# KumarRobotics/top_down_renderer

Measured on AMD Instinct MI355X. Metric: particle-updates/sec (render+score+resample), higher is better.
Workload: dtype f32

## Files before the change

top_down_renderer_amd/csrc/tdr_common.h:

```cpp
#ifndef TDR_COMMON_H_
#define TDR_COMMON_H_
#include <hip/hip_runtime.h>

#include <cmath>
#include <cstdarg>
#include <cstdint>
#include <cstdio>
#include <cstdlib>
#include <cstring>
#include <limits>
#include <type_traits>
#include <utility>
#include <vector>

#include "tdr.h"
#include "tdr_config.h"
#include "tdr_internal.h"

#ifndef TDR_SCORE_U
#define TDR_SCORE_U 4
#endif
#ifndef TDR_XCD_SWIZZLE
#define TDR_XCD_SWIZZLE 0
#endif
#ifndef TDR_OOB_ALIAS
#define TDR_OOB_ALIAS 1
#endif

int tdr_fail(int code, const char* fmt, ...);
#define fail tdr_fail
#define HIP_TRY(expr)                                                                       \
  do {                                                                                      \
    hipError_t e_ = (expr);                                                                 \
    if (e_ != hipSuccess) return fail(TDR_ERR_HIP, "%s: %s", #expr, hipGetErrorString(e_)); \
  } while (0)
#define LAUNCH_CHECK(name)                                                                   \
  do {                                                                                       \
    hipError_t e_ = hipGetLastError();                                                       \
    if (e_ != hipSuccess) return fail(TDR_ERR_HIP, "launch %s: %s", name, hipGetErrorString(e_)); \
  } while (0)

int tdr_libm_fma();

static inline int64_t cdiv(int64_t a, int64_t b) { return (a + b - 1) / b; }

template <class F>
static inline int with_flags(F&& f) { return f(); }
template <class F, class... Rest>
static inline int with_flags(F&& f, bool b, Rest... rest) {
  auto next = [&](auto B) { return with_flags([&](auto... bs) { return f(B, bs...); }, rest...); };
  return b ? next(std::true_type{}) : next(std::false_type{});
}
template <class F>
static inline int with_nv4(int rf, const char* who, F&& f) {
  switch (rf / 4) {
    case 1: return f(std::integral_constant<int, 1>{});
    case 2: return f(std::integral_constant<int, 2>{});
    case 3: return f(std::integral_constant<int, 3>{});
    case 4: return f(std::integral_constant<int, 4>{});
    default: return fail(TDR_ERR_ARG, "%s: unsupported record size %d", who, rf);
  }
}

#define PFX_HEAD 2048
#define INI_TILE 2048
#define INI_MAX_TILES 2048
int tdr_chain_total(const float* raw, const float* mean_dev, int kind, int64_t n, float* total_out, void* workspace,
                    bool have_sums, hipStream_t st);
struct UwExact {
  float sum, mean, bsum, pad;
};
int tdr_uw_chunk_pass1(const float* raw, int64_t n, void* workspace, int* cnt_valid, hipStream_t st);
int tdr_uw_chunk_pass2(const float* raw, int64_t n, UwExact* ex, const int* cnt_valid, void* workspace, int* cnt_under,
                       hipStream_t st);
int tdr_uw_small(const float* raw, const float* last_dist, int64_t n, float* w, float* info, hipStream_t st);
int tdr_mt_raw_stream(const uint32_t* state, int64_t nblocks, uint32_t* raw, hipStream_t s);
int tdr_mt_advance(const uint32_t* raw, int64_t nblocks, const uint32_t* consumed, uint32_t* state, hipStream_t s);
__host__ __device__ inline bool tdr_has_kslot(int ncls, int rf) { return ncls + 2 <= rf; }
uint32_t* tdr_profile_stats_ptr();
uint32_t* tdr_profile_gate_ptr();
uint32_t* tdr_profile_su_list_ptr();
#endif
```

top_down_renderer_amd/csrc/tdr_filter.hip:

```cpp
#include <random>

#include <rocprim/device/device_radix_sort.hpp>
using TdrSortConfig = rocprim::radix_sort_config<rocprim::default_config, rocprim::merge_sort_config<512, 512, 4>, rocprim::default_config>;

#include "tdr_common.h"
#include "tdr_filter_dev.h"

__device__ __forceinline__ uint32_t mulhi32(uint32_t a, uint32_t b) { return __umulhi(a, b); }
__device__ void philox4x32_10(uint32_t c[4], uint32_t k0, uint32_t k1) {
#pragma unroll
  for (int r = 0; r < 10; r++) {
    uint32_t hi0 = mulhi32(0xD2511F53u, c[0]), lo0 = 0xD2511F53u * c[0];
    uint32_t hi1 = mulhi32(0xCD9E8D57u, c[2]), lo1 = 0xCD9E8D57u * c[2];
    uint32_t n0 = hi1 ^ c[1] ^ k0, n1 = lo1, n2 = hi0 ^ c[3] ^ k1, n3 = lo0;
    c[0] = n0; c[1] = n1; c[2] = n2; c[3] = n3;
    k0 += 0x9E3779B9u; k1 += 0xBB67AE85u;
  }
}

__global__ void propagate_kernel(float* __restrict__ st, int64_t cap, int64_t n, float* __restrict__ last_dist,
                                 float tx, float ty, float omega, int scale_freeze, float pos_cov, float theta_cov,
                                 const float* __restrict__ z4, uint64_t seed, uint64_t step, int64_t index_base,
                                 int libm_fma) {
  const int64_t p = (int64_t)blockIdx.x * blockDim.x + threadIdx.x;
  if (p >= n) return;
  float z[4];
  if (z4) {
    z[0] = z4[4 * p]; z[1] = z4[4 * p + 1]; z[2] = z4[4 * p + 2]; z[3] = z4[4 * p + 3];
  } else {
    uint64_t gi = (uint64_t)(index_base + p);
    uint32_t c[4] = {(uint32_t)gi, (uint32_t)(gi >> 32), (uint32_t)step, (uint32_t)(step >> 32)};
    philox4x32_10(c, (uint32_t)seed, (uint32_t)(seed >> 32));
    float u0 = ((float)(c[0] >> 8) + 1.0f) * (1.0f / 16777216.0f), u1 = (float)(c[1] >> 8) * (1.0f / 16777216.0f);
    float u2 = ((float)(c[2] >> 8) + 1.0f) * (1.0f / 16777216.0f), u3 = (float)(c[3] >> 8) * (1.0f / 16777216.0f);
    float r0 = sqrtf(-2.0f * logf(u0)), r1 = sqrtf(-2.0f * logf(u2));
    z[0] = r0 * cosf(6.283185307f * u1); z[1] = r0 * sinf(6.283185307f * u1);
    z[2] = r1 * cosf(6.283185307f * u3); z[3] = r1 * sinf(6.283185307f * u3);
  }
  propagate_particle(st, cap, p, last_dist, z, tx, ty, omega, scale_freeze, pos_cov, theta_cov, libm_fma);
}

extern "C" int tdr_k_propagate(float* st, int64_t cap, int64_t n, float* last_dist, float tx, float ty, float omega,
                               int scale_freeze, float pos_cov, float theta_cov, const float* z4, uint64_t seed,
                               uint64_t step, int64_t index_base, void* stream) {
  if (!st || !last_dist) return fail(TDR_ERR_ARG, "propagate: null pointer");
  if (n < 0 || cap < n) return fail(TDR_ERR_ARG, "propagate: n exceeds capacity");
  if (n == 0) return TDR_OK;
  hipLaunchKernelGGL(propagate_kernel, dim3((unsigned)cdiv(n, 256)), dim3(256), 0, (hipStream_t)stream, st, cap, n,
                     last_dist, tx, ty, omega, scale_freeze, pos_cov, theta_cov, z4, seed, step, index_base,
                     tdr_libm_fma());
  LAUNCH_CHECK("propagate");
  return TDR_OK;
}

extern "C" void* tdr_rng_create(uint32_t seed) { return new std::mt19937(seed); }
extern "C" void tdr_rng_destroy(void* rng) { delete (std::mt19937*)rng; }
extern "C" float tdr_rng_uniform_host(void* rng) {
  std::uniform_real_distribution<float> d(0., 1.);
  return d(*(std::mt19937*)rng);
}
extern "C" int tdr_propagate_normals_host(void* rng, int64_t n, int scale_freeze, float* z4) {
  if (!rng || !z4 || n < 0) return fail(TDR_ERR_ARG, "propagate_normals: bad arguments");
  std::mt19937& gen = *(std::mt19937*)rng;
  for (int64_t p = 0; p < n; p++) {
    std::normal_distribution<float> disp{0, 1}, th{0, 1};
    z4[4 * p + 0] = th(gen);
    z4[4 * p + 1] = disp(gen);
    z4[4 * p + 2] = disp(gen);
    if (!scale_freeze) {
      std::normal_distribution<float> sc{0, 1};
      z4[4 * p + 3] = sc(gen);
    } else {
      z4[4 * p + 3] = 0.f;
    }
  }
  return TDR_OK;
}

static bool on_road_host(const float* maps, int ncls, int rows, int cols, float resolution, int px, int py) {
  const int c0 = (int)((float)px / resolution), c1 = (int)((float)py / resolution);
  if (ncls < 2) return false;
  if (!(c0 < cols && c1 < rows && c0 >= 0 && c1 >= 0)) return false;
  return maps[(size_t)1 * rows * cols + c1 + (size_t)rows * c0] < 1;
}
static tdr_state draw_particle(std::mt19937& gen, const float* maps, int ncls, int rows, int cols, float resolution,
                               const tdr_filter_params* fp) {
  std::uniform_real_distribution<float> uniform_dist(0., 1.);
  std::normal_distribution<float> normal_dist(0., 1.);
  tdr_state st;
  std::memset(&st, 0, sizeof(st));
  const float map_w = (float)cols * resolution, map_h = (float)rows * resolution;
  if (fp->fixed_scale < 0) st.scale = (float)std::pow(10, ((double)uniform_dist(gen) - 0.5) * 2);
  else st.scale = fp->fixed_scale;
  while (true) {
    if (fp->init_pos_px_x > 0) {
      st.init_x_px = std::min(std::max(normal_dist(gen) * fp->init_pos_px_cov + fp->init_pos_px_x, 0.f), map_w);
      st.init_y_px = std::min(std::max(normal_dist(gen) * fp->init_pos_px_cov + fp->init_pos_px_y, 0.f), map_h);
    } else {
      st.init_x_px = uniform_dist(gen) * map_w;
      st.init_y_px = uniform_dist(gen) * map_h;
    }
    if (on_road_host(maps, ncls, rows, cols, resolution, (int)st.init_x_px, (int)st.init_y_px)) break;
  }
  if (fp->init_pos_deg_theta != std::numeric_limits<float>::infinity()) {
    st.theta = normal_dist(gen) * fp->init_pos_deg_cov + fp->init_pos_deg_theta;
    st.theta = (float)((double)st.theta * (M_PI / 180));
    st.have_init = 1;
  } else {
    st.theta = 0;
    st.have_init = 0;
  }
  return st;
}
extern "C" int tdr_init_particle_host(void* rng, const float* class_maps, int ncls, int rows, int cols, float resolution,
                                      const tdr_filter_params* fp, tdr_state* out) {
  if (!rng || !class_maps || !fp || !out) return fail(TDR_ERR_ARG, "init_particle: bad arguments");
  if (ncls < 2) return fail(TDR_ERR_ARG, "init_particle: class 1 (road) is required for the on-road test");
  bool any_road = false;
  for (size_t k = 0; k < (size_t)rows * cols && !any_road; k++) any_road = class_maps[(size_t)rows * cols + k] < 1;
  if (!any_road) return fail(TDR_ERR_ARG, "init_particle: the map has no road cell, rejection sampling cannot end");
  *out = draw_particle(*(std::mt19937*)rng, class_maps, ncls, rows, cols, resolution, fp);
  return TDR_OK;
}
extern "C" int tdr_init_particles_host(void* rng, const float* class_maps, int ncls, int rows, int cols,
                                       float resolution, const tdr_filter_params* fp, int max_num, tdr_state* out,
                                       int64_t* n_out) {
  if (!rng || !class_maps || !fp || !out || !n_out || max_num < 0) return fail(TDR_ERR_ARG, "init_particles: bad arguments");
  if (ncls < 2) return fail(TDR_ERR_ARG, "init_particles: class 1 (road) is required for the on-road test");
  std::mt19937& gen = *(std::mt19937*)rng;
  bool any_road = false;
  for (size_t k = 0; k < (size_t)rows * cols && !any_road; k++) any_road = class_maps[(size_t)rows * cols + k] < 1;
  if (!any_road) return fail(TDR_ERR_ARG, "init_particles: the map has no road cell, rejection sampling cannot end");
  const size_t num_at_scale = (fp->fixed_scale < 0) ? 10 : 1;
  int64_t count = 0;
  for (int i = 0; i < (int)((size_t)max_num / num_at_scale); i++) {
    const tdr_state proto = draw_particle(gen, class_maps, ncls, rows, cols, resolution, fp);
    for (float scale = 0; scale < 1; scale += 1. / num_at_scale) {
      tdr_state part = draw_particle(gen, class_maps, ncls, rows, cols, resolution, fp);
      if (fp->fixed_scale < 0) {
        part = proto;
        part.scale = (float)std::pow(10., (double)scale);
      }
      if (count < max_num + 16) out[count] = part;
      count++;
      (void)draw_particle(gen, class_maps, ncls, rows, cols, resolution, fp);
    }
  }
  *n_out = count;
  return TDR_OK;
}

__device__ long long block_sum_ll(long long v, long long* sh) {
  const int lane = threadIdx.x & 63, wave = threadIdx.x >> 6;
  for (int o = 32; o > 0; o >>= 1) v += __shfl_down(v, o, 64);
  __syncthreads();
  if (lane == 0) sh[wave] = v;
  __syncthreads();
  long long t = 0;
  const int nw = blockDim.x >> 6;
  for (int w = 0; w < nw; w++) t += sh[w];
  return t;
}

#define UW_G 256
struct UwScratch {
  double a[UW_G];
  double b[UW_G];
};
__device__ __forceinline__ void uw_chunk(int64_t n, int64_t& lo, int64_t& hi) {
  const int64_t per = (n + UW_G - 1) / UW_G;
  lo = (int64_t)blockIdx.x * per;
  hi = lo + per < n ? lo + per : n;
  if (lo > n) lo = n;
}
__device__ double uw_total(const double* part) {
  __shared__ double stage[UW_G];
  __shared__ double result;
  __syncthreads();
  for (int g = threadIdx.x; g < UW_G; g += blockDim.x) stage[g] = part[g];
  __syncthreads();
  if (threadIdx.x == 0) {
    double t = 0;
    for (int g = 0; g < UW_G; g++) t += stage[g];
    result = t;
  }
  __syncthreads();
  return result;
}
__device__ long long uw_count_total(const int* __restrict__ cnt, int nch, long long* shl) {
  long long c = 0;
  for (int j = threadIdx.x; j < nch; j += blockDim.x) c += cnt[j];
  return block_sum_ll(c, shl);
}
__global__ __launch_bounds__(256) void uw_pass3(const float* __restrict__ raw, int64_t n, const UwExact* ex,
                                                const int* __restrict__ cnt_under, int nch, UwScratch* s3,
                                                float* __restrict__ w) {
  __shared__ double shd[4];
  __shared__ long long shl[4];
  const float sum = ex->sum, mean = ex->mean;
  const long long num_under = uw_count_total(cnt_under, nch, shl);
  const float bottom = sqrtf(ex->bsum / (float)num_under);
  const bool fallback = (sum == 0.f || num_under < 1);
  const float fill = mean - bottom;
  int64_t lo, hi;
  uw_chunk(n, lo, hi);
  double acc = 0;
  for (int64_t i = lo + threadIdx.x; i < hi; i += 256) {
    float v = raw[i];
    v = fallback ? 1.f : (isnan(v) ? fill : v);
    w[i] = v;
    acc += (double)v;
  }
  const double t = block_sum_d(acc, shd);
  if (threadIdx.x == 0) s3->a[blockIdx.x] = t;
}
__global__ __launch_bounds__(256) void uw_pass4(const float* __restrict__ last_dist, int64_t n, const UwScratch* s3,
                                                UwScratch* s4, float* __restrict__ w) {
  __shared__ double shd[4];
  const float fs1 = (float)uw_total(s3->a);
  const float fn = (float)n;
  int64_t lo, hi;
  uw_chunk(n, lo, hi);
  double acc = 0;
  for (int64_t i = lo + threadIdx.x; i < hi; i += 256) {
    float v = w[i] / fs1;
    const float d = fminf(last_dist[i] * 5.f, 1.f);
    v = d * v + (1.f - d) / fn;
    w[i] = v;
    acc += (double)v;
  }
  const double t = block_sum_d(acc, shd);
  if (threadIdx.x == 0) s4->a[blockIdx.x] = t;
}
__device__ __forceinline__ void uw_write_info(const UwScratch* s5, const int* __restrict__ cnt_valid,
                                              const int* __restrict__ cnt_under, int nch, const UwExact* ex, float* info) {
  static_assert(UW_G == 256, "one candidate per thread");
  __shared__ float sb[4];
  __shared__ long long si[4];
  __shared__ long long shl[4];
  float best = (float)s5->a[threadIdx.x];
  long long besti = (long long)s5->b[threadIdx.x];
  if (best != best) { best = -INFINITY; besti = 0x7fffffffffffffffll; }
  for (int o = 32; o > 0; o >>= 1) {
    const float ob = __shfl_down(best, o, 64);
    const long long oi = __shfl_down(besti, o, 64);
    if (ob > best || (ob == best && oi < besti)) { best = ob; besti = oi; }
  }
  if ((threadIdx.x & 63) == 0) { sb[threadIdx.x >> 6] = best; si[threadIdx.x >> 6] = besti; }
  const float sum = ex->sum, mean = ex->mean;
  const long long nv = uw_count_total(cnt_valid, nch, shl), nu = uw_count_total(cnt_under, nch, shl);
  const float bottom = sqrtf(ex->bsum / (float)nu);
  if (threadIdx.x != 0) return;
  for (int k = 1; k < 4; k++)
    if (sb[k] > best || (sb[k] == best && si[k] < besti)) { best = sb[k]; besti = si[k]; }
  if (besti == 0x7fffffffffffffffll) besti = 0;
  info[0] = __int_as_float((int)besti);
  info[1] = sum; info[2] = mean; info[3] = bottom; info[4] = (sum == 0.f || nu < 1) ? 1.f : 0.f;
  info[5] = (float)nv; info[6] = (float)nu; info[7] = 0.f;
}
__global__ __launch_bounds__(256) void uw_pass5(int64_t n, const UwScratch* s4, UwScratch* s5, float* __restrict__ w) {
  __shared__ float sb[4];
  __shared__ long long si[4];
  const float fs2 = (float)uw_total(s4->a);
  int64_t lo, hi;
  uw_chunk(n, lo, hi);
  float best = -INFINITY;
  long long besti = 0x7fffffffffffffffll;
  for (int64_t i = lo + threadIdx.x; i < hi; i += 256) {
    const float v = w[i] / fs2;
    w[i] = v;
    if (v > best || (v == best && i < besti)) { best = v; besti = i; }
  }
  for (int o = 32; o > 0; o >>= 1) {
    const float ob = __shfl_down(best, o, 64);
    const long long oi = __shfl_down(besti, o, 64);
    if (ob > best || (ob == best && oi < besti)) { best = ob; besti = oi; }
  }
  if ((threadIdx.x & 63) == 0) { sb[threadIdx.x >> 6] = best; si[threadIdx.x >> 6] = besti; }
  __syncthreads();
  if (threadIdx.x == 0) {
    for (int k = 1; k < 4; k++)
      if (sb[k] > best || (sb[k] == best && si[k] < besti)) { best = sb[k]; besti = si[k]; }
    s5->a[blockIdx.x] = (double)best;
    s5->b[blockIdx.x] = (double)besti;
  }
}
__global__ __launch_bounds__(256) void uw_pass6(const UwScratch* s5, const int* __restrict__ cnt_valid,
                                                const int* __restrict__ cnt_under, int nch, const UwExact* ex, float* info) {
  uw_write_info(s5, cnt_valid, cnt_under, nch, ex, info);
}

#define TDR_UW_SINGLE_MAX_N 32768
extern "C" int tdr_k_update_weights(const float* raw_w, const float* last_dist, int64_t n, float* w_out,
                                    float* info_out, void* stream) {
  if (!raw_w || !last_dist || !w_out || !info_out) return fail(TDR_ERR_ARG, "update_weights: null pointer");
  if (n < 1) return fail(TDR_ERR_ARG, "update_weights: n must be >= 1");
  hipStream_t s = (hipStream_t)stream;
  if (n <= TDR_UW_SINGLE_MAX_N) {
    const int rc = tdr_uw_small(raw_w, last_dist, n, w_out, info_out, s);
    if (rc) return rc;
    LAUNCH_CHECK("update_weights");
    return TDR_OK;
  }
  constexpr size_t kFixed = 8 * sizeof(float) + 64 + 3 * sizeof(UwScratch) + sizeof(UwExact) + 64;
  static_assert(kFixed + 40 * 1024 <= TDR_UW_INFO_FLOATS * sizeof(float), "info scratch");
  UwScratch* sc = reinterpret_cast<UwScratch*>(
      (reinterpret_cast<uintptr_t>(info_out + 8) + 63) & ~(uintptr_t)63);
  UwExact* ex = reinterpret_cast<UwExact*>(sc + 3);
  void* chain_ws = reinterpret_cast<void*>((reinterpret_cast<uintptr_t>(ex + 1) + 63) & ~(uintptr_t)63);
  const size_t chain_room = TDR_UW_INFO_FLOATS * sizeof(float) - kFixed;
  const int64_t nch = tdr_prefix_workspace_bytes(n) / 32;
  if ((size_t)tdr_prefix_workspace_bytes(n) + (size_t)nch * 2 * sizeof(int) > chain_room)
    return fail(TDR_ERR_ARG, "update_weights: n = %lld needs more than TDR_UW_INFO_FLOATS of scratch", (long long)n);
  int* cnt_valid = reinterpret_cast<int*>(reinterpret_cast<char*>(chain_ws) + tdr_prefix_workspace_bytes(n));
  int* cnt_under = cnt_valid + nch;
  int rc = tdr_uw_chunk_pass1(raw_w, n, chain_ws, cnt_valid, s);
  if (rc) return rc;
  rc = tdr_chain_total(raw_w, nullptr, 0, n, &ex->sum, chain_ws, true, s);
  if (rc) return rc;
  rc = tdr_uw_chunk_pass2(raw_w, n, ex, cnt_valid, chain_ws, cnt_under, s);
  if (rc) return rc;
  rc = tdr_chain_total(raw_w, &ex->mean, 1, n, &ex->bsum, chain_ws, true, s);
  if (rc) return rc;
  hipLaunchKernelGGL(uw_pass3, dim3(UW_G), dim3(256), 0, s, raw_w, n, (const UwExact*)ex, (const int*)cnt_under, (int)nch,
                     sc + 0, w_out);
  hipLaunchKernelGGL(uw_pass4, dim3(UW_G), dim3(256), 0, s, last_dist, n, (const UwScratch*)(sc + 0), sc + 1, w_out);
  hipLaunchKernelGGL(uw_pass5, dim3(UW_G), dim3(256), 0, s, n, (const UwScratch*)(sc + 1), sc + 2, w_out);
  hipLaunchKernelGGL(uw_pass6, dim3(1), dim3(256), 0, s, (const UwScratch*)(sc + 2), (const int*)cnt_valid,
                     (const int*)cnt_under, (int)nch, (const UwExact*)ex, info_out);
  LAUNCH_CHECK("update_weights(multi)");
  return TDR_OK;
}

__global__ void resample_kernel(const float* __restrict__ runmax, int64_t n, int64_t n_new, float shift,
                                int64_t i_begin, int64_t i_end, int32_t* __restrict__ idx) {
  const int64_t i = i_begin + (int64_t)blockIdx.x * blockDim.x + threadIdx.x;
  if (i >= i_end) return;
  idx[i - i_begin] = (int32_t)resample_pick(runmax, n, n_new, i, shift);
}

extern "C" int tdr_k_resample(const float* runmax, int64_t n, int64_t n_new, float shift, int64_t i_begin,
                              int64_t i_end, int32_t* idx_out, void* stream) {
  if (!runmax || !idx_out) return fail(TDR_ERR_ARG, "resample: null pointer");
  if (n < 1 || n_new < 1 || i_begin < 0 || i_end > n_new || i_begin > i_end)
    return fail(TDR_ERR_ARG, "resample: bad range");
  if (i_begin == i_end) return TDR_OK;
  hipLaunchKernelGGL(resample_kernel, dim3((unsigned)cdiv(i_end - i_begin, 256)), dim3(256), 0, (hipStream_t)stream,
                     runmax, n, n_new, shift, i_begin, i_end, idx_out);
  LAUNCH_CHECK("resample");
  return TDR_OK;
}

__global__ void resample_dev_kernel(const float* __restrict__ runmax, int64_t n, int64_t n_new, const float* __restrict__ shift_dev,
                                    int64_t i_begin, int64_t i_end, int32_t* __restrict__ idx) {
  const int64_t i = i_begin + (int64_t)blockIdx.x * blockDim.x + threadIdx.x;
  if (i >= i_end) return;
  idx[i - i_begin] = (int32_t)resample_pick(runmax, n, n_new, i, *shift_dev);
}
extern "C" int tdr_k_resample_dev(const float* runmax, int64_t n, int64_t n_new, const float* shift_dev, int64_t i_begin,
                                  int64_t i_end, int32_t* idx_out, void* stream) {
  if (!runmax || !idx_out || !shift_dev) return fail(TDR_ERR_ARG, "resample: null pointer");
  if (n < 1 || n_new < 1 || i_begin < 0 || i_end > n_new || i_begin > i_end)
    return fail(TDR_ERR_ARG, "resample: bad range");
  if (i_begin == i_end) return TDR_OK;
  hipLaunchKernelGGL(resample_dev_kernel, dim3((unsigned)cdiv(i_end - i_begin, 256)), dim3(256), 0, (hipStream_t)stream,
                     runmax, n, n_new, shift_dev, i_begin, i_end, idx_out);
  LAUNCH_CHECK("resample");
  return TDR_OK;
}

__device__ __forceinline__ void gather_state(const float* __restrict__ src, int64_t src_cap, int64_t src_shard, int64_t j,
                                             float* __restrict__ dst, int64_t dst_cap, int64_t i) {
  if (src_shard > 0) {
    const int64_t r = j / src_shard, l = j - r * src_shard;
#pragma unroll
    for (int f = 0; f < TDR_ST_FIELDS; f++) dst[f * dst_cap + i] = src[(r * TDR_ST_FIELDS + f) * src_shard + l];
  } else {
    gather_particle(src, src_cap, j, dst, dst_cap, i);
  }
}
__global__ void gather_states_kernel(const float* __restrict__ src, int64_t src_cap, int64_t src_shard,
                                     const int32_t* __restrict__ idx, int64_t n_new, float* __restrict__ dst,
                                     int64_t dst_cap) {
  const int64_t i = (int64_t)blockIdx.x * blockDim.x + threadIdx.x;
  if (i >= n_new) return;
  gather_state(src, src_cap, src_shard, idx[i], dst, dst_cap, i);
}

extern "C" int tdr_k_gather_states(const float* src, int64_t src_cap, int64_t src_shard, const int32_t* idx,
                                   int64_t n_new, float* dst, int64_t dst_cap, void* stream) {
  if (!src || !idx || !dst) return fail(TDR_ERR_ARG, "gather_states: null pointer");
  if (n_new < 0 || dst_cap < n_new || src_shard < 0) return fail(TDR_ERR_ARG, "gather_states: n_new exceeds capacity");
  if (n_new == 0) return TDR_OK;
  hipLaunchKernelGGL(gather_states_kernel, dim3((unsigned)cdiv(n_new, 256)), dim3(256), 0, (hipStream_t)stream, src,
                     src_cap, src_shard, idx, n_new, dst, dst_cap);
  LAUNCH_CHECK("gather_states");
  return TDR_OK;
}

__device__ __forceinline__ McScratch* mc_scratch(float* out) { return reinterpret_cast<McScratch*>(out + 24); }
__global__ __launch_bounds__(1024) void mean_cov_kernel(const float* __restrict__ st, int64_t cap, int64_t n,
                                                       const float* __restrict__ about, float* __restrict__ out,
                                                       int libm_fma) {
  mean_cov_body(st, cap, n, about, out, libm_fma);
}
__global__ __launch_bounds__(MC_THREADS) void mc_sums_kernel(const float* __restrict__ st, int64_t cap, int64_t n,
                                                             float* __restrict__ out, int libm_fma) {
  mc_sums_body(st, cap, n, mc_scratch(out), libm_fma);
}
__global__ __launch_bounds__(MC_THREADS) void mc_cov_kernel(const float* __restrict__ st, int64_t cap, int64_t n,
                                                            const float* __restrict__ about, float* __restrict__ out) {
  mc_cov_body(st, cap, n, about, mc_scratch(out));
}
__global__ __launch_bounds__(MC_THREADS) void mc_final_kernel(int64_t n, const float* __restrict__ about,
                                                              float* __restrict__ out) {
  mc_final_body(n, about, mc_scratch(out), out);
}

extern "C" int tdr_k_mean_cov(const float* st, int64_t cap, int64_t n, const float* about, float* out, void* stream) {
  if (!st || !out || n < 1 || cap < n) return fail(TDR_ERR_ARG, "mean_cov: bad arguments");
  hipStream_t s = (hipStream_t)stream;
  if (n <= MC_SINGLE_MAX_N) {
    hipLaunchKernelGGL(mean_cov_kernel, dim3(1), dim3(1024), 0, s, st, cap, n, about, out, tdr_libm_fma());
  } else {
    hipLaunchKernelGGL(mc_sums_kernel, dim3(MC_WGS), dim3(MC_THREADS), 0, s, st, cap, n, out, tdr_libm_fma());
    hipLaunchKernelGGL(mc_cov_kernel, dim3(MC_WGS), dim3(MC_THREADS), 0, s, st, cap, n, about, out);
    hipLaunchKernelGGL(mc_final_kernel, dim3(1), dim3(MC_THREADS), 0, s, n, about, out);
  }
  LAUNCH_CHECK("mean_cov");
  return TDR_OK;
}

__global__ void set_scale_kernel(float* __restrict__ st, int64_t cap, int64_t n, const float* __restrict__ scale) {
  const int64_t p = (int64_t)blockIdx.x * blockDim.x + threadIdx.x;
  if (p < n) st[TDR_ST_SCALE * cap + p] = *scale;
}
extern "C" int tdr_k_set_scale(float* st, int64_t cap, int64_t n, const float* scale_dev, void* stream) {
  if (!st || !scale_dev || n < 0 || cap < n) return fail(TDR_ERR_ARG, "set_scale: bad arguments");
  if (n == 0) return TDR_OK;
  hipLaunchKernelGGL(set_scale_kernel, dim3((unsigned)cdiv(n, 256)), dim3(256), 0, (hipStream_t)stream, st, cap, n,
                     scale_dev);
  LAUNCH_CHECK("set_scale");
  return TDR_OK;
}

__global__ void shift_init_kernel(float* __restrict__ st, int64_t cap, int64_t n, float dx, float dy) {
  const int64_t p = (int64_t)blockIdx.x * blockDim.x + threadIdx.x;
  if (p < n) {
    st[TDR_ST_INIT_X * cap + p] += dx;
    st[TDR_ST_INIT_Y * cap + p] += dy;
  }
}
extern "C" int tdr_k_shift_init(float* st, int64_t cap, int64_t n, float dx, float dy, void* stream) {
  if (!st || n < 0 || cap < n) return fail(TDR_ERR_ARG, "shift_init: bad arguments");
  if (n == 0) return TDR_OK;
  hipLaunchKernelGGL(shift_init_kernel, dim3((unsigned)cdiv(n, 256)), dim3(256), 0, (hipStream_t)stream, st, cap, n,
                     dx, dy);
  LAUNCH_CHECK("shift_init");
  return TDR_OK;
}

__device__ __forceinline__ void save_ml_state(const float* __restrict__ info, const float* __restrict__ st, int64_t cap,
                                              int64_t src_shard, int64_t n, float* __restrict__ out) {
  const int64_t best = ml_index(info, n);
  float f[TDR_ST_FIELDS];
  if (src_shard > 0) {
    const int64_t r = best / src_shard, l = best - r * src_shard;
#pragma unroll
    for (int k = 0; k < TDR_ST_FIELDS; k++) f[k] = st[(r * TDR_ST_FIELDS + k) * src_shard + l];
  } else {
#pragma unroll
    for (int k = 0; k < TDR_ST_FIELDS; k++) f[k] = st[(int64_t)k * cap + best];
  }
  ml_record(f, out);
}
__global__ void save_ml_state_kernel(const float* __restrict__ info, const float* __restrict__ st, int64_t cap,
                                     int64_t src_shard, int64_t n, float* __restrict__ out) {
  if (threadIdx.x != 0 || blockIdx.x != 0) return;
  save_ml_state(info, st, cap, src_shard, n, out);
}
extern "C" int tdr_k_save_ml_state(const float* info, const float* st, int64_t cap, int64_t src_shard, int64_t n,
                                   float* out12, void* stream) {
  if (!info || !st || !out12 || n < 1 || src_shard < 0 || (src_shard == 0 && cap < n))
    return fail(TDR_ERR_ARG, "save_ml_state: bad arguments");
  hipLaunchKernelGGL(save_ml_state_kernel, dim3(1), dim3(64), 0, (hipStream_t)stream, info, st, cap, src_shard, n,
                     out12);
  LAUNCH_CHECK("save_ml_state");
  return TDR_OK;
}

__global__ __launch_bounds__(256) void resample_gather_kernel(const float* __restrict__ runmax, int64_t n, int64_t n_new,
                                                              const float* __restrict__ shift_dev, float shift,
                                                              int64_t i_begin, int64_t i_end, int32_t* __restrict__ idx,
                                                              const float* __restrict__ src, int64_t src_cap,
                                                              int64_t src_shard, float* __restrict__ dst, int64_t dst_cap,
                                                              const float* __restrict__ info, float* __restrict__ out12) {
  const int64_t i = i_begin + (int64_t)blockIdx.x * blockDim.x + threadIdx.x;
  if (i < i_end) {
    const int64_t j = resample_pick(runmax, n, n_new, i, shift_dev ? *shift_dev : shift);
    idx[i - i_begin] = (int32_t)j;
    gather_state(src, src_cap, src_shard, j, dst, dst_cap, i - i_begin);
  }
  if (blockIdx.x == 0 && threadIdx.x == 0) save_ml_state(info, src, src_cap, src_shard, n, out12);
}
extern "C" int tdr_k_resample_gather(const float* runmax, int64_t n, int64_t n_new, const float* shift_dev, float shift,
                                     int64_t i_begin, int64_t i_end, int32_t* idx_out, const float* src, int64_t src_cap,
                                     int64_t src_shard, float* dst, int64_t dst_cap, const float* info, float* out12,
                                     void* stream) {
  if (!runmax || !idx_out || !src || !dst || !info || !out12) return fail(TDR_ERR_ARG, "resample_gather: null pointer");
  if (n < 1 || n_new < 1 || i_begin < 0 || i_end > n_new || i_begin > i_end)
    return fail(TDR_ERR_ARG, "resample_gather: bad range");
  if (src_shard < 0 || (src_shard == 0 && src_cap < n) || dst_cap < i_end - i_begin || dst == src)
    return fail(TDR_ERR_ARG, "resample_gather: bad state buffers");
  const unsigned blocks = (unsigned)std::max<int64_t>(1, cdiv(i_end - i_begin, 256));
  hipLaunchKernelGGL(resample_gather_kernel, dim3(blocks), dim3(256), 0, (hipStream_t)stream, runmax, n, n_new, shift_dev,
                     shift, i_begin, i_end, idx_out, src, src_cap, src_shard, dst, dst_cap, info, out12);
  LAUNCH_CHECK("resample_gather");
  return TDR_OK;
}

__global__ void sample_ml_states_kernel(const float* __restrict__ st, int64_t cap, int64_t n, int num,
                                        float* __restrict__ out) {
  const int i = blockIdx.x * blockDim.x + threadIdx.x;
  if (i >= num) return;
  sample_ml_state(st, cap, n, num, i, out + 3 * i);
}
extern "C" int tdr_k_sample_ml_states(const float* st, int64_t cap, int64_t n, int num, float* out, void* stream) {
  if (!st || !out || n < 1 || cap < n || num < 1) return fail(TDR_ERR_ARG, "sample_ml_states: bad arguments");
  hipLaunchKernelGGL(sample_ml_states_kernel, dim3((unsigned)cdiv(num, 256)), dim3(256), 0, (hipStream_t)stream, st,
                     cap, n, num, out);
  LAUNCH_CHECK("sample_ml_states");
  return TDR_OK;
}

__global__ void shard_pack2_kernel(const float* __restrict__ a, const float* __restrict__ b, int64_t nl,
                                   float* __restrict__ out) {
  const int64_t i = (int64_t)blockIdx.x * blockDim.x + threadIdx.x;
  if (i < nl) { out[i] = a[i]; out[nl + i] = b[i]; }
}
__global__ void shard_unpack2_kernel(const float* __restrict__ in, int world, int64_t nl, float* __restrict__ a,
                                     float* __restrict__ b) {
  const int64_t g = (int64_t)blockIdx.x * blockDim.x + threadIdx.x;
  if (g >= (int64_t)world * nl) return;
  const int64_t r = g / nl, l = g - r * nl;
  a[g] = in[(2 * r) * nl + l];
  b[g] = in[(2 * r + 1) * nl + l];
}
__global__ void unshard_states_kernel(const float* __restrict__ in, int world, int64_t nl, float* __restrict__ st,
                                      int64_t cap) {
  const int64_t g = (int64_t)blockIdx.x * blockDim.x + threadIdx.x;
  if (g >= (int64_t)world * nl) return;
  const int64_t r = g / nl, l = g - r * nl;
#pragma unroll
  for (int f = 0; f < TDR_ST_FIELDS; f++) st[f * cap + g] = in[(r * TDR_ST_FIELDS + f) * nl + l];
}
extern "C" int tdr_k_shard_pack2(const float* a, const float* b, int64_t nl, float* out, void* stream) {
  if (!a || !b || !out || nl < 0) return fail(TDR_ERR_ARG, "shard_pack2: bad arguments");
  if (nl == 0) return TDR_OK;
  hipLaunchKernelGGL(shard_pack2_kernel, dim3((unsigned)cdiv(nl, 256)), dim3(256), 0, (hipStream_t)stream, a, b, nl, out);
  LAUNCH_CHECK("shard_pack2");
  return TDR_OK;
}
extern "C" int tdr_k_shard_unpack2(const float* in, int world, int64_t nl, float* a_glob, float* b_glob, void* stream) {
  if (!in || !a_glob || !b_glob || world < 1 || nl < 0) return fail(TDR_ERR_ARG, "shard_unpack2: bad arguments");
  if (nl == 0) return TDR_OK;
  hipLaunchKernelGGL(shard_unpack2_kernel, dim3((unsigned)cdiv((int64_t)world * nl, 256)), dim3(256), 0,
                     (hipStream_t)stream, in, world, nl, a_glob, b_glob);
  LAUNCH_CHECK("shard_unpack2");
  return TDR_OK;
}
extern "C" int tdr_k_unshard_states(const float* in, int world, int64_t nl, float* st, int64_t cap, void* stream) {
  if (!in || !st || world < 1 || nl < 0 || cap < (int64_t)world * nl) return fail(TDR_ERR_ARG, "unshard_states: bad arguments");
  if (nl == 0) return TDR_OK;
  hipLaunchKernelGGL(unshard_states_kernel, dim3((unsigned)cdiv((int64_t)world * nl, 256)), dim3(256), 0,
                     (hipStream_t)stream, in, world, nl, st, cap);
  LAUNCH_CHECK("unshard_states");
  return TDR_OK;
}

__global__ void aos_to_soa_kernel(const tdr_state* __restrict__ aos, int64_t n, float* __restrict__ st, int64_t cap) {
  const int64_t p = (int64_t)blockIdx.x * blockDim.x + threadIdx.x;
  if (p >= n) return;
  const tdr_state s = aos[p];
  st[TDR_ST_INIT_X * cap + p] = s.init_x_px;
  st[TDR_ST_INIT_Y * cap + p] = s.init_y_px;
  st[TDR_ST_DX * cap + p] = s.dx_m;
  st[TDR_ST_DY * cap + p] = s.dy_m;
  st[TDR_ST_THETA * cap + p] = s.theta;
  st[TDR_ST_SCALE * cap + p] = s.scale;
  st[TDR_ST_HAVE_INIT * cap + p] = s.have_init ? 1.f : 0.f;
}
__global__ void soa_to_aos_kernel(const float* __restrict__ st, int64_t cap, int64_t n, tdr_state* __restrict__ aos) {
  const int64_t p = (int64_t)blockIdx.x * blockDim.x + threadIdx.x;
  if (p >= n) return;
  tdr_state s;
  s.init_x_px = st[TDR_ST_INIT_X * cap + p];
  s.init_y_px = st[TDR_ST_INIT_Y * cap + p];
  s.dx_m = st[TDR_ST_DX * cap + p];
  s.dy_m = st[TDR_ST_DY * cap + p];
  s.theta = st[TDR_ST_THETA * cap + p];
  s.scale = st[TDR_ST_SCALE * cap + p];
  s.have_init = st[TDR_ST_HAVE_INIT * cap + p] != 0.f;
  s.pad_[0] = s.pad_[1] = s.pad_[2] = 0;
  aos[p] = s;
}
extern "C" int tdr_k_states_aos_to_soa(const tdr_state* aos, int64_t n, float* st, int64_t cap, void* stream) {
  if (!aos || !st || n < 0 || cap < n) return fail(TDR_ERR_ARG, "aos_to_soa: bad arguments");
  if (n == 0) return TDR_OK;
  hipLaunchKernelGGL(aos_to_soa_kernel, dim3((unsigned)cdiv(n, 256)), dim3(256), 0, (hipStream_t)stream, aos, n, st,
                     cap);
  LAUNCH_CHECK("aos_to_soa");
  return TDR_OK;
}
extern "C" int tdr_k_states_soa_to_aos(const float* st, int64_t cap, int64_t n, tdr_state* aos, void* stream) {
  if (!aos || !st || n < 0 || cap < n) return fail(TDR_ERR_ARG, "soa_to_aos: bad arguments");
  if (n == 0) return TDR_OK;
  hipLaunchKernelGGL(soa_to_aos_kernel, dim3((unsigned)cdiv(n, 256)), dim3(256), 0, (hipStream_t)stream, st, cap, n,
                     aos);
  LAUNCH_CHECK("soa_to_aos");
  return TDR_OK;
}

__device__ __forceinline__ uint32_t spread_bits16(uint32_t v) {
  v &= 0xFFFFu;
  v = (v | (v << 8)) & 0x00FF00FFu;
  v = (v | (v << 4)) & 0x0F0F0F0Fu;
  v = (v | (v << 2)) & 0x33333333u;
  v = (v | (v << 1)) & 0x55555555u;
  return v;
}
__global__ void loc_key_kernel(const float* __restrict__ st, int64_t cap, int64_t n, float xmax, float ymax,
                               uint32_t* __restrict__ keys, int32_t* __restrict__ vals) {
  const int64_t p = (int64_t)blockIdx.x * blockDim.x + threadIdx.x;
  if (p >= n) return;
  const float sc = st[TDR_ST_SCALE * cap + p];
  float cx = st[TDR_ST_DX * cap + p] * sc + st[TDR_ST_INIT_X * cap + p];
  float cy = st[TDR_ST_DY * cap + p] * sc + st[TDR_ST_INIT_Y * cap + p];
  if (!(cx == cx)) cx = 0.f;
  if (!(cy == cy)) cy = 0.f;
  const uint32_t hx = (uint32_t)fminf(fmaxf(cx * 2.f, 0.f), xmax);
  const uint32_t hy = (uint32_t)fminf(fmaxf(cy * 2.f, 0.f), ymax);
  keys[p] = spread_bits16(hx) | (spread_bits16(hy) << 1);
  vals[p] = (int32_t)p;
}

__device__ __forceinline__ uint64_t spread_bits21_3(uint64_t v) {
  v &= 0x1FFFFFull;
  v = (v | (v << 32)) & 0x1F00000000FFFFull;
  v = (v | (v << 16)) & 0x1F0000FF0000FFull;
  v = (v | (v << 8)) & 0x100F00F00F00F00Full;
  v = (v | (v << 4)) & 0x10C30C30C30C30C3ull;
  v = (v | (v << 2)) & 0x1249249249249249ull;
  return v;
}
__global__ void loc_key_pose_kernel(const float* __restrict__ st, int64_t cap, int64_t n, float xmax, float ymax,
                                    float theta_step, uint64_t* __restrict__ keys, int32_t* __restrict__ vals) {
  const int64_t p = (int64_t)blockIdx.x * blockDim.x + threadIdx.x;
  if (p >= n) return;
  const float sc = st[TDR_ST_SCALE * cap + p];
  float cx = st[TDR_ST_DX * cap + p] * sc + st[TDR_ST_INIT_X * cap + p];
  float cy = st[TDR_ST_DY * cap + p] * sc + st[TDR_ST_INIT_Y * cap + p];
  float th = st[TDR_ST_THETA * cap + p];
  if (!(cx == cx)) cx = 0.f;
  if (!(cy == cy)) cy = 0.f;
  if (!(fabsf(th) < 1e6f)) th = 0.f;
  th = th - 6.2831855f * floorf(th / 6.2831855f);
  const uint64_t hx = (uint64_t)fminf(fmaxf(cx * 2.f, 0.f), xmax);
  const uint64_t hy = (uint64_t)fminf(fmaxf(cy * 2.f, 0.f), ymax);
  const uint64_t ht = (uint64_t)fminf(fmaxf(th / theta_step, 0.f), 2097151.f);
  keys[p] = spread_bits21_3(hx) | (spread_bits21_3(hy) << 1) | (spread_bits21_3(ht) << 2);
  vals[p] = (int32_t)p;
}
static size_t radix_tmp_bytes64(int64_t n) {
  size_t bytes = 0;
  uint64_t* k = nullptr;
  int32_t* v = nullptr;
  hipError_t e = rocprim::radix_sort_pairs(nullptr, bytes, k, k, v, v, (size_t)n, 0u, 63u, (hipStream_t)0, false);
  if (e != hipSuccess || bytes == 0) bytes = (size_t)(n + 4096) * 32;
  return bytes;
}
extern "C" size_t tdr_locality_pose_tmp_ints(int64_t n) {
  if (n < 1) n = 1;
  return (size_t)(5 * n + 64) + (radix_tmp_bytes64(n) + 3) / 4 + 64;
}
extern "C" int tdr_k_locality_order_pose(const float* st, int64_t cap, int64_t n, int map_rows, int map_cols,
                                         float theta_radius, int32_t* perm_out, int32_t* keys_tmp, void* stream) {
  if (!st || !perm_out || !keys_tmp || n < 0 || cap < n || map_rows < 1 || map_cols < 1 || !(theta_radius > 0.f))
    return fail(TDR_ERR_ARG, "locality_order_pose: bad arguments");
  if (map_rows > 1000000 || map_cols > 1000000) return fail(TDR_ERR_ARG, "locality_order_pose: map too large");
  if (n == 0) return TDR_OK;
  hipStream_t s = (hipStream_t)stream;
  uint64_t* keys_in = reinterpret_cast<uint64_t*>(keys_tmp);
  uint64_t* keys_out = keys_in + n;
  int32_t* vals_in = keys_tmp + 4 * n;
  void* tmp = keys_tmp + 5 * n + 64 - ((5 * n) % 64);
  size_t tmp_bytes = radix_tmp_bytes64(n);
  hipLaunchKernelGGL(loc_key_pose_kernel, dim3((unsigned)cdiv(n, 256)), dim3(256), 0, s, st, cap, n,
                     (float)(2 * map_cols - 1), (float)(2 * map_rows - 1), 0.5f / theta_radius, keys_in, vals_in);
  LAUNCH_CHECK("loc_key_pose");
  HIP_TRY(rocprim::radix_sort_pairs(tmp, tmp_bytes, keys_in, keys_out, vals_in, perm_out, (size_t)n, 0u, 63u, s, false));
  return TDR_OK;
}

static size_t radix_tmp_bytes(int64_t n) {
  size_t bytes = 0;
  uint32_t* k = nullptr;
  int32_t* v = nullptr;
  hipError_t e = rocprim::radix_sort_pairs<TdrSortConfig>(nullptr, bytes, k, k, v, v, (size_t)n, 0u, 32u, (hipStream_t)0, false);
  if (e != hipSuccess || bytes == 0) bytes = (size_t)(n + 4096) * 16;
  return bytes;
}

extern "C" size_t tdr_locality_tmp_ints(int64_t n, int map_rows, int map_cols) {
  (void)map_rows; (void)map_cols;
  if (n < 1) n = 1;
  return (size_t)(3 * n + 64) + (radix_tmp_bytes(n) + 3) / 4 + 64;
}

extern "C" int tdr_k_locality_order(const float* st, int64_t cap, int64_t n, int map_rows, int map_cols,
                                    int32_t* perm_out, int32_t* keys_tmp, void* stream) {
  if (!st || !perm_out || !keys_tmp || n < 0 || cap < n || map_rows < 1 || map_cols < 1)
    return fail(TDR_ERR_ARG, "locality_order: bad arguments");
  if (map_rows > 32767 || map_cols > 32767) return fail(TDR_ERR_ARG, "locality_order: map larger than 32767 px");
  if (n == 0) return TDR_OK;
  hipStream_t s = (hipStream_t)stream;
  uint32_t* keys_in = reinterpret_cast<uint32_t*>(keys_tmp);
  uint32_t* keys_out = keys_in + n;
  int32_t* vals_in = keys_tmp + 2 * n;
  void* tmp = keys_tmp + 3 * n + 64 - ((3 * n) % 64);
  size_t tmp_bytes = radix_tmp_bytes(n);
  hipLaunchKernelGGL(loc_key_kernel, dim3((unsigned)cdiv(n, 256)), dim3(256), 0, s, st, cap, n,
                     (float)(2 * map_cols - 1), (float)(2 * map_rows - 1), keys_in, vals_in);
  LAUNCH_CHECK("loc_key");
  unsigned bits = 2;
  while ((1u << (bits / 2)) < (unsigned)(2 * std::max(map_rows, map_cols)) && bits < 32) bits += 2;
  HIP_TRY(rocprim::radix_sort_pairs<TdrSortConfig>(tmp, tmp_bytes, keys_in, keys_out, vals_in, perm_out, (size_t)n, 0u, bits, s,
                                    false));
  return TDR_OK;
}
```

top_down_renderer_amd/csrc/tdr_prefix.hip:

```cpp
#include "tdr_common.h"
#include "tdr_batch.h"

#define TDR_PFX_BLOCK 4096
__global__ __launch_bounds__(64) void prefix_serial_kernel(const float* __restrict__ w, int64_t n,
                                                           float* __restrict__ runmax) {
  __shared__ float4 buf4[TDR_PFX_BLOCK / 4];
  float* buf = reinterpret_cast<float*>(buf4);
  const int lane = threadIdx.x;
  float run = 0.f;
  float carry_max = -INFINITY;
  for (int64_t base = 0; base < n; base += TDR_PFX_BLOCK) {
    const int cnt = (int)min((int64_t)TDR_PFX_BLOCK, n - base);
    for (int t = lane; t < TDR_PFX_BLOCK; t += 64) buf[t] = (t < cnt) ? w[base + t] : 0.f;
    __builtin_amdgcn_s_waitcnt(0);
    __builtin_amdgcn_wave_barrier();
    if (lane == 0) {
      const int q4 = (cnt + 3) / 4;
#pragma unroll 4
      for (int q = 0; q < q4; q++) {
        float4 v = buf4[q];
        run = run + v.x; v.x = run;
        run = run + v.y; v.y = run;
        run = run + v.z; v.z = run;
        run = run + v.w; v.w = run;
        buf4[q] = v;
      }
    }
    __builtin_amdgcn_s_waitcnt(0);
    __builtin_amdgcn_wave_barrier();
    float m = -INFINITY;
    float loc[64];
#pragma unroll
    for (int t = 0; t < 64; t++) {
      float x = buf[lane * 64 + t];
      if (x != x) x = -INFINITY;
      m = fmaxf(m, x);
      loc[t] = m;
    }
    float incl = m;
#pragma unroll
    for (int o = 1; o < 64; o <<= 1) {
      float t = __shfl_up(incl, o, 64);
      if (lane >= o) incl = fmaxf(incl, t);
    }
    float excl = __shfl_up(incl, 1, 64);
    if (lane == 0) excl = -INFINITY;
    excl = fmaxf(excl, carry_max);
    __builtin_amdgcn_wave_barrier();
#pragma unroll
    for (int t = 0; t < 64; t++) buf[lane * 64 + t] = fmaxf(loc[t], excl);
    __builtin_amdgcn_s_waitcnt(0);
    __builtin_amdgcn_wave_barrier();
    for (int t = lane; t < cnt; t += 64) runmax[base + t] = buf[t];
    carry_max = fmaxf(__shfl(incl, 63, 64), carry_max);
    __builtin_amdgcn_s_waitcnt(0);
    __builtin_amdgcn_wave_barrier();
  }
}

#define PFX_THREADS 1024
#define PFX_K 8
#define PFX_TILE (PFX_THREADS * PFX_K)
#define PFX_TIE_CAP 2048

__device__ __forceinline__ void pfx_sync() {
  __builtin_amdgcn_fence(__ATOMIC_RELEASE, "workgroup", "local");
  __builtin_amdgcn_s_barrier();
  __builtin_amdgcn_fence(__ATOMIC_ACQUIRE, "workgroup", "local");
}

template <int NT, class T>
__device__ __forceinline__ T pfx_block_scan(T v, T* sh, T& total) {
  const int lane = threadIdx.x & 63, wave = threadIdx.x >> 6;
#pragma unroll
  for (int o = 1; o < 64; o <<= 1) {
    T t = __shfl_up(v, o, 64);
    if (lane >= o) v += t;
  }
  pfx_sync();
  if (lane == 63) sh[wave] = v;
  pfx_sync();
  T off = 0, tot = 0;
#pragma unroll
  for (int k = 0; k < NT / 64; k++) {
    const T x = sh[k];
    if (k < wave) off += x;
    tot += x;
  }
  total = tot;
  return v + off;
}
template <int NT>
__device__ __forceinline__ float pfx_block_scan_max(float v, float* sh) {
  const int lane = threadIdx.x & 63, wave = threadIdx.x >> 6;
#pragma unroll
  for (int o = 1; o < 64; o <<= 1) {
    float t = __shfl_up(v, o, 64);
    if (lane >= o) v = fmaxf(v, t);
  }
  pfx_sync();
  if (lane == 63) sh[wave] = v;
  pfx_sync();
  float off = -INFINITY;
  for (int k = 0; k < wave; k++) off = fmaxf(off, sh[k]);
  return fmaxf(v, off);
}

template <int NT>
__device__ __forceinline__ void pfx_exact_range(const float* __restrict__ w, long long lo, long long hi,
                                             float* __restrict__ runmax, float* __restrict__ prefix_opt,
                                             float& r_io, float& carry_io, int head_len = PFX_HEAD) {
  const long long n = hi;
  __shared__ long long sh_ll[NT / 64];
  __shared__ int sh_i[NT / 64];
  __shared__ float sh_f[NT / 64];
  __shared__ int tie_pos[PFX_TIE_CAP];
  __shared__ long long tie_sval[PFX_TIE_CAP];
  __shared__ signed char tie_corr[PFX_TIE_CAP];
  __shared__ float head[PFX_HEAD];
  __shared__ float last_val[NT], last_max[NT];
  __shared__ int s_first_bad, s_first_cross, s_first_nz;
  __shared__ float s_r, s_carry;
  __shared__ long long s_base;
  const int tid = threadIdx.x;
  pfx_sync();
  if (tid == 0) { s_r = r_io; s_carry = carry_io; s_base = lo; }
  pfx_sync();
  if (lo == 0) {
    const int hn = (int)min((long long)head_len, (long long)n);
    for (int t = tid; t < hn; t += NT) head[t] = w[t];
    pfx_sync();
    if (tid == 0) {
      float run = 0.f, mx = -INFINITY;
      for (int t = 0; t < hn; t++) {
        run = run + head[t];
        if (prefix_opt) prefix_opt[t] = run;
        if (run == run) mx = fmaxf(mx, run);
        head[t] = mx;
      }
      s_r = run; s_carry = mx; s_base = hn;
    }
    pfx_sync();
    for (int t = tid; t < hn; t += NT) runmax[t] = head[t];
    pfx_sync();
  }

  while (true) {
    const long long base = s_base;
    if (base >= n) break;
    const float r = s_r;
    const float carry = s_carry;
    const int cnt = (int)min((long long)(NT * PFX_K), (long long)n - base);
    const unsigned rb = __float_as_uint(r);
    const int re = (rb >> 23) & 0xFF;
    float wv[PFX_K];
#pragma unroll
    for (int k = 0; k < PFX_K; k++) {
      const int li = tid * PFX_K + k;
      wv[k] = (li < cnt) ? w[base + li] : 0.f;
    }
    if (tid == 0) { s_first_bad = (NT * PFX_K); s_first_cross = (NT * PFX_K); s_first_nz = (NT * PFX_K); }
    pfx_sync();

    if (r != r) {
#pragma unroll
      for (int k = 0; k < PFX_K; k++) {
        const int li = tid * PFX_K + k;
        if (li < cnt) {
          runmax[base + li] = carry;
          if (prefix_opt) prefix_opt[base + li] = r;
        }
      }
      pfx_sync();
      if (tid == 0) s_base = base + cnt;
      pfx_sync();
      continue;
    }
    const bool r_zero = (rb & 0x7FFFFFFFu) == 0;
    const bool r_slow = (rb >> 31) != 0 || re == 0 || re == 255;
    if (r_slow) {
      int stop = 0;
      if (r_zero) {
#pragma unroll
        for (int k = 0; k < PFX_K; k++) {
          const int li = tid * PFX_K + k;
          if (li < cnt && (__float_as_uint(wv[k]) & 0x7FFFFFFFu) != 0) atomicMin(&s_first_nz, li);
        }
        pfx_sync();
        stop = min(s_first_nz, cnt);
      }
      const float m0 = fmaxf(carry, r);
#pragma unroll
      for (int k = 0; k < PFX_K; k++) {
        const int li = tid * PFX_K + k;
        if (li < stop) {
          runmax[base + li] = m0;
          if (prefix_opt) prefix_opt[base + li] = r;
        }
      }
      pfx_sync();
      if (tid == 0) {
        float nr = r, nc = stop > 0 ? m0 : carry;
        long long nb = base + stop;
        if (stop < cnt) {
          nr = r + w[base + stop];
          if (nr == nr) nc = fmaxf(nc, nr);
          runmax[base + stop] = nc;
          if (prefix_opt) prefix_opt[base + stop] = nr;
          nb = base + stop + 1;
        }
        s_r = nr; s_carry = nc; s_base = nb;
      }
      pfx_sync();
      continue;
    }

    const int e = re - 127;
    const long long R = (long long)((rb & 0x7FFFFFu) | 0x800000u);
    long long inc[PFX_K];
    bool tie[PFX_K], neg[PFX_K];
    long long tsum = 0;
    int ntie = 0;
#pragma unroll
    for (int k = 0; k < PFX_K; k++) {
      const int li = tid * PFX_K + k;
      const unsigned b = __float_as_uint(wv[k]);
      const int ew = (b >> 23) & 0xFF;
      unsigned mw = b & 0x7FFFFFu;
      const bool zero = (b & 0x7FFFFFFFu) == 0;
      const int E = ew == 0 ? -126 : ew - 127;
      if (ew != 0) mw |= 0x800000u;
      const int sft = e - E;
      const bool in = li < cnt;
      const bool bad = in && ((ew == 255) || (sft < 0));
      neg[k] = (b >> 31) != 0 && !zero;
      const int sc = sft < 0 ? 0 : (sft > 26 ? 26 : sft);
      const unsigned f = mw >> sc;
      const unsigned rem = mw & ((1u << sc) - 1u);
      const unsigned half = sc >= 1 ? (1u << (sc - 1)) : 0u;
      const bool up = sc >= 1 && rem > half;
      tie[k] = in && !bad && sc >= 1 && rem == half;
      long long q = (long long)f + (up ? 1 : 0);
      if (neg[k]) q = -q;
      if (!in || bad) q = 0;
      if (bad) atomicMin(&s_first_bad, li);
      inc[k] = q;
      tsum += q;
      ntie += tie[k] ? 1 : 0;
    }
    long long tot_ll;
    const long long sincl = pfx_block_scan<NT, long long>(tsum, sh_ll, tot_ll);
    long long S[PFX_K];
    {
      long long acc = sincl - tsum;
#pragma unroll
      for (int k = 0; k < PFX_K; k++) { acc += inc[k]; S[k] = acc; }
    }
    int tot_tie;
    const int tincl = pfx_block_scan<NT, int>(ntie, sh_i, tot_tie);
    const int tfirst = tincl - ntie;
    {
      int pos = tfirst;
#pragma unroll
      for (int k = 0; k < PFX_K; k++)
        if (tie[k]) {
          if (pos < PFX_TIE_CAP) {
            tie_pos[pos] = (tid * PFX_K + k) | (neg[k] ? (int)0x80000000 : 0);
            tie_sval[pos] = S[k];
          } else if (pos == PFX_TIE_CAP) {
            atomicMin(&s_first_bad, tid * PFX_K + k);
          }
          pos++;
        }
    }
    pfx_sync();
    if (tid == 0 && tot_tie > 0) {
      long long c = 0;
      const int fb = s_first_bad;
      const int nt = min(tot_tie, PFX_TIE_CAP);
      for (int t = 0; t < nt; t++) {
        const int pk = tie_pos[t];
        const int li = pk & 0x7FFFFFFF;
        signed char corr = 0;
        if (li < fb) {
          const long long V = R + tie_sval[t] + c;
          if (V & 1) corr = (pk < 0) ? -1 : 1;
        }
        tie_corr[t] = corr;
        c += corr;
      }
    }
    pfx_sync();
    int csum = 0;
    int corr[PFX_K];
    {
      int pos = tfirst;
#pragma unroll
      for (int k = 0; k < PFX_K; k++) {
        corr[k] = 0;
        if (tie[k]) { corr[k] = pos < PFX_TIE_CAP ? tie_corr[pos] : 0; pos++; }
        csum += corr[k];
      }
    }
    int tot_c;
    const int cincl = pfx_block_scan<NT, int>(csum, sh_i, tot_c);
    long long state[PFX_K];
    {
      int cacc = cincl - csum;
#pragma unroll
      for (int k = 0; k < PFX_K; k++) {
        cacc += corr[k];
        state[k] = R + S[k] + cacc;
        const int li = tid * PFX_K + k;
        if (li < cnt && (state[k] >= (1ll << 24) || state[k] < (1ll << 23))) atomicMin(&s_first_cross, li);
      }
    }
    pfx_sync();
    const int stop = min(min(s_first_bad, s_first_cross), cnt);
    float val[PFX_K], lm[PFX_K];
    float m = -INFINITY;
#pragma unroll
    for (int k = 0; k < PFX_K; k++) {
      const int li = tid * PFX_K + k;
      val[k] = __uint_as_float(((unsigned)re << 23) | ((unsigned)state[k] & 0x7FFFFFu));
      if (li < stop) m = fmaxf(m, val[k]);
      lm[k] = m;
    }
    const float mincl = pfx_block_scan_max<NT>(m, sh_f);
    float mexcl = __shfl_up(mincl, 1, 64);
    {
      pfx_sync();
      last_max[tid] = mincl;
      pfx_sync();
      mexcl = tid > 0 ? last_max[tid - 1] : -INFINITY;
    }
    const float mbase = fmaxf(carry, mexcl);
    float lastv = r, lastm = carry;
#pragma unroll
    for (int k = 0; k < PFX_K; k++) {
      const int li = tid * PFX_K + k;
      if (li < stop) {
        const float rm = fmaxf(mbase, lm[k]);
        runmax[base + li] = rm;
        if (prefix_opt) prefix_opt[base + li] = val[k];
        lastv = val[k];
        lastm = rm;
      }
    }
    pfx_sync();
    last_val[tid] = lastv;
    last_max[tid] = lastm;
    pfx_sync();
    if (tid == 0) {
      float pv = r, pm = carry;
      if (stop > 0) {
        const int ot = (stop - 1) / PFX_K;
        pv = last_val[ot];
        pm = last_max[ot];
      }
      long long nb = base + stop;
      if (stop < cnt) {
        const float nr = pv + w[base + stop];
        if (nr == nr) pm = fmaxf(pm, nr);
        runmax[base + stop] = pm;
        if (prefix_opt) prefix_opt[base + stop] = nr;
        pv = nr;
        nb = base + stop + 1;
      }
      s_r = pv; s_carry = pm; s_base = nb;
    }
    pfx_sync();
  }
  r_io = s_r;
  carry_io = s_carry;
  pfx_sync();
}

__global__ __launch_bounds__(PFX_THREADS) void prefix_exact_kernel(const float* __restrict__ w, int64_t n,
                                                                   float* __restrict__ runmax,
                                                                   float* __restrict__ prefix_opt) {
  float r = 0.f, carry = -INFINITY;
  pfx_exact_range<PFX_THREADS>(w, 0, n, runmax, prefix_opt, r, carry);
}

#define PFXM_THREADS 256
#define PFXM_K 16
#define PFXM_CHUNK (PFXM_THREADS * PFXM_K)
#define PFXM_SAT (1u << 30)
struct PfxChunk {
  double sum;
  int re;
  unsigned d0, d1;
  float r0, carry0;
  int accepted;
};
static_assert(sizeof(PfxChunk) == 32, "PfxChunk");
#ifndef PFXW_THREADS
#define PFXW_THREADS 512
#endif
#define PFXW_K (PFXM_CHUNK / PFXW_THREADS)
#define CHAIN_K PFXW_K
#define UWS_WC (64 * CHAIN_K)
#define PFXM_RE_MIN 24
#define PFXM_RE_MAX 254

#ifdef TDR_UW_TIMELINE
__device__ unsigned long long g_uw_tl[16];
extern "C" int tdr_debug_read_uw_timeline(unsigned long long* out) {
  return hipMemcpyFromSymbol(out, HIP_SYMBOL(g_uw_tl), sizeof(unsigned long long) * 16) == hipSuccess ? 0 : -1;
}
#define UW_STAMP(k) do { __syncthreads(); if (threadIdx.x == 0) g_uw_tl[k] = wall_clock64(); } while (0)
#define UW_COUNT(k) do { if (threadIdx.x == 0) g_uw_tl[k]++; } while (0)
#else
#define UW_STAMP(k) do { } while (0)
#define UW_COUNT(k) do { } while (0)
#endif

struct PfxPair { unsigned a0, a1; };
__device__ __forceinline__ unsigned pfx_sat(unsigned x) { return x > PFXM_SAT ? PFXM_SAT : x; }
__device__ __forceinline__ PfxPair pfx_compose(PfxPair A, PfxPair B) {
  PfxPair c;
  c.a0 = pfx_sat(A.a0 + ((A.a0 & 1u) ? B.a1 : B.a0));
  c.a1 = pfx_sat(A.a1 + ((A.a1 & 1u) ? B.a0 : B.a1));
  return c;
}
__device__ __forceinline__ PfxPair pfx_element_pair(unsigned f, bool tie) {
  PfxPair p;
  p.a0 = f + (tie ? (f & 1u) : 0u);
  p.a1 = f + (tie ? ((f & 1u) ^ 1u) : 0u);
  return p;
}
template <int K>
__device__ __forceinline__ PfxPair chain_lane_pair(const unsigned (&f)[K], unsigned tiebits) {
  PfxPair mine = {0u, 0u};
#pragma unroll
  for (int k = 0; k < K; k++) mine = pfx_compose(mine, pfx_element_pair(f[k], ((tiebits >> k) & 1u) != 0u));
  return mine;
}
template <int CTRL, int ROW_MASK>
__device__ __forceinline__ PfxPair pfx_pair_dpp(PfxPair v) {
  PfxPair t;
  t.a0 = (unsigned)__builtin_amdgcn_update_dpp(0, (int)v.a0, CTRL, ROW_MASK, 0xF, false);
  t.a1 = (unsigned)__builtin_amdgcn_update_dpp(0, (int)v.a1, CTRL, ROW_MASK, 0xF, false);
  return t;
}
__device__ __forceinline__ PfxPair pfx_pair_wave_scan(PfxPair v) {
  v = pfx_compose(pfx_pair_dpp<0x111, 0xF>(v), v);
  v = pfx_compose(pfx_pair_dpp<0x112, 0xF>(v), v);
  v = pfx_compose(pfx_pair_dpp<0x114, 0xF>(v), v);
  v = pfx_compose(pfx_pair_dpp<0x118, 0xF>(v), v);
  v = pfx_compose(pfx_pair_dpp<0x142, 0xA>(v), v);
  v = pfx_compose(pfx_pair_dpp<0x143, 0xC>(v), v);
  return v;
}
template <int NT>
__device__ __forceinline__ PfxPair pfx_pair_scan(PfxPair v, PfxPair* sh, PfxPair& total) {
  const int lane = threadIdx.x & 63, wave = threadIdx.x >> 6;
  v = pfx_pair_wave_scan(v);
  pfx_sync();
  if (lane == 63) sh[wave] = v;
  pfx_sync();
  PfxPair pre = {0u, 0u}, tot = {0u, 0u};
#pragma unroll
  for (int k = 0; k < NT / 64; k++) {
    const PfxPair x = sh[k];
    if (k < wave) pre = pfx_compose(pre, x);
    tot = pfx_compose(tot, x);
  }
  total = tot;
  PfxPair ex = pfx_pair_dpp<0x138, 0xF>(v);
  return pfx_compose(pre, ex);
}
template <int CTRL, int ROW_MASK>
__device__ __forceinline__ int uws_min_dpp(int v) {
  return min(v, __builtin_amdgcn_update_dpp(0x7FFFFFFF, v, CTRL, ROW_MASK, 0xF, false));
}
__device__ __forceinline__ int uws_wave_min(int v) {
  v = uws_min_dpp<0x111, 0xF>(v);
  v = uws_min_dpp<0x112, 0xF>(v);
  v = uws_min_dpp<0x114, 0xF>(v);
  v = uws_min_dpp<0x118, 0xF>(v);
  v = uws_min_dpp<0x142, 0xA>(v);
  v = uws_min_dpp<0x143, 0xC>(v);
  return __builtin_amdgcn_readlane(v, 63);
}
template <int CTRL, int ROW_MASK>
__device__ __forceinline__ double uws_add_dpp(double v) {
  const int lo = __builtin_amdgcn_update_dpp(0, __double2loint(v), CTRL, ROW_MASK, 0xF, false);
  const int hi = __builtin_amdgcn_update_dpp(0, __double2hiint(v), CTRL, ROW_MASK, 0xF, false);
  return v + __hiloint2double(hi, lo);
}
__device__ __forceinline__ double uws_wave_scan_d(double v) {
  v = uws_add_dpp<0x111, 0xF>(v);
  v = uws_add_dpp<0x112, 0xF>(v);
  v = uws_add_dpp<0x114, 0xF>(v);
  v = uws_add_dpp<0x118, 0xF>(v);
  v = uws_add_dpp<0x142, 0xA>(v);
  v = uws_add_dpp<0x143, 0xC>(v);
  return v;
}
template <int CTRL, int ROW_MASK>
__device__ __forceinline__ unsigned uws_addu_dpp(unsigned v) {
  return v + (unsigned)__builtin_amdgcn_update_dpp(0, (int)v, CTRL, ROW_MASK, 0xF, false);
}
__device__ __forceinline__ unsigned uws_wave_scan_u(unsigned v) {
  v = uws_addu_dpp<0x111, 0xF>(v);
  v = uws_addu_dpp<0x112, 0xF>(v);
  v = uws_addu_dpp<0x114, 0xF>(v);
  v = uws_addu_dpp<0x118, 0xF>(v);
  v = uws_addu_dpp<0x142, 0xA>(v);
  v = uws_addu_dpp<0x143, 0xC>(v);
  return v;
}
template <int CTRL, int ROW_MASK>
__device__ __forceinline__ float pfs_max_dpp(float v) {
  return fmaxf(v, __uint_as_float((unsigned)__builtin_amdgcn_update_dpp((int)0xFF800000u, (int)__float_as_uint(v), CTRL,
                                                                        ROW_MASK, 0xF, false)));
}
__device__ __forceinline__ float pfs_wave_scan_max(float v) {
  v = pfs_max_dpp<0x111, 0xF>(v);
  v = pfs_max_dpp<0x112, 0xF>(v);
  v = pfs_max_dpp<0x114, 0xF>(v);
  v = pfs_max_dpp<0x118, 0xF>(v);
  v = pfs_max_dpp<0x142, 0xA>(v);
  v = pfs_max_dpp<0x143, 0xC>(v);
  return v;
}
__device__ __forceinline__ double uws_readlane_d(double v, int lane) {
  return __hiloint2double(__builtin_amdgcn_readlane(__double2hiint(v), lane),
                          __builtin_amdgcn_readlane(__double2loint(v), lane));
}
__device__ __forceinline__ double chain_readlane(double v, int lane) { return uws_readlane_d(v, lane); }
__device__ __forceinline__ float chain_readlane(float v, int lane) {
  return __uint_as_float((unsigned)__builtin_amdgcn_readlane((int)__float_as_uint(v), lane));
}
template <int NT>
__device__ __forceinline__ double chain_wg_sum(double acc, double* shd) {
#pragma unroll
  for (int o = 32; o >= 1; o >>= 1) acc += __shfl_xor(acc, o, 64);
  if ((threadIdx.x & 63) == 0) shd[threadIdx.x >> 6] = acc;
  pfx_sync();
  double t = 0.0;
  for (int k = 0; k < NT / 64; k++) t += shd[k];
  return t;
}

enum { CHAIN_SUM = 0, CHAIN_BOTTOM = 1, CHAIN_RUNSUM = 2 };
struct ChainGlobal {
  const float* p;
  static constexpr bool lds = false;
  __device__ __forceinline__ float read(long long i, bool take) const { return take ? p[i] : 0.f; }
};
__device__ __forceinline__ int uws_idx(int e) { return e + (e >> 5); }
#define UWS_PAD 16
template <bool GUARD>
struct ChainLds {
  static constexpr bool lds = true;
  __device__ __forceinline__ float read(long long i, bool take) const {
    extern __shared__ float uws_lraw[];
    if (GUARD) return take ? uws_lraw[uws_idx((int)i)] : 0.f;
    return uws_lraw[uws_idx((int)i)];
  }
};
__device__ __forceinline__ float chain_add(float r, float x) { return r + x; }
__device__ __forceinline__ float chain_add(float r, double x) { return (float)((double)r + x); }
__device__ __forceinline__ bool chain_finite(float x) { return fabsf(x) < INFINITY; }
__device__ __forceinline__ bool chain_finite(double x) { return fabs(x) < INFINITY; }
#define CHAIN_BOUND_24 24
#define CHAIN_BOUND_22 22
template <int LOG2_BOUND>
__device__ __forceinline__ void chain_classify(float x, unsigned re, unsigned& f, bool& tie, bool& bad) {
  const float t = x * __uint_as_float((277u - re) << 23);
  bad = !(x >= 0.f) || !(t < (float)(1 << LOG2_BOUND));
  const float fl = floorf(t);
  const float fr = t - fl;
  tie = fr == 0.5f;
  f = (unsigned)fl + (fr > 0.5f ? 1u : 0u);
  if (bad) { f = 0; tie = false; }
}
template <int LOG2_BOUND>
__device__ __forceinline__ void chain_classify(double x, unsigned re, unsigned& f, bool& tie, bool& bad) {
  const double scale = __longlong_as_double((long long)(1023 + 150 - (int)re) << 52);
  const double t = x * scale;
  bad = !(x >= 0.0) || !(t < (double)(1 << LOG2_BOUND));
  const double tg = (t + 8388608.0) - 8388608.0;
  const double fl = floor(tg);
  const double fr = tg - fl;
  tie = fr == 0.5;
  f = (unsigned)fl + (fr > 0.5 ? 1u : 0u);
  if (bad) { f = 0; tie = false; }
}
template <class X, class SRC, int LOG2B>
struct ChainAddend {
  using value_t = X;
  using src_t = SRC;
  SRC src;
  int kind;
  float mean;
  __device__ __forceinline__ X value(float v) const {
    if (kind == CHAIN_RUNSUM) return (X)v;
    if (kind == CHAIN_SUM) return (v != v) ? X(0) : (X)v;
    if (v != v || !(v < mean)) return X(0);
    const double d = (double)(v - mean);
    return (X)(d * d);
  }
  __device__ __forceinline__ X load(long long i, bool take) const {
    const X x = value(src.read(i, take));
    return take ? x : X(0);
  }
  template <int K>
  __device__ __forceinline__ void load_items(long long lo, int cnt, int t0, X (&xv)[K]) const {
    if constexpr (!SRC::lds && sizeof(X) == sizeof(float)) {
      if (t0 + K <= cnt && ((lo & 3) == 0)) {
        const float4* p = reinterpret_cast<const float4*>(src.p + lo + t0);
#pragma unroll
        for (int k = 0; k < K / 4; k++) {
          const float4 v = p[k];
          xv[4 * k] = value(v.x); xv[4 * k + 1] = value(v.y); xv[4 * k + 2] = value(v.z); xv[4 * k + 3] = value(v.w);
        }
        return;
      }
    }
#pragma unroll
    for (int k = 0; k < K; k++) xv[k] = load(lo + t0 + k, t0 + k < cnt);
  }
  static __device__ __forceinline__ void classify(X x, unsigned re, unsigned& f, bool& tie, bool& bad) {
    chain_classify<LOG2B>(x, re, f, tie, bad);
  }
  __device__ __forceinline__ ChainAddend<double, SRC, CHAIN_BOUND_22> as_double() const { return {src, kind, mean}; }
};
using PfxRunSum = ChainAddend<float, ChainGlobal, CHAIN_BOUND_24>;
using ChainStat = ChainAddend<double, ChainGlobal, CHAIN_BOUND_22>;
using UwsAddF = ChainAddend<float, ChainLds<false>, CHAIN_BOUND_22>;
using UwsAddD = ChainAddend<double, ChainLds<false>, CHAIN_BOUND_22>;
using UwsWgAdd = ChainAddend<double, ChainLds<true>, CHAIN_BOUND_22>;
__device__ __forceinline__ float chain_mant(unsigned re, unsigned state) { return __uint_as_float((re << 23) | (state & 0x7FFFFFu)); }

template <class X> struct ChainWgStop { int stop; unsigned state; X xstop; };
template <int NT, class X>
struct ChainWg {
  static constexpr bool nan_inf_apart = false;
  PfxPair* shp;
  ChainWgStop<X>* s;
  __device__ __forceinline__ bool leader() const { return threadIdx.x == 0; }
  __device__ __forceinline__ void reset(int cnt) const {
    pfx_sync();
    if (threadIdx.x == 0) s->stop = cnt;
    pfx_sync();
  }
  template <int K>
  __device__ __forceinline__ unsigned enter(unsigned R, const unsigned (&f)[K], unsigned tiebits) const {
    PfxPair total;
    const PfxPair ex = pfx_pair_scan<NT>(chain_lane_pair(f, tiebits), shp, total);
    return R + ((R & 1u) ? ex.a1 : ex.a0);
  }
  __device__ __forceinline__ int first_of(int first, int cnt) const {
    if (first < cnt) atomicMin(&s->stop, first);
    pfx_sync();
    return s->stop;
  }
  template <int K>
  __device__ __forceinline__ void pick(const unsigned (&st)[K], const X (&xv)[K], int t0, int pos, int stop, int cnt,
                                       unsigned& sv, X& xstop) const {
#pragma unroll
    for (int k = 0; k < K; k++) {
      const int li = t0 + k;
      if (li >= pos && li == stop - 1) s->state = st[k];
      if (li == stop) s->xstop = xv[k];
    }
    pfx_sync();
    sv = s->state;
    xstop = s->xstop;
  }
};
template <bool NOTIE>
struct ChainWave {
  static constexpr bool nan_inf_apart = true;
  __device__ __forceinline__ bool leader() const { return (threadIdx.x & 63) == 0; }
  __device__ __forceinline__ void reset(int) const {}
  template <int K>
  __device__ __forceinline__ unsigned enter(unsigned R, const unsigned (&f)[K], unsigned tiebits) const {
    if (NOTIE && __ballot(tiebits != 0u) == 0ull) {
      unsigned lane_sum = 0u;
#pragma unroll
      for (int k = 0; k < K; k++) lane_sum += f[k];
      return R + (uws_wave_scan_u(lane_sum) - lane_sum);
    }
    const PfxPair ex = pfx_pair_dpp<0x138, 0xF>(pfx_pair_wave_scan(chain_lane_pair(f, tiebits)));
    return R + ((R & 1u) ? ex.a1 : ex.a0);
  }
  __device__ __forceinline__ int first_of(int first, int) const { return uws_wave_min(first); }
  template <int K, class X>
  __device__ __forceinline__ void pick(const unsigned (&st)[K], const X (&xv)[K], int t0, int pos, int stop, int cnt,
                                       unsigned& sv, X& xstop) const {
    unsigned v = 0u;
    X xs = X(0);
#pragma unroll
    for (int k = 0; k < K; k++) {
      if (t0 + k == stop - 1) v = st[k];
      if (t0 + k == stop) xs = xv[k];
    }
    if (stop > pos) sv = (unsigned)__builtin_amdgcn_readlane((int)v, (stop - 1) / K);
    if (stop < cnt) xstop = chain_readlane(xs, stop / K);
  }
};

struct ChainNoSink {
  static constexpr bool own_irregular = false;
  __device__ __forceinline__ void put(int, int, float) {}
  __device__ __forceinline__ void committed(float) {}
  __device__ __forceinline__ void put_stop(int, int, float) {}
};
template <int K>
struct ChainRegSink {
  static constexpr bool own_irregular = false;
  float pv[K];
  __device__ __forceinline__ void put(int k, int, float v) { pv[k] = v; }
  __device__ __forceinline__ void committed(float) {}
  __device__ __forceinline__ void put_stop(int t0, int li, float r) {
#pragma unroll
    for (int k = 0; k < K; k++)
      if (t0 + k == li) pv[k] = r;
  }
};
struct PfxGlobalSink {
  static constexpr bool own_irregular = true;
  const float* __restrict__ w;
  long long lo;
  float* __restrict__ runmax;
  float* __restrict__ prefix_opt;
  float& carry;
  int head_len;
  __device__ __forceinline__ void put(int, int li, float v) {
    runmax[lo + li] = fmaxf(carry, v);
    if (prefix_opt) prefix_opt[lo + li] = v;
  }
  __device__ __forceinline__ void committed(float r) { carry = fmaxf(carry, r); }
  __device__ __forceinline__ void put_stop(int, int li, float nr) {
    if (nr == nr) carry = fmaxf(carry, nr);
    if (threadIdx.x == 0) {
      runmax[lo + li] = carry;
      if (prefix_opt) prefix_opt[lo + li] = nr;
    }
  }
  __device__ __forceinline__ void irregular(float& r, int& pos, int cnt) {
    const long long a = lo + pos;
    const long long b = a == 0 ? min((long long)head_len, (long long)cnt) : lo + cnt;
    pfx_exact_range<PFXW_THREADS>(w, a, b, runmax, prefix_opt, r, carry, head_len);
    pos = (int)(b - lo);
  }
};

template <bool STOP, class A, int K, class SCOPE>
__device__ __forceinline__ int chain_step(const typename A::value_t (&xv)[K], int t0, int pos, int cnt, float r,
                                          const SCOPE& sc, unsigned (&st)[K]) {
  const unsigned rb = __float_as_uint(r), re = rb >> 23, R = (rb & 0x7FFFFFu) | 0x800000u;
  unsigned f[K];
  unsigned tiebits = 0u;
  int first = cnt;
#pragma unroll
  for (int k = 0; k < K; k++) {
    const int li = t0 + k;
    bool bad, tie;
    A::classify(xv[k], re, f[k], tie, bad);
    if (STOP) {
      if (li < pos || li >= cnt) { f[k] = 0u; tie = false; bad = false; }
      if (bad) first = min(first, li);
    }
    tiebits |= tie ? (1u << k) : 0u;
  }
  unsigned state = sc.enter(R, f, tiebits);
#pragma unroll
  for (int k = 0; k < K; k++) {
    state += f[k] + (((tiebits >> k) & 1u) ? ((state + f[k]) & 1u) : 0u);
    st[k] = state;
    const int li = t0 + k;
    if (STOP && li >= pos && li < cnt && state >= (1u << 24)) first = min(first, li);
  }
  return first;
}
template <class A, int K, class SCOPE, class SINK>
__device__ __forceinline__ float chain_walk(const A& a, const typename A::value_t (&xv)[K], int t0, int pos, int cnt,
                                            float r, const SCOPE& sc, SINK& sink) {
  using X = typename A::value_t;
  while (pos < cnt) {
#ifdef TDR_UW_TIMELINE
    if (A::src_t::lds && a.kind < 2 && sc.leader()) g_uw_tl[10 + a.kind]++;
#endif
    const unsigned rb = __float_as_uint(r);
    const unsigned re = rb >> 23;
    const bool regular = re >= PFXM_RE_MIN && re <= PFXM_RE_MAX;
    if (SCOPE::nan_inf_apart && r != r) {
#pragma unroll
      for (int k = 0; k < K; k++)
        if (t0 + k >= pos && t0 + k < cnt) sink.put(k, t0 + k, r);
      break;
    }
    if constexpr (SINK::own_irregular) {
      if (!regular) {
        sink.irregular(r, pos, cnt);
        continue;
      }
    }
    sc.reset(cnt);
    int first = cnt;
    unsigned st[K] = {};
    if (!regular) {
      const bool isinf = SCOPE::nan_inf_apart && (rb & 0x7FFFFFFFu) == 0x7F800000u;
#pragma unroll
      for (int k = 0; k < K; k++) {
        const int li = t0 + k;
        const bool acts = isinf ? !chain_finite(xv[k]) : (xv[k] != X(0));
        if (li >= pos && li < cnt && acts) first = min(first, li);
      }
    } else {
      first = chain_step<true, A>(xv, t0, pos, cnt, r, sc, st);
    }
    const int stop = sc.first_of(first, cnt);
#pragma unroll
    for (int k = 0; k < K; k++)
      if (t0 + k >= pos && t0 + k < stop) sink.put(k, t0 + k, regular ? chain_mant(re, st[k]) : r);
    unsigned sv = 0u;
    X xstop = X(0);
    sc.pick(st, xv, t0, pos, stop, cnt, sv, xstop);
    if (regular) {
      if (stop > pos) r = chain_mant(re, sv);
      sink.committed(r);
    }
    if (stop < cnt) {
      r = chain_add(r, xstop);
      sink.put_stop(t0, stop, r);
      pos = stop + 1;
    } else {
      pos = cnt;
    }
  }
  return r;
}

template <bool KEEP, class A>
__device__ __forceinline__ float chain_head_lanes(const A& a, int hn) {
  using X = typename A::value_t;
  extern __shared__ float uws_lraw[];
  const int lane = threadIdx.x & 63;
  float run = 0.f;
  X nxt = a.load(min(lane, hn - 1), lane < hn);
  for (int b = 0; b < hn; b += 64) {
    const X cur = nxt;
    nxt = a.load(min(b + 64 + lane, hn - 1), b + 64 + lane < hn);
    float mine = 0.f;
#pragma unroll
    for (int j = 0; j < 64; j++) {
      run = chain_add(run, chain_readlane(cur, j));
      if (KEEP) mine = (lane == j) ? run : mine;
    }
    if (KEEP && b + lane < hn) uws_lraw[uws_idx(b + lane)] = mine;
  }
  return run;
}
#ifndef CHAIN_HEAD
#define CHAIN_HEAD 1024
#endif
template <int NT, class A>
__device__ __forceinline__ float chain_head_serial(const A& a, int hn, float r0) {
  __shared__ double head[CHAIN_HEAD];
  __shared__ float s_head_r;
  pfx_sync();
  for (int t = threadIdx.x; t < hn; t += NT) head[t] = a.load(t, true);
  pfx_sync();
  if (threadIdx.x == 0) {
    float run = r0;
    if (a.kind == CHAIN_SUM) {
      for (int t = 0; t < hn; t++) run = chain_add(run, (float)head[t]);
    } else {
      for (int t = 0; t < hn; t++) run = chain_add(run, head[t]);
    }
    s_head_r = run;
  }
  pfx_sync();
  return s_head_r;
}

template <int NT, int K, class A>
__device__ __forceinline__ void chain_sum_body(const A& a, int64_t n, PfxChunk* __restrict__ ch) {
  __shared__ double shd[NT / 64];
  const long long lo = (long long)blockIdx.x * PFXM_CHUNK;
  const int cnt = (int)min((long long)PFXM_CHUNK, (long long)n - lo);
  typename A::value_t xv[K];
  a.load_items(lo, cnt, threadIdx.x * K, xv);
  double acc = 0.0;
#pragma unroll
  for (int k = 0; k < K; k++) acc += (double)xv[k];
  const double t = chain_wg_sum<NT>(acc, shd);
  if (threadIdx.x == 0) ch[blockIdx.x].sum = t;
}
template <int NT, int K, class A>
__device__ __forceinline__ void chain_summary_body(const A& a, int64_t n, PfxChunk* __restrict__ ch, int c_first) {
  __shared__ double shd[NT / 64];
  __shared__ PfxPair shp[NT / 64];
  __shared__ int s_bad;
  const int c = blockIdx.x + c_first;
  const long long lo = (long long)c * PFXM_CHUNK;
  const int cnt = (int)min((long long)PFXM_CHUNK, (long long)n - lo);
  double acc = 0.0;
  for (int j = threadIdx.x; j < c; j += NT) acc += ch[j].sum;
  if (threadIdx.x == 0) s_bad = 0;
  const double before = chain_wg_sum<NT>(acc, shd);
  const float r_pred = (float)before, r_end = (float)(before + ch[c].sum);
  const unsigned pb = __float_as_uint(r_pred), eb = __float_as_uint(r_end);
  const int re = (pb >> 23) & 0xFF;
  const bool plausible = (pb >> 31) == 0 && re >= PFXM_RE_MIN && re <= PFXM_RE_MAX && (int)((eb >> 23) & 0xFF) == re && (eb >> 31) == 0;
  if (!plausible) {
    if (threadIdx.x == 0) { ch[c].re = -1; ch[c].d0 = 0u; ch[c].d1 = 0u; }
    return;
  }
  typename A::value_t xv[K];
  a.load_items(lo, cnt, threadIdx.x * K, xv);
  PfxPair mine = {0u, 0u};
  bool anybad = false;
#pragma unroll
  for (int k = 0; k < K; k++) {
    unsigned f; bool tie, bad;
    A::classify(xv[k], (unsigned)re, f, tie, bad);
    anybad |= bad;
    mine = pfx_compose(mine, pfx_element_pair(f, tie));
  }
  if (anybad) s_bad = 1;
  PfxPair total;
  (void)pfx_pair_scan<NT>(mine, shp, total);
  if (threadIdx.x == 0) {
    const bool ok = s_bad == 0 && total.a0 < (1u << 24) && total.a1 < (1u << 24);
    ch[c].re = ok ? re : -1;
    ch[c].d0 = total.a0;
    ch[c].d1 = total.a1;
  }
}
#define PFXW_BLOCK 512
template <bool FILL, class CH, class SLOW>
__device__ __forceinline__ void chain_walk_chunks(CH* __restrict__ ch, int nch, int c_first, float& r, float& carry, SLOW slow) {
  __shared__ int sm_re[PFXW_BLOCK];
  __shared__ unsigned sm_d0[PFXW_BLOCK], sm_d1[PFXW_BLOCK];
  __shared__ int sm_acc[FILL ? PFXW_BLOCK : 1];
  __shared__ float sm_r0[FILL ? PFXW_BLOCK : 1], sm_c0[FILL ? PFXW_BLOCK : 1];
  for (int cb = 0; cb < nch; cb += PFXW_BLOCK) {
    pfx_sync();
    for (int t = threadIdx.x; t < PFXW_BLOCK && cb + t < nch; t += PFXW_THREADS) {
      const PfxChunk x = ch[cb + t];
      sm_re[t] = x.re; sm_d0[t] = x.d0; sm_d1[t] = x.d1;
      if constexpr (FILL) sm_acc[t] = 0;
    }
    pfx_sync();
    const int ce = min(nch, cb + PFXW_BLOCK);
    for (int c = max(cb, c_first); c < ce; c++) {
      const unsigned rb = __float_as_uint(r);
      const int re = (int)(rb >> 23);
      const unsigned R = (rb & 0x7FFFFFu) | 0x800000u;
      const unsigned D = (R & 1u) ? sm_d1[c - cb] : sm_d0[c - cb];
      if (c > 0 && sm_re[c - cb] == re && R + D < (1u << 24)) {
        if constexpr (FILL) { sm_r0[c - cb] = r; sm_c0[c - cb] = carry; sm_acc[c - cb] = 1; }
        r = chain_mant((unsigned)re, R + D);
        carry = fmaxf(carry, r);
      } else {
        slow(c);
      }
#ifdef TDR_PFX_TIMING
      if constexpr (FILL)
        if (threadIdx.x == 0) *reinterpret_cast<long long*>(&ch[c].sum) = (long long)wall_clock64();
#endif
    }
    if constexpr (FILL) {
      pfx_sync();
      for (int t = threadIdx.x; t < PFXW_BLOCK && cb + t < nch; t += PFXW_THREADS) {
        PfxChunk* o = ch + cb + t;
        o->r0 = sm_r0[t];
        o->carry0 = sm_c0[t];
        o->accepted = sm_acc[t];
      }
    }
  }
}

__global__ __launch_bounds__(PFXM_THREADS) void pfx_chunk_sum_kernel(const float* __restrict__ w, int64_t n,
                                                                     PfxChunk* __restrict__ ch) {
  chain_sum_body<PFXM_THREADS, PFXM_K>(PfxRunSum{{w}, CHAIN_RUNSUM, 0.f}, n, ch);
}
__global__ __launch_bounds__(PFXM_THREADS) void pfx_chunk_summary_kernel(const float* __restrict__ w, int64_t n,
                                                                         PfxChunk* __restrict__ ch, int c_first) {
  chain_summary_body<PFXM_THREADS, PFXM_K>(PfxRunSum{{w}, CHAIN_RUNSUM, 0.f}, n, ch, c_first);
}
__device__ __forceinline__ void pfx_walk_chunk(const float* __restrict__ w, long long lo, int cnt,
                                               float* __restrict__ runmax, float* __restrict__ prefix_opt,
                                               float& r, float& carry, int head_len) {
  __shared__ PfxPair shp[PFXW_THREADS / 64];
  __shared__ ChainWgStop<float> stp;
  const PfxRunSum a{{w}, CHAIN_RUNSUM, 0.f};
  const int t0 = threadIdx.x * PFXW_K;
  float wv[PFXW_K];
  a.load_items(lo, cnt, t0, wv);
  const ChainWg<PFXW_THREADS, float> sc{shp, &stp};
  PfxGlobalSink sink{w, lo, runmax, prefix_opt, carry, head_len};
  r = chain_walk(a, wv, t0, 0, cnt, r, sc, sink);
}
__global__ __launch_bounds__(PFXW_THREADS) void pfx_walk_kernel(const float* __restrict__ w, int64_t n,
                                                               PfxChunk* __restrict__ ch, int nch,
                                                               float* __restrict__ runmax,
                                                               float* __restrict__ prefix_opt, int head_len,
                                                               int c_first, const float* __restrict__ tail) {
  float r = c_first > 0 ? tail[0] : 0.f, carry = c_first > 0 ? tail[1] : -INFINITY;
  chain_walk_chunks<true>(ch, nch, c_first, r, carry, [&](int c) {
    const long long lo = (long long)c * PFXM_CHUNK;
    const int cnt = (int)min((long long)PFXM_CHUNK, (long long)n - lo);
    pfx_walk_chunk(w, lo, cnt, runmax, prefix_opt, r, carry, head_len);
  });
}
__global__ __launch_bounds__(PFXM_THREADS) void pfx_chunk_fill_kernel(const float* __restrict__ w, int64_t n,
                                                                      const PfxChunk* __restrict__ ch,
                                                                      float* __restrict__ runmax,
                                                                      float* __restrict__ prefix_opt) {
  __shared__ PfxPair shp[PFXM_THREADS / 64];
  const int c = blockIdx.x;
  const PfxChunk hdr = ch[c];
  if (!hdr.accepted) return;
  const long long lo = (long long)c * PFXM_CHUNK;
  const int cnt = (int)min((long long)PFXM_CHUNK, (long long)n - lo);
  const PfxRunSum a{{w}, CHAIN_RUNSUM, 0.f};
  const int t0 = threadIdx.x * PFXM_K;
  float wv[PFXM_K];
  a.load_items(lo, cnt, t0, wv);
  const ChainWg<PFXM_THREADS, float> sc{shp, nullptr};
  unsigned st[PFXM_K];
  (void)chain_step<false, PfxRunSum>(wv, t0, 0, cnt, hdr.r0, sc, st);
  float val[PFXM_K];
#pragma unroll
  for (int k = 0; k < PFXM_K; k++) val[k] = chain_mant(__float_as_uint(hdr.r0) >> 23, st[k]);
  const float carry = hdr.carry0;
  if (t0 + PFXM_K <= cnt && ((lo & 3) == 0)) {
    float4* o = reinterpret_cast<float4*>(runmax + lo + t0);
#pragma unroll
    for (int k = 0; k < PFXM_K / 4; k++)
      o[k] = make_float4(fmaxf(carry, val[4 * k]), fmaxf(carry, val[4 * k + 1]), fmaxf(carry, val[4 * k + 2]),
                         fmaxf(carry, val[4 * k + 3]));
    if (prefix_opt) {
      float4* q = reinterpret_cast<float4*>(prefix_opt + lo + t0);
#pragma unroll
      for (int k = 0; k < PFXM_K / 4; k++) q[k] = make_float4(val[4 * k], val[4 * k + 1], val[4 * k + 2], val[4 * k + 3]);
    }
  } else {
#pragma unroll
    for (int k = 0; k < PFXM_K; k++)
      if (t0 + k < cnt) {
        runmax[lo + t0 + k] = fmaxf(carry, val[k]);
        if (prefix_opt) prefix_opt[lo + t0 + k] = val[k];
      }
  }
}

struct ChainSrc {
  const float* raw;
  const float* mean;
  int kind;
};
__device__ __forceinline__ ChainStat chain_stat(const ChainSrc& s) { return {{s.raw}, s.kind, s.kind ? *s.mean : 0.f}; }
__global__ __launch_bounds__(PFXW_THREADS) void chain_sum_kernel(ChainSrc s, int64_t n, PfxChunk* __restrict__ ch) {
  chain_sum_body<PFXW_THREADS, CHAIN_K>(chain_stat(s), n, ch);
}
__global__ __launch_bounds__(PFXW_THREADS) void chain_summary_kernel(ChainSrc s, int64_t n, PfxChunk* __restrict__ ch,
                                                                    int c_first) {
  chain_summary_body<PFXW_THREADS, CHAIN_K>(chain_stat(s), n, ch, c_first);
}
template <class A>
__device__ __forceinline__ void chain_walk_chunk(const A& a, long long lo, int cnt, float& r, int pos) {
  __shared__ PfxPair shp[PFXW_THREADS / 64];
  __shared__ ChainWgStop<double> stp;
  const int t0 = threadIdx.x * CHAIN_K;
  double xv[CHAIN_K];
  a.load_items(lo, cnt, t0, xv);
  const ChainWg<PFXW_THREADS, double> sc{shp, &stp};
  ChainNoSink sink;
  r = chain_walk(a, xv, t0, pos, cnt, r, sc, sink);
}
__global__ __launch_bounds__(PFXW_THREADS) void chain_walk_kernel(ChainSrc s, int64_t n, const PfxChunk* __restrict__ ch,
                                                                 int nch, float* __restrict__ total_out, int c_first,
                                                                 const float* __restrict__ r_first) {
  const ChainStat a = chain_stat(s);
  const int hn = c_first > 0 ? 0 : (int)min((long long)CHAIN_HEAD, (long long)n);
  float r = chain_head_serial<PFXW_THREADS>(a, hn, c_first > 0 ? *r_first : 0.f), carry = 0.f;
  chain_walk_chunks<false>(ch, nch, c_first, r, carry, [&](int c) {
    const long long lo = (long long)c * PFXM_CHUNK;
    chain_walk_chunk(a, lo, (int)min((long long)PFXM_CHUNK, (long long)n - lo), r, c == 0 ? hn : 0);
  });
  if (threadIdx.x == 0) *total_out = r;
}
#define CHAIN_HEAD_N 32768
static int chain_head_chunks(int64_t n) { return (tdr_cfg().pfx_small && n >= CHAIN_HEAD_N) ? CHAIN_HEAD_N / PFXM_CHUNK : 0; }
static int chain_head_launch(const float* raw, const float* mean_dev, int kind, int n_head, float* r_out, int64_t n,
                             PfxChunk* ch, int nch, hipStream_t st);
int tdr_chain_total(const float* raw, const float* mean_dev, int kind, int64_t n, float* total_out, void* workspace,
                    bool have_sums, hipStream_t st) {
  const int64_t nch64 = cdiv(n, (int64_t)PFXM_CHUNK);
  if (nch64 > (1 << 24)) return fail(TDR_ERR_ARG, "chain_total: n too large");
  const int nch = (int)nch64;
  PfxChunk* ch = reinterpret_cast<PfxChunk*>(workspace);
  ChainSrc s{raw, mean_dev, kind};
  const int c_first = chain_head_chunks(n);
  if (!have_sums) hipLaunchKernelGGL(chain_sum_kernel, dim3(nch), dim3(PFXW_THREADS), 0, st, s, n, ch);
  float* r_first = reinterpret_cast<float*>(&ch[0].r0);
  if (c_first > 0) {
    const int rc = chain_head_launch(raw, mean_dev, kind, c_first * PFXM_CHUNK, r_first, n, ch, nch, st);
    if (rc) return rc;
  } else if (nch > c_first) {
    hipLaunchKernelGGL(chain_summary_kernel, dim3(nch - c_first), dim3(PFXW_THREADS), 0, st, s, n, ch, c_first);
  }
  hipLaunchKernelGGL(chain_walk_kernel, dim3(1), dim3(PFXW_THREADS), 0, st, s, n, (const PfxChunk*)ch, nch, total_out,
                     c_first, (const float*)r_first);
  return TDR_OK;
}

template <int NT>
__device__ __forceinline__ int uw_wg_sum_int(int v, int* sh) {
#pragma unroll
  for (int o = 32; o >= 1; o >>= 1) v += __shfl_xor(v, o, 64);
  pfx_sync();
  if ((threadIdx.x & 63) == 0) sh[threadIdx.x >> 6] = v;
  pfx_sync();
  int t = 0;
  for (int k = 0; k < NT / 64; k++) t += sh[k];
  return t;
}
template <bool BELOW>
__device__ __forceinline__ int uw_chunk_count(const float* __restrict__ raw, int64_t n, float mean, int* sh) {
  const long long lo = (long long)blockIdx.x * PFXM_CHUNK;
  const int cnt = (int)min((long long)PFXM_CHUNK, (long long)n - lo);
  const ChainAddend<float, ChainGlobal, CHAIN_BOUND_22> plain{{raw}, CHAIN_RUNSUM, 0.f};
  float v[CHAIN_K];
  const int t0 = threadIdx.x * CHAIN_K;
  plain.load_items(lo, cnt, t0, v);
  int c = 0;
#pragma unroll
  for (int k = 0; k < CHAIN_K; k++) c += (t0 + k < cnt && v[k] == v[k] && (!BELOW || v[k] < mean)) ? 1 : 0;
  return uw_wg_sum_int<PFXW_THREADS>(c, sh);
}
__global__ __launch_bounds__(PFXW_THREADS) void uw_chunk_pass1_kernel(const float* __restrict__ raw, int64_t n,
                                                                     PfxChunk* __restrict__ ch, int* __restrict__ cnt_valid) {
  __shared__ int shc[PFXW_THREADS / 64];
  const int c = uw_chunk_count<false>(raw, n, 0.f, shc);
  if (threadIdx.x == 0) cnt_valid[blockIdx.x] = c;
  chain_sum_body<PFXW_THREADS, CHAIN_K>(ChainStat{{raw}, CHAIN_SUM, 0.f}, n, ch);
}
__global__ __launch_bounds__(PFXW_THREADS) void uw_chunk_pass2_kernel(const float* __restrict__ raw, int64_t n,
                                                                     UwExact* __restrict__ ex,
                                                                     const int* __restrict__ cnt_valid,
                                                                     PfxChunk* __restrict__ ch, int* __restrict__ cnt_under) {
  __shared__ int shc[PFXW_THREADS / 64];
  __shared__ long long shv[PFXW_THREADS / 64];
  long long nv = 0;
  for (int j = threadIdx.x; j < (int)gridDim.x; j += PFXW_THREADS) nv += cnt_valid[j];
#pragma unroll
  for (int o = 32; o >= 1; o >>= 1) nv += __shfl_xor(nv, o, 64);
  if ((threadIdx.x & 63) == 0) shv[threadIdx.x >> 6] = nv;
  pfx_sync();
  nv = 0;
  for (int k = 0; k < PFXW_THREADS / 64; k++) nv += shv[k];
  const float mean = ex->sum / (float)nv;
  const int c = uw_chunk_count<true>(raw, n, mean, shc);
  if (threadIdx.x == 0) {
    cnt_under[blockIdx.x] = c;
    if (blockIdx.x == 0) ex->mean = mean;
  }
  chain_sum_body<PFXW_THREADS, CHAIN_K>(ChainStat{{raw}, CHAIN_BOTTOM, mean}, n, ch);
}
int tdr_uw_chunk_pass1(const float* raw, int64_t n, void* workspace, int* cnt_valid, hipStream_t st) {
  hipLaunchKernelGGL(uw_chunk_pass1_kernel, dim3((unsigned)cdiv(n, (int64_t)PFXM_CHUNK)), dim3(PFXW_THREADS), 0, st, raw, n,
                     reinterpret_cast<PfxChunk*>(workspace), cnt_valid);
  return TDR_OK;
}
int tdr_uw_chunk_pass2(const float* raw, int64_t n, UwExact* ex, const int* cnt_valid, void* workspace, int* cnt_under,
                       hipStream_t st) {
  hipLaunchKernelGGL(uw_chunk_pass2_kernel, dim3((unsigned)cdiv(n, (int64_t)PFXM_CHUNK)), dim3(PFXW_THREADS), 0, st, raw, n,
                     ex, cnt_valid, reinterpret_cast<PfxChunk*>(workspace), cnt_under);
  return TDR_OK;
}

__device__ __forceinline__ float uws_chain_total(int kind, int n, float mean) {
  const UwsWgAdd a{{}, kind, mean};
  const int hn = min(CHAIN_HEAD, n);
  float r = chain_head_serial<PFXW_THREADS>(a, hn, 0.f);
  UW_STAMP(kind ? 5 : 2);
  const int nch = (n + PFXM_CHUNK - 1) / PFXM_CHUNK;
  for (int c = 0; c < nch; c++) {
    const int lo = c * PFXM_CHUNK;
    const int cnt = min((int)PFXM_CHUNK, n - lo);
    if (c == 0 && hn >= cnt) continue;
    chain_walk_chunk(a, lo, cnt, r, c == 0 ? hn : 0);
  }
  return r;
}
#define UWS_THREADS 1024
#define UWS_DUAL_SLOTS 8
#define UWS_DUAL_FLAG 0x100
struct UwsShared {
  double csum[64];
  int code[64];
  unsigned d0[64], d1[64];
  uint4 dual[UWS_DUAL_SLOTS][64];
  double shd[UWS_THREADS / 64];
  float total;
};
template <class A>
__device__ __forceinline__ float uws_wave_walk(const A& a, int lo, int cnt, float r, int pos) {
  const auto ad = a.as_double();
  const int t0 = (threadIdx.x & 63) * CHAIN_K;
  double xv[CHAIN_K];
  ad.load_items(lo, cnt, t0, xv);
  ChainNoSink sink;
  return chain_walk(ad, xv, t0, pos, cnt, r, ChainWave<false>{}, sink);
}
template <class A>
__device__ __forceinline__ float uws_wave_dual(const A& a, int lo, int cnt, float r, const uint4* pq, int& pos) {
  const int lane = threadIdx.x & 63, t0 = lane * CHAIN_K;
  const unsigned rb = __float_as_uint(r), re = rb >> 23, R = (rb & 0x7FFFFFu) | 0x800000u;
  const uint4 v = pq[lane];
  const unsigned after = R + ((R & 1u) ? v.y : v.x);
  const unsigned long long cross = __ballot(after >= (1u << 24));
  pos = cnt;
  if (cross == 0ull) return chain_mant(re, (unsigned)__builtin_amdgcn_readlane((int)after, 63));
  const int L = __ffsll((long long)cross) - 1;
  float rl = chain_mant(re, L > 0 ? (unsigned)__builtin_amdgcn_readlane((int)after, L - 1) : R);
  typename A::value_t x[CHAIN_K];
  a.load_items(lo, cnt, t0, x);
#pragma unroll
  for (int k = 0; k < CHAIN_K; k++) rl = chain_add(rl, x[k]);
  const float r2 = __uint_as_float((unsigned)__builtin_amdgcn_readlane((int)__float_as_uint(rl), L));
  const unsigned rb2 = __float_as_uint(r2), R2 = (rb2 & 0x7FFFFFu) | 0x800000u;
  const int next = (L + 1) * CHAIN_K;
  if (next >= cnt) return r2;
  pos = next;
  if ((rb2 >> 23) != re + 1u) return r2;
  const unsigned qL = (unsigned)__builtin_amdgcn_readlane((int)v.z, L);
  if (qL != (unsigned)__builtin_amdgcn_readlane((int)v.w, L)) return r2;
  const unsigned q63 = (unsigned)__builtin_amdgcn_readlane((int)(((R2 + qL) & 1u) ? v.w : v.z), 63);
  if (q63 >= PFXM_SAT || R2 + (q63 - qL) >= (1u << 24)) return r2;
  pos = cnt;
  return chain_mant(re + 1u, R2 + (q63 - qL));
}
template <class A>
__device__ __forceinline__ float uws_chain_total_waves(const A& a, int n, UwsShared& sh, float* rin = nullptr) {
  const int kind = a.kind;
  constexpr int NW = UWS_THREADS / 64;
  const int lane = threadIdx.x & 63, wave = __builtin_amdgcn_readfirstlane(threadIdx.x >> 6), t0 = lane * CHAIN_K;
  const int nwc = (n + UWS_WC - 1) / UWS_WC;
  float r = 0.f;
  if (wave == 0) {
    r = kind == CHAIN_RUNSUM ? chain_head_lanes<true>(a, min(UWS_WC, n)) : chain_head_lanes<false>(a, min(UWS_WC, n));
  } else {
    int my_code;
    {
      const double own = lane < nwc ? sh.csum[lane] : 0.0;
      const double after = uws_wave_scan_d(own), before = after - own;
      const int re_b = (int)(__float_as_uint((float)before) >> 23), re_a = (int)(__float_as_uint((float)after) >> 23);
      const bool inr = lane >= 1 && lane < nwc && re_b >= PFXM_RE_MIN && re_a <= PFXM_RE_MAX;
      const bool dualc = inr && re_a == re_b + 1;
      const unsigned long long dm = __ballot(dualc);
      const int slot = __popcll(dm & ((1ull << lane) - 1ull));
      my_code = (inr && re_a == re_b) ? re_b : (dualc && slot < UWS_DUAL_SLOTS) ? (re_b | UWS_DUAL_FLAG | (slot << 16)) : -1;
    }
    for (int c = wave; c < nwc; c += NW - 1) {
      const int code = __builtin_amdgcn_readlane(my_code, c);
      const int lo = c * UWS_WC, cnt = min(UWS_WC, n - lo);
      PfxPair P = {0u, 0u}, Q = {0u, 0u};
      bool anybad = false;
      if (code >= 0) {
        const unsigned re = (unsigned)(code & 0xFF);
        const bool dual = (code & UWS_DUAL_FLAG) != 0;
        typename A::value_t x[CHAIN_K];
        a.load_items(lo, cnt, t0, x);
        bool anytie = false;
        unsigned f; bool tie, bad;
#pragma unroll
        for (int k = 0; k < CHAIN_K; k++) {
          A::classify(x[k], re, f, tie, bad);
          anybad |= bad; anytie |= tie;
          P.a0 += f;
        }
        if (dual) {
#pragma unroll
          for (int k = 0; k < CHAIN_K; k++) {
            A::classify(x[k], re + 1u, f, tie, bad);
            anybad |= bad; anytie |= tie;
            Q.a0 += f;
          }
        }
        if (__ballot(anytie) == 0ull) {
          P.a0 = P.a1 = uws_wave_scan_u(P.a0);
          if (dual) Q.a0 = Q.a1 = uws_wave_scan_u(Q.a0);
        } else {
          unsigned re_t = re;
          asm volatile("" : "+s"(re_t));
          P = PfxPair{0u, 0u}; Q = PfxPair{0u, 0u};
#pragma unroll
          for (int k = 0; k < CHAIN_K; k++) {
            A::classify(x[k], re_t, f, tie, bad);
            P = pfx_compose(P, pfx_element_pair(f, tie));
          }
          P = pfx_pair_wave_scan(P);
          if (dual) {
#pragma unroll
            for (int k = 0; k < CHAIN_K; k++) {
              A::classify(x[k], re_t + 1u, f, tie, bad);
              Q = pfx_compose(Q, pfx_element_pair(f, tie));
            }
            Q = pfx_pair_wave_scan(Q);
          }
        }
        if (dual) sh.dual[code >> 16][lane] = make_uint4(P.a0, P.a1, Q.a0, Q.a1);
      }
      const bool ok = code >= 0 && __ballot(anybad) == 0ull;
      if (lane == 63) {
        sh.code[c] = (ok && ((code & UWS_DUAL_FLAG) || (P.a0 < (1u << 24) && P.a1 < (1u << 24)))) ? code : -1;
        sh.d0[c] = P.a0; sh.d1[c] = P.a1;
      }
    }
  }
  pfx_sync();
  UW_STAMP(kind ? 5 : 2);
  if (wave == 0) {
    const int v_code = (lane >= 1 && lane < nwc) ? sh.code[lane] : -1;
    const unsigned v_d0 = (lane >= 1 && lane < nwc) ? sh.d0[lane] : 0u, v_d1 = (lane >= 1 && lane < nwc) ? sh.d1[lane] : 0u;
    float v_rin = 0.f;
    int c = 1;
    while (c < nwc) {
      const unsigned rb = __float_as_uint(r);
      const int re = (int)(rb >> 23);
      const unsigned R = (rb & 0x7FFFFFu) | 0x800000u;
      bool overflow = false;
      const unsigned long long other = ~__ballot(lane < nwc && v_code == re) & (~0ull << c);
      const int cend = other ? __ffsll((long long)other) - 1 : 64;
      if (cend > c) {
        const bool in_run = lane >= c && lane < cend;
        unsigned after;
        if (__ballot(in_run && v_d0 != v_d1) == 0ull) {
          after = R + uws_wave_scan_u(in_run ? v_d0 : 0u);
        } else {
          const PfxPair in = pfx_pair_wave_scan(in_run ? PfxPair{v_d0, v_d1} : PfxPair{0u, 0u});
          after = R + ((R & 1u) ? in.a1 : in.a0);
        }
        const unsigned long long cross = __ballot(in_run && after >= (1u << 24));
        const int c1 = cross ? __ffsll((long long)cross) - 1 : cend;
        if (kind == CHAIN_RUNSUM) {
          const unsigned prev = (unsigned)__builtin_amdgcn_update_dpp(0, (int)after, 0x138, 0xF, 0xF, false);
          if (lane >= c && lane < c1) v_rin = lane == c ? r : chain_mant((unsigned)re, prev);
        }
        if (c1 > c) r = chain_mant((unsigned)re, (unsigned)__builtin_amdgcn_readlane((int)after, c1 - 1));
#ifdef TDR_UW_TIMELINE
        if (threadIdx.x == 0) g_uw_tl[12] += c1 - c;
#endif
        c = c1;
        if (c1 == cend) continue;
        overflow = true;
      }
      const int lo = c * UWS_WC, cnt = min(UWS_WC, n - lo);
      const int code = __builtin_amdgcn_readlane(v_code, c);
      if (kind == CHAIN_RUNSUM) v_rin = (lane == c) ? r : v_rin;
      int pos = 0;
      const int re_now = (int)(__float_as_uint(r) >> 23);
      if (!overflow && code >= 0 && re_now <= PFXM_RE_MAX && (code & 0x1FF) == (re_now | UWS_DUAL_FLAG)) {
        r = uws_wave_dual(a, lo, cnt, r, sh.dual[code >> 16], pos);
        UW_COUNT(13);
      }
      if (pos < cnt) {
        UW_COUNT(14);
        r = uws_wave_walk(a, lo, cnt, r, pos);
      }
      c++;
    }
    if (kind == CHAIN_RUNSUM) rin[lane] = v_rin;
    if (lane == 0) sh.total = r;
  }
  pfx_sync();
  return sh.total;
}
template <int NT>
__device__ __forceinline__ double uws_sum_d(double v, double* sh) {
  v = uws_wave_scan_d(v);
  pfx_sync();
  if ((threadIdx.x & 63) == 63) sh[threadIdx.x >> 6] = v;
  pfx_sync();
  double t = 0;
  for (int w = 0; w < NT / 64; w++) t += sh[w];
  return t;
}
template <bool WAVES>
__device__ __forceinline__ void uw_small_body(const float* __restrict__ raw, const float* __restrict__ last_dist, int n,
                                              float* __restrict__ w, float* __restrict__ info) {
  extern __shared__ float uws_lraw[];
  float* const lraw = uws_lraw;
  constexpr int nt = WAVES ? UWS_THREADS : PFXW_THREADS;
  __shared__ UwsShared ush;
  double* const shd = ush.shd;
  __shared__ float sh_best[nt / 64];
  __shared__ int sh_besti[nt / 64];
  const int tid = threadIdx.x;
#ifdef TDR_UW_TIMELINE
  if (tid == 0) { for (int k = 10; k < 16; k++) g_uw_tl[k] = 0; }
#endif
  UW_STAMP(0);
  float sum = 0.f, mean = 0.f, bsum = 0.f;
  long long num_valid = 0, num_under = 0;
  double valid_sum = 0.0;
  if constexpr (WAVES) {
    const int lane = tid & 63, nwc = (n + UWS_WC - 1) / UWS_WC;
#pragma unroll
    for (int kind = 0; kind < 2; kind++) {
      int cnt = 0;
      for (int c = tid >> 6; c < nwc; c += nt / 64) {
        const int base = c * UWS_WC + lane;
        float v[CHAIN_K];
        if (kind == 0) {
#pragma unroll
          for (int m = 0; m < CHAIN_K; m++) v[m] = base + 64 * m < n ? raw[base + 64 * m] : __uint_as_float(0x7FC00000u);
#pragma unroll
          for (int m = 0; m < CHAIN_K; m++)
            if (base + 64 * m < n) lraw[uws_idx(base + 64 * m)] = v[m];
        } else {
#pragma unroll
          for (int m = 0; m < CHAIN_K; m++) {
            const float x = lraw[uws_idx(min(base + 64 * m, n - 1))];
            v[m] = base + 64 * m < n ? x : __uint_as_float(0x7FC00000u);
          }
        }
        double acc = 0;
#pragma unroll
        for (int m = 0; m < CHAIN_K; m++) {
          const bool take = kind == 0 ? v[m] == v[m] : (v[m] == v[m] && v[m] < mean);
          double x = (double)(kind == 0 ? v[m] : v[m] - mean);
          if (kind) x = x * x;
          cnt += take ? 1 : 0;
          acc += take ? x : 0.0;
        }
        acc = uws_wave_scan_d(acc);
        if (lane == 63) ush.csum[c] = acc;
      }
      const long long count = (long long)uws_sum_d<nt>((double)cnt, shd);
      if (kind == 0) valid_sum = uws_readlane_d(uws_wave_scan_d(lane < nwc ? ush.csum[lane] : 0.0), 63);
      UW_STAMP(kind ? 4 : 1);
      const float total = kind == 0 ? uws_chain_total_waves(UwsAddF{{}, CHAIN_SUM, 0.f}, n, ush)
                                    : uws_chain_total_waves(UwsAddD{{}, CHAIN_BOTTOM, mean}, n, ush);
      UW_STAMP(kind ? 6 : 3);
      if (kind == 0) {
        sum = total; num_valid = count;
        mean = sum / (float)num_valid;
      } else {
        bsum = total; num_under = count;
      }
    }
  } else {
    double cnt = 0;
    int i = tid;
    for (; i + 3 * nt < n; i += 4 * nt) {
      const float v0 = raw[i], v1 = raw[i + nt], v2 = raw[i + 2 * nt], v3 = raw[i + 3 * nt];
      lraw[uws_idx(i)] = v0; lraw[uws_idx(i + nt)] = v1; lraw[uws_idx(i + 2 * nt)] = v2; lraw[uws_idx(i + 3 * nt)] = v3;
      cnt += (v0 == v0 ? 1.0 : 0.0) + (v1 == v1 ? 1.0 : 0.0) + (v2 == v2 ? 1.0 : 0.0) + (v3 == v3 ? 1.0 : 0.0);
    }
    for (; i < n; i += nt) {
      const float v = raw[i];
      lraw[uws_idx(i)] = v;
      cnt += (v == v) ? 1.0 : 0.0;
    }
    num_valid = (long long)uws_sum_d<nt>(cnt, shd);
    UW_STAMP(1);
    sum = uws_chain_total(CHAIN_SUM, n, 0.f);
    UW_STAMP(3);
    mean = sum / (float)num_valid;
    double cu = 0;
    for (int i = tid; i < n; i += nt) {
      const float v = lraw[uws_idx(i)];
      cu += (v == v && v < mean) ? 1.0 : 0.0;
    }
    num_under = (long long)uws_sum_d<nt>(cu, shd);
    UW_STAMP(4);
    bsum = uws_chain_total(CHAIN_BOTTOM, n, mean);
    UW_STAMP(6);
  }
  const float bottom = sqrtf(bsum / (float)num_under);
  const bool fallback = (sum == 0.f || num_under < 1);
  const float fill = mean - bottom;
  const float fn = (float)n;
  float fs1;
  double s2 = 0;
  if constexpr (WAVES) {
    const double fill_sum = num_valid == n ? 0.0 : (double)(n - num_valid) * (double)fill;
    fs1 = (float)(fallback ? (double)n : valid_sum + fill_sum);
    UW_STAMP(7);
    for (int i0 = tid; i0 < n; i0 += 16 * nt) {
      float ld[16];
#pragma unroll
      for (int j = 0; j < 16; j++) ld[j] = i0 + j * nt < n ? last_dist[i0 + j * nt] : 0.f;
#pragma unroll
      for (int j = 0; j < 16; j++) {
        const int i = i0 + j * nt;
        if (i < n) {
          float v = lraw[uws_idx(i)];
          v = (fallback ? 1.f : (v != v ? fill : v)) / fs1;
          const float d = fminf(ld[j] * 5.f, 1.f);
          v = d * v + (1.f - d) / fn;
          lraw[uws_idx(i)] = v;
          s2 += (double)v;
        }
      }
    }
  } else {
    pfx_sync();
    double s1a = 0;
    for (int i = tid; i < n; i += nt) {
      float v = lraw[uws_idx(i)];
      v = fallback ? 1.f : (v != v ? fill : v);
      lraw[uws_idx(i)] = v;
      s1a += (double)v;
    }
    fs1 = (float)uws_sum_d<nt>(s1a, shd);
    UW_STAMP(7);
    auto one = [&](int i, float ld) {
      float v = lraw[uws_idx(i)] / fs1;
      const float d = fminf(ld * 5.f, 1.f);
      v = d * v + (1.f - d) / fn;
      lraw[uws_idx(i)] = v;
      s2 += (double)v;
    };
    int i = tid;
    for (; i + 3 * nt < n; i += 4 * nt) {
      const float l0 = last_dist[i], l1 = last_dist[i + nt], l2 = last_dist[i + 2 * nt], l3 = last_dist[i + 3 * nt];
      one(i, l0); one(i + nt, l1); one(i + 2 * nt, l2); one(i + 3 * nt, l3);
    }
    for (; i < n; i += nt) one(i, last_dist[i]);
  }
  const float fs2 = (float)uws_sum_d<nt>(s2, shd);
  UW_STAMP(8);
  float best = -INFINITY;
  int besti = 0x7fffffff;
  for (int i = tid; i < n; i += nt) {
    const float v = lraw[uws_idx(i)] / fs2;
    w[i] = v;
    if (v > best || (v == best && i < besti)) { best = v; besti = i; }
  }
  for (int o = 32; o > 0; o >>= 1) {
    const float ob = __shfl_down(best, o, 64);
    const int oi = __shfl_down(besti, o, 64);
    if (ob > best || (ob == best && oi < besti)) { best = ob; besti = oi; }
  }
  pfx_sync();
  if ((tid & 63) == 0) { sh_best[tid >> 6] = best; sh_besti[tid >> 6] = besti; }
  pfx_sync();
  if (tid == 0) {
    for (int k = 1; k < nt / 64; k++)
      if (sh_best[k] > best || (sh_best[k] == best && sh_besti[k] < besti)) { best = sh_best[k]; besti = sh_besti[k]; }
    if (besti == 0x7fffffff) besti = 0;
    info[0] = __int_as_float(besti);
    info[1] = sum; info[2] = mean; info[3] = bottom; info[4] = fallback ? 1.f : 0.f;
    info[5] = (float)num_valid; info[6] = (float)num_under; info[7] = 0.f;
  }
  UW_STAMP(9);
}
template <bool WAVES>
__global__ __launch_bounds__(WAVES ? UWS_THREADS : PFXW_THREADS) void uw_small_kernel(const float* __restrict__ raw,
                                                                const float* __restrict__ last_dist, int n,
                                                                float* __restrict__ w, float* __restrict__ info) {
  uw_small_body<WAVES>(raw, last_dist, n, w, info);
}
template <bool WAVES>
__global__ __launch_bounds__(WAVES ? UWS_THREADS : PFXW_THREADS) void uw_small_batch_kernel(const TdrBatchEntry* __restrict__ tab) {
  const TdrBatchEntry& e = tab[blockIdx.x];
  uw_small_body<WAVES>(e.raw_w, e.last_dist, (int)e.n, e.w_out, e.info_out);
}
int tdr_uw_small(const float* raw, const float* last_dist, int64_t n, float* w, float* info, hipStream_t st) {
  if (n < 1 || n > 32768) return fail(TDR_ERR_ARG, "uw_small: n out of range");
  const size_t lds = ((size_t)n + (size_t)(n >> 5) + 1 + UWS_PAD) * sizeof(float);
  static bool attr_set[64] = {false};
  int dev = 0;
  if (hipGetDevice(&dev) != hipSuccess || dev < 0) dev = 0;
  if (dev >= 64 || !attr_set[dev]) {
    if (hipFuncSetAttribute(reinterpret_cast<const void*>(uw_small_kernel<false>),
                            hipFuncAttributeMaxDynamicSharedMemorySize, 133 * 1024) != hipSuccess ||
        hipFuncSetAttribute(reinterpret_cast<const void*>(uw_small_kernel<true>),
                            hipFuncAttributeMaxDynamicSharedMemorySize, 133 * 1024) != hipSuccess)
      return fail(TDR_ERR_HIP, "uw_small: cannot raise the dynamic LDS limit");
    if (dev < 64) attr_set[dev] = true;
  }
  if (tdr_cfg().uw_waves)
    hipLaunchKernelGGL(uw_small_kernel<true>, dim3(1), dim3(UWS_THREADS), lds, st, raw, last_dist, (int)n, w, info);
  else
    hipLaunchKernelGGL(uw_small_kernel<false>, dim3(1), dim3(PFXW_THREADS), lds, st, raw, last_dist, (int)n, w, info);
  return TDR_OK;
}

struct PfsShared {
  UwsShared u;
  float rin[64];
  float cmax[64];
  int irregular;
};
__device__ __forceinline__ void pfs_wave_fill(int lo, int cnt, float r) {
  extern __shared__ float uws_lraw[];
  const UwsAddF a{{}, CHAIN_RUNSUM, 0.f};
  const int t0 = (threadIdx.x & 63) * CHAIN_K;
  float x[CHAIN_K];
  a.load_items(lo, cnt, t0, x);
  ChainRegSink<CHAIN_K> sink;
#pragma unroll
  for (int k = 0; k < CHAIN_K; k++) sink.pv[k] = 0.f;
  (void)chain_walk(a, x, t0, 0, cnt, r, ChainWave<true>{}, sink);
#pragma unroll
  for (int k = 0; k < CHAIN_K; k++)
    if (t0 + k < cnt) uws_lraw[uws_idx(lo + t0 + k)] = sink.pv[k];
}
__device__ __forceinline__ void pfx_small_body(const float* __restrict__ w, int n, float* __restrict__ runmax,
                                               float* __restrict__ prefix_opt,
                                               float* __restrict__ tail) {
  extern __shared__ float uws_lraw[];
  float* const lraw = uws_lraw;
  __shared__ PfsShared sh;
  constexpr int nt = UWS_THREADS, NW = UWS_THREADS / 64;
  const int tid = threadIdx.x, lane = tid & 63, wave = __builtin_amdgcn_readfirstlane(tid >> 6);
  const int nwc = (n + UWS_WC - 1) / UWS_WC;
  if (tid == 0) sh.irregular = 0;
  pfx_sync();
  bool irr = false;
  for (int c = wave; c < nwc; c += NW) {
    const int base = c * UWS_WC + lane;
    float v[CHAIN_K];
#pragma unroll
    for (int m = 0; m < CHAIN_K; m++) v[m] = base + 64 * m < n ? w[base + 64 * m] : 0.f;
    double acc = 0;
#pragma unroll
    for (int m = 0; m < CHAIN_K; m++) {
      if (base + 64 * m < n) lraw[uws_idx(base + 64 * m)] = v[m];
      irr |= !(v[m] >= 0.f);
      acc += (double)v[m];
    }
    acc = uws_wave_scan_d(acc);
    if (lane == 63) sh.u.csum[c] = acc;
  }
  if (__ballot(irr) != 0ull && lane == 0) atomicOr(&sh.irregular, 1);
  pfx_sync();
  const float total = uws_chain_total_waves(UwsAddF{{}, CHAIN_RUNSUM, 0.f}, n, sh.u, sh.rin);
  for (int c = 1 + wave; c < nwc; c += NW) pfs_wave_fill(c * UWS_WC, min(UWS_WC, n - c * UWS_WC), sh.rin[c]);
  pfx_sync();
  if (sh.irregular == 0) {
    if (tail && tid == 0) { tail[0] = total; tail[1] = total; }
    for (int i = tid; i < n; i += nt) {
      const float v = lraw[uws_idx(i)];
      runmax[i] = v;
      if (prefix_opt) prefix_opt[i] = v;
    }
    return;
  }
  const int t0 = lane * CHAIN_K;
  for (int c = wave; c < nwc; c += NW) {
    const int lo = c * UWS_WC, cnt = min(UWS_WC, n - lo);
    float m = -INFINITY;
#pragma unroll
    for (int k = 0; k < CHAIN_K; k++) {
      const float v = lraw[uws_idx(lo + t0 + k)];
      if (t0 + k < cnt && v == v) m = fmaxf(m, v);
    }
    m = pfs_wave_scan_max(m);
    if (lane == 63) sh.cmax[c] = m;
  }
  pfx_sync();
  const float before = pfs_wave_scan_max(lane < nwc ? sh.cmax[lane] : -INFINITY);
  if (tail && tid == 63) { tail[0] = total; tail[1] = before; }
  for (int c = wave; c < nwc; c += NW) {
    const int lo = c * UWS_WC, cnt = min(UWS_WC, n - lo);
    const float carry = c > 0 ? __uint_as_float((unsigned)__builtin_amdgcn_readlane((int)__float_as_uint(before), c - 1)) : -INFINITY;
    float pv[CHAIN_K], lm[CHAIN_K];
    float m = -INFINITY;
#pragma unroll
    for (int k = 0; k < CHAIN_K; k++) {
      pv[k] = lraw[uws_idx(lo + t0 + k)];
      if (t0 + k < cnt && pv[k] == pv[k]) m = fmaxf(m, pv[k]);
      lm[k] = m;
    }
    const float incl = pfs_wave_scan_max(m);
    float ex = __uint_as_float((unsigned)__builtin_amdgcn_update_dpp((int)0xFF800000u, (int)__float_as_uint(incl), 0x138, 0xF, 0xF, false));
    ex = fmaxf(ex, carry);
#pragma unroll
    for (int k = 0; k < CHAIN_K; k++)
      if (t0 + k < cnt) {
        runmax[lo + t0 + k] = fmaxf(lm[k], ex);
        if (prefix_opt) prefix_opt[lo + t0 + k] = pv[k];
      }
  }
}
static_assert(PFXM_THREADS % 64 == 0 && PFXW_THREADS % 64 == 0 && PFXM_THREADS <= UWS_THREADS && PFXW_THREADS <= UWS_THREADS,
              "summary blocks: whole waves of the head's workgroup");
__global__ __launch_bounds__(UWS_THREADS) void pfx_small_kernel(const float* __restrict__ w, int n,
                                                                float* __restrict__ runmax, float* __restrict__ prefix_opt,
                                                                float* __restrict__ tail, int64_t n_all,
                                                                PfxChunk* __restrict__ ch, int c_first) {
  if (blockIdx.x > 0) {
    if (threadIdx.x < PFXM_THREADS)
      chain_summary_body<PFXM_THREADS, PFXM_K>(PfxRunSum{{w}, CHAIN_RUNSUM, 0.f}, n_all, ch, c_first - 1);
    return;
  }
  pfx_small_body(w, n, runmax, prefix_opt, tail);
}
__global__ __launch_bounds__(UWS_THREADS) void pfx_small_batch_kernel(const TdrBatchEntry* __restrict__ tab) {
  const TdrBatchEntry& e = tab[blockIdx.x];
  pfx_small_body(e.w_out, (int)e.n, e.runmax_out, nullptr, nullptr);
}
#define TDR_PFX_SMALL_MAX_N 32768
static int pfx_small(const float* w, int64_t n, float* runmax, float* prefix_opt, hipStream_t st, float* tail = nullptr,
                     int64_t n_all = 0, PfxChunk* ch = nullptr, int nch = 0) {
  if (n < 1 || n > TDR_PFX_SMALL_MAX_N) return fail(TDR_ERR_ARG, "pfx_small: n out of range");
  const size_t lds = ((size_t)n + (size_t)(n >> 5) + 1 + UWS_PAD) * sizeof(float);
  static bool attr_set[64] = {false};
  int dev = 0;
  if (hipGetDevice(&dev) != hipSuccess || dev < 0) dev = 0;
  if (dev >= 64 || !attr_set[dev]) {
    if (hipFuncSetAttribute(reinterpret_cast<const void*>(pfx_small_kernel), hipFuncAttributeMaxDynamicSharedMemorySize,
                            133 * 1024) != hipSuccess)
      return fail(TDR_ERR_HIP, "pfx_small: cannot raise the dynamic LDS limit");
    if (dev < 64) attr_set[dev] = true;
  }
  const int c_first = ch ? (int)(n / PFXM_CHUNK) : 0;
  hipLaunchKernelGGL(pfx_small_kernel, dim3(1 + (ch ? (unsigned)std::max(0, nch - c_first) : 0u)), dim3(UWS_THREADS), lds,
                     st, w, (int)n, runmax, prefix_opt, tail, n_all, ch, c_first);
  return TDR_OK;
}

template <int KIND>
__global__ __launch_bounds__(UWS_THREADS) void chain_head_kernel(const float* __restrict__ raw, const float* __restrict__ mean_dev,
                                                                 int n, float* __restrict__ r_out, int64_t n_all,
                                                                 PfxChunk* __restrict__ ch, int c_first) {
  const float mean = KIND ? *mean_dev : 0.f;
  if (blockIdx.x > 0) {
    if (threadIdx.x < PFXW_THREADS)
      chain_summary_body<PFXW_THREADS, CHAIN_K>(ChainStat{{raw}, KIND, mean}, n_all, ch, c_first - 1);
    return;
  }
  extern __shared__ float uws_lraw[];
  __shared__ UwsShared ush;
  const int tid = threadIdx.x, lane = tid & 63, nwc = (n + UWS_WC - 1) / UWS_WC;
  for (int c = tid >> 6; c < nwc; c += UWS_THREADS / 64) {
    const int base = c * UWS_WC + lane;
    float v[CHAIN_K];
#pragma unroll
    for (int m = 0; m < CHAIN_K; m++) v[m] = base + 64 * m < n ? raw[base + 64 * m] : __uint_as_float(0x7FC00000u);
    double acc = 0;
#pragma unroll
    for (int m = 0; m < CHAIN_K; m++) {
      if (base + 64 * m < n) uws_lraw[uws_idx(base + 64 * m)] = v[m];
      const bool take = KIND == 0 ? v[m] == v[m] : (v[m] == v[m] && v[m] < mean);
      double x = (double)(KIND == 0 ? v[m] : v[m] - mean);
      if (KIND) x = x * x;
      acc += take ? x : 0.0;
    }
    acc = uws_wave_scan_d(acc);
    if (lane == 63) ush.csum[c] = acc;
  }
  pfx_sync();
  float r;
  if constexpr (KIND == CHAIN_SUM) r = uws_chain_total_waves(UwsAddF{{}, CHAIN_SUM, 0.f}, n, ush);
  else r = uws_chain_total_waves(UwsAddD{{}, CHAIN_BOTTOM, mean}, n, ush);
  if (tid == 0) *r_out = r;
}
static int chain_head_launch(const float* raw, const float* mean_dev, int kind, int n_head, float* r_out, int64_t n,
                             PfxChunk* ch, int nch, hipStream_t st) {
  const size_t lds = ((size_t)n_head + (size_t)(n_head >> 5) + 1 + UWS_PAD) * sizeof(float);
  static bool attr_set[64] = {false};
  int dev = 0;
  if (hipGetDevice(&dev) != hipSuccess || dev < 0) dev = 0;
  if (dev >= 64 || !attr_set[dev]) {
    if (hipFuncSetAttribute(reinterpret_cast<const void*>(chain_head_kernel<0>), hipFuncAttributeMaxDynamicSharedMemorySize,
                            133 * 1024) != hipSuccess ||
        hipFuncSetAttribute(reinterpret_cast<const void*>(chain_head_kernel<1>), hipFuncAttributeMaxDynamicSharedMemorySize,
                            133 * 1024) != hipSuccess)
      return fail(TDR_ERR_HIP, "chain_head: cannot raise the dynamic LDS limit");
    if (dev < 64) attr_set[dev] = true;
  }
  const int c_first = n_head / PFXM_CHUNK;
  const dim3 grid(1 + (unsigned)std::max(0, nch - c_first));
  if (kind == 0)
    hipLaunchKernelGGL(chain_head_kernel<0>, grid, dim3(UWS_THREADS), lds, st, raw, mean_dev, n_head, r_out, n, ch, c_first);
  else
    hipLaunchKernelGGL(chain_head_kernel<1>, grid, dim3(UWS_THREADS), lds, st, raw, mean_dev, n_head, r_out, n, ch, c_first);
  return TDR_OK;
}

#define TDR_PFX_MULTI_MIN_N 6144
#define TDR_PFX_EXACT_MIN_N 24576
#define TDR_PFX_SMALL_MIN_N 256
extern "C" int64_t tdr_prefix_workspace_bytes(int64_t n) {
  return n < 1 ? 0 : (int64_t)sizeof(PfxChunk) * cdiv(n, (int64_t)PFXM_CHUNK);
}
static int prefix_multi(const float* w, int64_t n, float* runmax_out, float* prefix_out, void* workspace,
                        hipStream_t st) {
  const int64_t nch64 = cdiv(n, (int64_t)PFXM_CHUNK);
  if (nch64 > (1 << 24)) return fail(TDR_ERR_ARG, "prefix: n too large");
  const int nch = (int)nch64;
  PfxChunk* ch = reinterpret_cast<PfxChunk*>(workspace);
  const int c_first = chain_head_chunks(n);
  float* tail = reinterpret_cast<float*>(&ch[0].r0);
  static_assert(offsetof(PfxChunk, carry0) == offsetof(PfxChunk, r0) + sizeof(float), "tail: sum, maximum");
  hipLaunchKernelGGL(pfx_chunk_sum_kernel, dim3(nch), dim3(PFXM_THREADS), 0, st, w, n, ch);
  if (c_first > 0) {
    const int rc = pfx_small(w, (int64_t)c_first * PFXM_CHUNK, runmax_out, prefix_out, st, tail, n, ch, nch);
    if (rc) return rc;
  } else if (nch > c_first) {
    hipLaunchKernelGGL(pfx_chunk_summary_kernel, dim3(nch - c_first), dim3(PFXM_THREADS), 0, st, w, n, ch, c_first);
  }
  const int head_len = tdr_cfg().pfx_head;
  hipLaunchKernelGGL(pfx_walk_kernel, dim3(1), dim3(PFXW_THREADS), 0, st, w, n, ch, nch, runmax_out, prefix_out,
                     head_len, c_first, (const float*)tail);
  hipLaunchKernelGGL(pfx_chunk_fill_kernel, dim3(nch), dim3(PFXM_THREADS), 0, st, w, n, (const PfxChunk*)ch,
                     runmax_out, prefix_out);
  return TDR_OK;
}
extern "C" int tdr_k_prefix(const float* w, int64_t n, float* runmax_out, void* workspace, void* stream) {
  if (!w || !runmax_out || n < 1) return fail(TDR_ERR_ARG, "prefix: bad arguments");
  if (tdr_cfg().pfx_small && n >= TDR_PFX_SMALL_MIN_N && n <= TDR_PFX_SMALL_MAX_N) {
    const int rc = pfx_small(w, n, runmax_out, nullptr, (hipStream_t)stream);
    if (rc) return rc;
  } else if (workspace && n >= TDR_PFX_MULTI_MIN_N) {
    const int rc = prefix_multi(w, n, runmax_out, nullptr, workspace, (hipStream_t)stream);
    if (rc) return rc;
  } else if (n < TDR_PFX_EXACT_MIN_N)
    hipLaunchKernelGGL(prefix_serial_kernel, dim3(1), dim3(64), 0, (hipStream_t)stream, w, n, runmax_out);
  else
    hipLaunchKernelGGL(prefix_exact_kernel, dim3(1), dim3(PFX_THREADS), 0, (hipStream_t)stream, w, n, runmax_out,
                       (float*)nullptr);
  LAUNCH_CHECK("prefix");
  return TDR_OK;
}
extern "C" int tdr_k_prefix_mode(const float* w, int64_t n, int mode, float* runmax_out, float* prefix_out,
                                 void* workspace, void* stream) {
  if (!w || !runmax_out || n < 1) return fail(TDR_ERR_ARG, "prefix_mode: bad arguments");
  if (mode == 2 && !workspace) return fail(TDR_ERR_ARG, "prefix_mode: mode 2 needs a workspace");
  if (mode == 3) {
    const int rc = pfx_small(w, n, runmax_out, prefix_out, (hipStream_t)stream);
    if (rc) return rc;
  } else if (mode == 0)
    hipLaunchKernelGGL(prefix_serial_kernel, dim3(1), dim3(64), 0, (hipStream_t)stream, w, n, runmax_out);
  else if (mode == 2) {
    const int rc = prefix_multi(w, n, runmax_out, prefix_out, workspace, (hipStream_t)stream);
    if (rc) return rc;
  } else
    hipLaunchKernelGGL(prefix_exact_kernel, dim3(1), dim3(PFX_THREADS), 0, (hipStream_t)stream, w, n, runmax_out,
                       prefix_out);
  LAUNCH_CHECK("prefix_mode");
  return TDR_OK;
}

static int batch_lds_attr(const void* fn) {
  return hipFuncSetAttribute(fn, hipFuncAttributeMaxDynamicSharedMemorySize, 133 * 1024) == hipSuccess ? TDR_OK
         : fail(TDR_ERR_HIP, "batch: cannot raise the dynamic LDS limit");
}
int tdr_batch_update_weights(const TdrBatchEntry* tab, int k, int64_t n_max, hipStream_t st) {
  if (!tab || k < 1 || n_max < 1 || n_max > 32768) return fail(TDR_ERR_ARG, "batch_update_weights: bad arguments");
  const size_t lds = ((size_t)n_max + (size_t)(n_max >> 5) + 1 + UWS_PAD) * sizeof(float);
  if (tdr_cfg().uw_waves) {
    if (int rc = batch_lds_attr(reinterpret_cast<const void*>(uw_small_batch_kernel<true>))) return rc;
    hipLaunchKernelGGL(uw_small_batch_kernel<true>, dim3((unsigned)k), dim3(UWS_THREADS), lds, st, tab);
  } else {
    if (int rc = batch_lds_attr(reinterpret_cast<const void*>(uw_small_batch_kernel<false>))) return rc;
    hipLaunchKernelGGL(uw_small_batch_kernel<false>, dim3((unsigned)k), dim3(PFXW_THREADS), lds, st, tab);
  }
  LAUNCH_CHECK("batch_update_weights");
  return TDR_OK;
}
int tdr_batch_prefix(const TdrBatchEntry* tab, int k, int64_t n_max, hipStream_t st) {
  if (!tab || k < 1 || n_max < 1 || n_max > TDR_PFX_SMALL_MAX_N) return fail(TDR_ERR_ARG, "batch_prefix: bad arguments");
  const size_t lds = ((size_t)n_max + (size_t)(n_max >> 5) + 1 + UWS_PAD) * sizeof(float);
  if (int rc = batch_lds_attr(reinterpret_cast<const void*>(pfx_small_batch_kernel))) return rc;
  hipLaunchKernelGGL(pfx_small_batch_kernel, dim3((unsigned)k), dim3(UWS_THREADS), lds, st, tab);
  LAUNCH_CHECK("batch_prefix");
  return TDR_OK;
}
```

Before: 25.09 million.

## Replace single-block chain head with grid-wide wave-chunk summary and walk for large n

```diff
diff --git a/top_down_renderer_amd/csrc/tdr_common.h b/top_down_renderer_amd/csrc/tdr_common.h
--- a/top_down_renderer_amd/csrc/tdr_common.h
+++ b/top_down_renderer_amd/csrc/tdr_common.h
@@ -66,13 +66,15 @@
 #define INI_TILE 2048
 #define INI_MAX_TILES 2048
 int tdr_chain_total(const float* raw, const float* mean_dev, int kind, int64_t n, float* total_out, void* workspace,
-                    bool have_sums, hipStream_t st);
+                    bool have_sums, bool grid, hipStream_t st);
+int64_t tdr_chain_workspace_bytes(int64_t n, bool grid);
+bool tdr_chain_grid(int64_t n);
 struct UwExact {
   float sum, mean, bsum, pad;
 };
-int tdr_uw_chunk_pass1(const float* raw, int64_t n, void* workspace, int* cnt_valid, hipStream_t st);
-int tdr_uw_chunk_pass2(const float* raw, int64_t n, UwExact* ex, const int* cnt_valid, void* workspace, int* cnt_under,
-                       hipStream_t st);
+int tdr_uw_chunk_pass1(const float* raw, int64_t n, void* workspace, bool grid, int* cnt_valid, hipStream_t st);
+int tdr_uw_chunk_pass2(const float* raw, int64_t n, UwExact* ex, const int* cnt_valid, void* workspace, bool grid,
+                       int* cnt_under, hipStream_t st);
 int tdr_uw_small(const float* raw, const float* last_dist, int64_t n, float* w, float* info, hipStream_t st);
 int tdr_mt_raw_stream(const uint32_t* state, int64_t nblocks, uint32_t* raw, hipStream_t s);
 int tdr_mt_advance(const uint32_t* raw, int64_t nblocks, const uint32_t* consumed, uint32_t* state, hipStream_t s);
diff --git a/top_down_renderer_amd/csrc/tdr_filter.hip b/top_down_renderer_amd/csrc/tdr_filter.hip
--- a/top_down_renderer_amd/csrc/tdr_filter.hip
+++ b/top_down_renderer_amd/csrc/tdr_filter.hip
@@ -309,18 +309,21 @@
   UwExact* ex = reinterpret_cast<UwExact*>(sc + 3);
   void* chain_ws = reinterpret_cast<void*>((reinterpret_cast<uintptr_t>(ex + 1) + 63) & ~(uintptr_t)63);
   const size_t chain_room = TDR_UW_INFO_FLOATS * sizeof(float) - kFixed;
-  const int64_t nch = tdr_prefix_workspace_bytes(n) / 32;
-  if ((size_t)tdr_prefix_workspace_bytes(n) + (size_t)nch * 2 * sizeof(int) > chain_room)
+  const int64_t nch = tdr_chain_workspace_bytes(n, false) / 32;
+  const size_t counts = (size_t)nch * 2 * sizeof(int);
+  const bool grid = tdr_chain_grid(n) && (size_t)tdr_chain_workspace_bytes(n, true) + counts <= chain_room;
+  const size_t ws_bytes = (size_t)tdr_chain_workspace_bytes(n, grid);
+  if (ws_bytes + counts > chain_room)
     return fail(TDR_ERR_ARG, "update_weights: n = %lld needs more than TDR_UW_INFO_FLOATS of scratch", (long long)n);
-  int* cnt_valid = reinterpret_cast<int*>(reinterpret_cast<char*>(chain_ws) + tdr_prefix_workspace_bytes(n));
+  int* cnt_valid = reinterpret_cast<int*>(reinterpret_cast<char*>(chain_ws) + ws_bytes);
   int* cnt_under = cnt_valid + nch;
-  int rc = tdr_uw_chunk_pass1(raw_w, n, chain_ws, cnt_valid, s);
+  int rc = tdr_uw_chunk_pass1(raw_w, n, chain_ws, grid, cnt_valid, s);
   if (rc) return rc;
-  rc = tdr_chain_total(raw_w, nullptr, 0, n, &ex->sum, chain_ws, true, s);
+  rc = tdr_chain_total(raw_w, nullptr, 0, n, &ex->sum, chain_ws, true, grid, s);
   if (rc) return rc;
-  rc = tdr_uw_chunk_pass2(raw_w, n, ex, cnt_valid, chain_ws, cnt_under, s);
+  rc = tdr_uw_chunk_pass2(raw_w, n, ex, cnt_valid, chain_ws, grid, cnt_under, s);
   if (rc) return rc;
-  rc = tdr_chain_total(raw_w, &ex->mean, 1, n, &ex->bsum, chain_ws, true, s);
+  rc = tdr_chain_total(raw_w, &ex->mean, 1, n, &ex->bsum, chain_ws, true, grid, s);
   if (rc) return rc;
   hipLaunchKernelGGL(uw_pass3, dim3(UW_G), dim3(256), 0, s, raw_w, n, (const UwExact*)ex, (const int*)cnt_under, (int)nch,
                      sc + 0, w_out);
diff --git a/top_down_renderer_amd/csrc/tdr_prefix.hip b/top_down_renderer_amd/csrc/tdr_prefix.hip
--- a/top_down_renderer_amd/csrc/tdr_prefix.hip
+++ b/top_down_renderer_amd/csrc/tdr_prefix.hip
@@ -395,6 +395,25 @@
   int accepted;
 };
 static_assert(sizeof(PfxChunk) == 32, "PfxChunk");
+struct WcRec {
+  double sum;
+  int code;
+  unsigned d0, d1;
+  float rin;
+};
+struct WcCtl {
+  int slots;
+  int irregular;
+  int pad[2];
+};
+#define UWG_DUAL_SLOTS 32
+struct ChainGridWs {
+  PfxChunk* ch;
+  WcRec* wc;
+  int* irr;
+  WcCtl* ctl;
+  uint4* dual;
+};
 #ifndef PFXW_THREADS
 #define PFXW_THREADS 512
 #endif
@@ -838,10 +857,9 @@
   return r;
 }
 
-template <bool KEEP, class A>
-__device__ __forceinline__ float chain_head_lanes(const A& a, int hn) {
+template <bool KEEP, class A, class PUT>
+__device__ __forceinline__ float chain_head_lanes(const A& a, int hn, PUT keep) {
   using X = typename A::value_t;
-  extern __shared__ float uws_lraw[];
   const int lane = threadIdx.x & 63;
   float run = 0.f;
   X nxt = a.load(min(lane, hn - 1), lane < hn);
@@ -854,9 +872,14 @@
       run = chain_add(run, chain_readlane(cur, j));
       if (KEEP) mine = (lane == j) ? run : mine;
     }
-    if (KEEP && b + lane < hn) uws_lraw[uws_idx(b + lane)] = mine;
+    if (KEEP && b + lane < hn) keep(b + lane, mine);
   }
   return run;
+}
+template <bool KEEP, class A>
+__device__ __forceinline__ float chain_head_lanes(const A& a, int hn) {
+  extern __shared__ float uws_lraw[];
+  return chain_head_lanes<KEEP>(a, hn, [](int i, float v) { uws_lraw[uws_idx(i)] = v; });
 }
 #ifndef CHAIN_HEAD
 #define CHAIN_HEAD 1024
@@ -881,9 +904,11 @@
   return s_head_r;
 }
 
-template <int NT, int K, class A>
-__device__ __forceinline__ void chain_sum_body(const A& a, int64_t n, PfxChunk* __restrict__ ch) {
+template <int NT, int K, bool FLAGS = false, class A>
+__device__ __forceinline__ void chain_sum_body(const A& a, int64_t n, const ChainGridWs& ws) {
+  static_assert(K == CHAIN_K && NT * K == PFXM_CHUNK, "one wave, one wave-chunk");
   __shared__ double shd[NT / 64];
+  __shared__ int shi[FLAGS ? NT / 64 : 1];
   const long long lo = (long long)blockIdx.x * PFXM_CHUNK;
   const int cnt = (int)min((long long)PFXM_CHUNK, (long long)n - lo);
   typename A::value_t xv[K];
@@ -891,15 +916,33 @@
   double acc = 0.0;
 #pragma unroll
   for (int k = 0; k < K; k++) acc += (double)xv[k];
+  if constexpr (FLAGS) {
+    bool irr = false;
+#pragma unroll
+    for (int k = 0; k < K; k++) irr |= !(xv[k] >= 0);
+    const bool any = __ballot(irr) != 0ull;
+    if ((threadIdx.x & 63) == 0) shi[threadIdx.x >> 6] = any ? 1 : 0;
+  }
   const double t = chain_wg_sum<NT>(acc, shd);
-  if (threadIdx.x == 0) ch[blockIdx.x].sum = t;
+  if (threadIdx.x == 0) ws.ch[blockIdx.x].sum = t;
+  if (ws.wc) {
+    if constexpr (FLAGS) {
+      if (threadIdx.x == 0) {
+        int f = 0;
+        for (int k = 0; k < NT / 64; k++) f |= shi[k];
+        ws.irr[blockIdx.x] = f;
+      }
+    }
+    if (threadIdx.x < NT / 64 && threadIdx.x * UWS_WC < cnt) ws.wc[blockIdx.x * (NT / 64) + threadIdx.x].sum = shd[threadIdx.x];
+    if (blockIdx.x == 0 && threadIdx.x == 0) ws.ctl->slots = 0;
+  }
 }
 template <int NT, int K, class A>
-__device__ __forceinline__ void chain_summary_body(const A& a, int64_t n, PfxChunk* __restrict__ ch, int c_first) {
+__device__ __forceinline__ void chain_summary_body(const A& a, int64_t n, PfxChunk* __restrict__ ch) {
   __shared__ double shd[NT / 64];
   __shared__ PfxPair shp[NT / 64];
   __shared__ int s_bad;
-  const int c = blockIdx.x + c_first;
+  const int c = blockIdx.x;
   const long long lo = (long long)c * PFXM_CHUNK;
   const int cnt = (int)min((long long)PFXM_CHUNK, (long long)n - lo);
   double acc = 0.0;
@@ -937,7 +980,7 @@
 }
 #define PFXW_BLOCK 512
 template <bool FILL, class CH, class SLOW>
-__device__ __forceinline__ void chain_walk_chunks(CH* __restrict__ ch, int nch, int c_first, float& r, float& carry, SLOW slow) {
+__device__ __forceinline__ void chain_walk_chunks(CH* __restrict__ ch, int nch, float& r, float& carry, SLOW slow) {
   __shared__ int sm_re[PFXW_BLOCK];
   __shared__ unsigned sm_d0[PFXW_BLOCK], sm_d1[PFXW_BLOCK];
   __shared__ int sm_acc[FILL ? PFXW_BLOCK : 1];
@@ -951,7 +994,7 @@
     }
     pfx_sync();
     const int ce = min(nch, cb + PFXW_BLOCK);
-    for (int c = max(cb, c_first); c < ce; c++) {
+    for (int c = cb; c < ce; c++) {
       const unsigned rb = __float_as_uint(r);
       const int re = (int)(rb >> 23);
       const unsigned R = (rb & 0x7FFFFFu) | 0x800000u;
@@ -980,13 +1023,12 @@
   }
 }
 
-__global__ __launch_bounds__(PFXM_THREADS) void pfx_chunk_sum_kernel(const float* __restrict__ w, int64_t n,
-                                                                     PfxChunk* __restrict__ ch) {
-  chain_sum_body<PFXM_THREADS, PFXM_K>(PfxRunSum{{w}, CHAIN_RUNSUM, 0.f}, n, ch);
+__global__ __launch_bounds__(PFXW_THREADS) void pfx_chunk_sum_kernel(const float* __restrict__ w, int64_t n, ChainGridWs ws) {
+  chain_sum_body<PFXW_THREADS, CHAIN_K, true>(ChainAddend<float, ChainGlobal, CHAIN_BOUND_22>{{w}, CHAIN_RUNSUM, 0.f}, n, ws);
 }
 __global__ __launch_bounds__(PFXM_THREADS) void pfx_chunk_summary_kernel(const float* __restrict__ w, int64_t n,
-                                                                         PfxChunk* __restrict__ ch, int c_first) {
-  chain_summary_body<PFXM_THREADS, PFXM_K>(PfxRunSum{{w}, CHAIN_RUNSUM, 0.f}, n, ch, c_first);
+                                                                         PfxChunk* __restrict__ ch) {
+  chain_summary_body<PFXM_THREADS, PFXM_K>(PfxRunSum{{w}, CHAIN_RUNSUM, 0.f}, n, ch);
 }
 __device__ __forceinline__ void pfx_walk_chunk(const float* __restrict__ w, long long lo, int cnt,
                                                float* __restrict__ runmax, float* __restrict__ prefix_opt,
@@ -1001,24 +1043,24 @@
   PfxGlobalSink sink{w, lo, runmax, prefix_opt, carry, head_len};
   r = chain_walk(a, wv, t0, 0, cnt, r, sc, sink);
 }
-__global__ __launch_bounds__(PFXW_THREADS) void pfx_walk_kernel(const float* __restrict__ w, int64_t n,
-                                                               PfxChunk* __restrict__ ch, int nch,
-                                                               float* __restrict__ runmax,
-                                                               float* __restrict__ prefix_opt, int head_len,
-                                                               int c_first, const float* __restrict__ tail) {
-  float r = c_first > 0 ? tail[0] : 0.f, carry = c_first > 0 ? tail[1] : -INFINITY;
-  chain_walk_chunks<true>(ch, nch, c_first, r, carry, [&](int c) {
+__device__ __forceinline__ void pfx_walk_body(const float* __restrict__ w, int64_t n, PfxChunk* __restrict__ ch, int nch,
+                                              float* __restrict__ runmax, float* __restrict__ prefix_opt, int head_len) {
+  float r = 0.f, carry = -INFINITY;
+  chain_walk_chunks<true>(ch, nch, r, carry, [&](int c) {
     const long long lo = (long long)c * PFXM_CHUNK;
     const int cnt = (int)min((long long)PFXM_CHUNK, (long long)n - lo);
     pfx_walk_chunk(w, lo, cnt, runmax, prefix_opt, r, carry, head_len);
   });
 }
-__global__ __launch_bounds__(PFXM_THREADS) void pfx_chunk_fill_kernel(const float* __restrict__ w, int64_t n,
-                                                                      const PfxChunk* __restrict__ ch,
-                                                                      float* __restrict__ runmax,
-                                                                      float* __restrict__ prefix_opt) {
+__global__ __launch_bounds__(PFXW_THREADS) void pfx_walk_kernel(const float* __restrict__ w, int64_t n,
+                                                               PfxChunk* __restrict__ ch, int nch,
+                                                               float* __restrict__ runmax,
+                                                               float* __restrict__ prefix_opt, int head_len) {
+  pfx_walk_body(w, n, ch, nch, runmax, prefix_opt, head_len);
+}
+__device__ __forceinline__ void pfx_chunk_fill_body(const float* __restrict__ w, int64_t n, const PfxChunk* __restrict__ ch,
+                                                    int c, float* __restrict__ runmax, float* __restrict__ prefix_opt) {
   __shared__ PfxPair shp[PFXM_THREADS / 64];
-  const int c = blockIdx.x;
   const PfxChunk hdr = ch[c];
   if (!hdr.accepted) return;
   const long long lo = (long long)c * PFXM_CHUNK;
@@ -1054,6 +1096,12 @@
       }
   }
 }
+__global__ __launch_bounds__(PFXM_THREADS) void pfx_chunk_fill_kernel(const float* __restrict__ w, int64_t n,
+                                                                      const PfxChunk* __restrict__ ch,
+                                                                      float* __restrict__ runmax,
+                                                                      float* __restrict__ prefix_opt) {
+  pfx_chunk_fill_body(w, n, ch, blockIdx.x, runmax, prefix_opt);
+}
 
 struct ChainSrc {
   const float* raw;
@@ -1061,12 +1109,11 @@
   int kind;
 };
 __device__ __forceinline__ ChainStat chain_stat(const ChainSrc& s) { return {{s.raw}, s.kind, s.kind ? *s.mean : 0.f}; }
-__global__ __launch_bounds__(PFXW_THREADS) void chain_sum_kernel(ChainSrc s, int64_t n, PfxChunk* __restrict__ ch) {
-  chain_sum_body<PFXW_THREADS, CHAIN_K>(chain_stat(s), n, ch);
-}
-__global__ __launch_bounds__(PFXW_THREADS) void chain_summary_kernel(ChainSrc s, int64_t n, PfxChunk* __restrict__ ch,
-                                                                    int c_first) {
-  chain_summary_body<PFXW_THREADS, CHAIN_K>(chain_stat(s), n, ch, c_first);
+__global__ __launch_bounds__(PFXW_THREADS) void chain_sum_kernel(ChainSrc s, int64_t n, ChainGridWs ws) {
+  chain_sum_body<PFXW_THREADS, CHAIN_K>(chain_stat(s), n, ws);
+}
+__global__ __launch_bounds__(PFXW_THREADS) void chain_summary_kernel(ChainSrc s, int64_t n, PfxChunk* __restrict__ ch) {
+  chain_summary_body<PFXW_THREADS, CHAIN_K>(chain_stat(s), n, ch);
 }
 template <class A>
 __device__ __forceinline__ void chain_walk_chunk(const A& a, long long lo, int cnt, float& r, int pos) {
@@ -1080,39 +1127,54 @@
   r = chain_walk(a, xv, t0, pos, cnt, r, sc, sink);
 }
 __global__ __launch_bounds__(PFXW_THREADS) void chain_walk_kernel(ChainSrc s, int64_t n, const PfxChunk* __restrict__ ch,
-                                                                 int nch, float* __restrict__ total_out, int c_first,
-                                                                 const float* __restrict__ r_first) {
+                                                                 int nch, float* __restrict__ total_out) {
   const ChainStat a = chain_stat(s);
-  const int hn = c_first > 0 ? 0 : (int)min((long long)CHAIN_HEAD, (long long)n);
-  float r = chain_head_serial<PFXW_THREADS>(a, hn, c_first > 0 ? *r_first : 0.f), carry = 0.f;
-  chain_walk_chunks<false>(ch, nch, c_first, r, carry, [&](int c) {
+  const int hn = (int)min((long long)CHAIN_HEAD, (long long)n);
+  float r = chain_head_serial<PFXW_THREADS>(a, hn, 0.f), carry = 0.f;
+  chain_walk_chunks<false>(ch, nch, r, carry, [&](int c) {
     const long long lo = (long long)c * PFXM_CHUNK;
     chain_walk_chunk(a, lo, (int)min((long long)PFXM_CHUNK, (long long)n - lo), r, c == 0 ? hn : 0);
   });
   if (threadIdx.x == 0) *total_out = r;
 }
-#define CHAIN_HEAD_N 32768
-static int chain_head_chunks(int64_t n) { return (tdr_cfg().pfx_small && n >= CHAIN_HEAD_N) ? CHAIN_HEAD_N / PFXM_CHUNK : 0; }
-static int chain_head_launch(const float* raw, const float* mean_dev, int kind, int n_head, float* r_out, int64_t n,
-                             PfxChunk* ch, int nch, hipStream_t st);
+#define CHAIN_GRID_MIN_N 32769
+int64_t tdr_chain_workspace_bytes(int64_t n, bool grid) {
+  if (n < 1) return 0;
+  const int64_t nch = cdiv(n, (int64_t)PFXM_CHUNK), nwc = cdiv(n, (int64_t)UWS_WC);
+  int64_t b = (int64_t)sizeof(PfxChunk) * nch;
+  if (grid)
+    b += (int64_t)sizeof(WcRec) * nwc + (nwc & 1) * 8 + ((nch * (int64_t)sizeof(int) + 15) & ~(int64_t)15) + (int64_t)sizeof(WcCtl) +
+         (int64_t)UWG_DUAL_SLOTS * 64 * (int64_t)sizeof(uint4);
+  return b;
+}
+static ChainGridWs chain_grid_ws(void* workspace, int64_t n, bool grid) {
+  const int64_t nch = cdiv(n, (int64_t)PFXM_CHUNK), nwc = cdiv(n, (int64_t)UWS_WC);
+  ChainGridWs ws{reinterpret_cast<PfxChunk*>(workspace), nullptr, nullptr, nullptr, nullptr};
+  if (!grid) return ws;
+  char* p = reinterpret_cast<char*>(workspace) + sizeof(PfxChunk) * nch;
+  ws.wc = reinterpret_cast<WcRec*>(p); p += sizeof(WcRec) * nwc + (nwc & 1) * 8;
+  ws.irr = reinterpret_cast<int*>(p); p += (nch * sizeof(int) + 15) & ~(size_t)15;
+  ws.ctl = reinterpret_cast<WcCtl*>(p); p += sizeof(WcCtl);
+  ws.dual = reinterpret_cast<uint4*>(p);
+  return ws;
+}
+bool tdr_chain_grid(int64_t n) { return tdr_cfg().pfx_small && n >= CHAIN_GRID_MIN_N; }
+static void chain_grid_total(const ChainSrc& s, int64_t n, float* total_out, const ChainGridWs& ws, hipStream_t st);
 int tdr_chain_total(const float* raw, const float* mean_dev, int kind, int64_t n, float* total_out, void* workspace,
-                    bool have_sums, hipStream_t st) {
+                    bool have_sums, bool grid, hipStream_t st) {
   const int64_t nch64 = cdiv(n, (int64_t)PFXM_CHUNK);
   if (nch64 > (1 << 24)) return fail(TDR_ERR_ARG, "chain_total: n too large");
+  if (grid && n < CHAIN_GRID_MIN_N) return fail(TDR_ERR_ARG, "chain_total: the wave-chunk path starts at 32 769 addends");
   const int nch = (int)nch64;
-  PfxChunk* ch = reinterpret_cast<PfxChunk*>(workspace);
+  const ChainGridWs ws = chain_grid_ws(workspace, n, grid);
   ChainSrc s{raw, mean_dev, kind};
-  const int c_first = chain_head_chunks(n);
-  if (!have_sums) hipLaunchKernelGGL(chain_sum_kernel, dim3(nch), dim3(PFXW_THREADS), 0, st, s, n, ch);
-  float* r_first = reinterpret_cast<float*>(&ch[0].r0);
-  if (c_first > 0) {
-    const int rc = chain_head_launch(raw, mean_dev, kind, c_first * PFXM_CHUNK, r_first, n, ch, nch, st);
-    if (rc) return rc;
-  } else if (nch > c_first) {
-    hipLaunchKernelGGL(chain_summary_kernel, dim3(nch - c_first), dim3(PFXW_THREADS), 0, st, s, n, ch, c_first);
-  }
-  hipLaunchKernelGGL(chain_walk_kernel, dim3(1), dim3(PFXW_THREADS), 0, st, s, n, (const PfxChunk*)ch, nch, total_out,
-                     c_first, (const float*)r_first);
+  if (!have_sums) hipLaunchKernelGGL(chain_sum_kernel, dim3(nch), dim3(PFXW_THREADS), 0, st, s, n, ws);
+  if (grid) {
+    chain_grid_total(s, n, total_out, ws, st);
+    return TDR_OK;
+  }
+  hipLaunchKernelGGL(chain_summary_kernel, dim3(nch), dim3(PFXW_THREADS), 0, st, s, n, ws.ch);
+  hipLaunchKernelGGL(chain_walk_kernel, dim3(1), dim3(PFXW_THREADS), 0, st, s, n, (const PfxChunk*)ws.ch, nch, total_out);
   return TDR_OK;
 }
 
@@ -1141,16 +1203,16 @@
   return uw_wg_sum_int<PFXW_THREADS>(c, sh);
 }
 __global__ __launch_bounds__(PFXW_THREADS) void uw_chunk_pass1_kernel(const float* __restrict__ raw, int64_t n,
-                                                                     PfxChunk* __restrict__ ch, int* __restrict__ cnt_valid) {
+                                                                     ChainGridWs ws, int* __restrict__ cnt_valid) {
   __shared__ int shc[PFXW_THREADS / 64];
   const int c = uw_chunk_count<false>(raw, n, 0.f, shc);
   if (threadIdx.x == 0) cnt_valid[blockIdx.x] = c;
-  chain_sum_body<PFXW_THREADS, CHAIN_K>(ChainStat{{raw}, CHAIN_SUM, 0.f}, n, ch);
+  chain_sum_body<PFXW_THREADS, CHAIN_K>(ChainStat{{raw}, CHAIN_SUM, 0.f}, n, ws);
 }
 __global__ __launch_bounds__(PFXW_THREADS) void uw_chunk_pass2_kernel(const float* __restrict__ raw, int64_t n,
                                                                      UwExact* __restrict__ ex,
                                                                      const int* __restrict__ cnt_valid,
-                                                                     PfxChunk* __restrict__ ch, int* __restrict__ cnt_under) {
+                                                                     ChainGridWs ws, int* __restrict__ cnt_under) {
   __shared__ int shc[PFXW_THREADS / 64];
   __shared__ long long shv[PFXW_THREADS / 64];
   long long nv = 0;
@@ -1167,17 +1229,17 @@
     cnt_under[blockIdx.x] = c;
     if (blockIdx.x == 0) ex->mean = mean;
   }
-  chain_sum_body<PFXW_THREADS, CHAIN_K>(ChainStat{{raw}, CHAIN_BOTTOM, mean}, n, ch);
-}
-int tdr_uw_chunk_pass1(const float* raw, int64_t n, void* workspace, int* cnt_valid, hipStream_t st) {
+  chain_sum_body<PFXW_THREADS, CHAIN_K>(ChainStat{{raw}, CHAIN_BOTTOM, mean}, n, ws);
+}
+int tdr_uw_chunk_pass1(const float* raw, int64_t n, void* workspace, bool grid, int* cnt_valid, hipStream_t st) {
   hipLaunchKernelGGL(uw_chunk_pass1_kernel, dim3((unsigned)cdiv(n, (int64_t)PFXM_CHUNK)), dim3(PFXW_THREADS), 0, st, raw, n,
-                     reinterpret_cast<PfxChunk*>(workspace), cnt_valid);
+                     chain_grid_ws(workspace, n, grid), cnt_valid);
   return TDR_OK;
 }
-int tdr_uw_chunk_pass2(const float* raw, int64_t n, UwExact* ex, const int* cnt_valid, void* workspace, int* cnt_under,
-                       hipStream_t st) {
+int tdr_uw_chunk_pass2(const float* raw, int64_t n, UwExact* ex, const int* cnt_valid, void* workspace, bool grid,
+                       int* cnt_under, hipStream_t st) {
   hipLaunchKernelGGL(uw_chunk_pass2_kernel, dim3((unsigned)cdiv(n, (int64_t)PFXM_CHUNK)), dim3(PFXW_THREADS), 0, st, raw, n,
-                     ex, cnt_valid, reinterpret_cast<PfxChunk*>(workspace), cnt_under);
+                     ex, cnt_valid, chain_grid_ws(workspace, n, grid), cnt_under);
   return TDR_OK;
 }
 
@@ -1206,8 +1268,8 @@
   double shd[UWS_THREADS / 64];
   float total;
 };
-template <class A>
-__device__ __forceinline__ float uws_wave_walk(const A& a, int lo, int cnt, float r, int pos) {
+template <class A, class I>
+__device__ __forceinline__ float uws_wave_walk(const A& a, I lo, int cnt, float r, int pos) {
   const auto ad = a.as_double();
   const int t0 = (threadIdx.x & 63) * CHAIN_K;
   double xv[CHAIN_K];
@@ -1215,8 +1277,8 @@
   ChainNoSink sink;
   return chain_walk(ad, xv, t0, pos, cnt, r, ChainWave<false>{}, sink);
 }
-template <class A>
-__device__ __forceinline__ float uws_wave_dual(const A& a, int lo, int cnt, float r, const uint4* pq, int& pos) {
+template <class A, class I>
+__device__ __forceinline__ float uws_wave_dual(const A& a, I lo, int cnt, float r, const uint4* pq, int& pos) {
   const int lane = threadIdx.x & 63, t0 = lane * CHAIN_K;
   const unsigned rb = __float_as_uint(r), re = rb >> 23, R = (rb & 0x7FFFFFu) | 0x800000u;
   const uint4 v = pq[lane];
@@ -1243,11 +1305,124 @@
   pos = cnt;
   return chain_mant(re + 1u, R2 + (q63 - qL));
 }
+__device__ __forceinline__ int uws_predict(double before, double after, bool& dualc) {
+  const int re_b = (int)(__float_as_uint((float)before) >> 23), re_a = (int)(__float_as_uint((float)after) >> 23);
+  const bool inr = re_b >= PFXM_RE_MIN && re_a <= PFXM_RE_MAX;
+  dualc = inr && re_a == re_b + 1;
+  return (inr && re_a == re_b) ? re_b : dualc ? (re_b | UWS_DUAL_FLAG) : -1;
+}
+template <class A, class I>
+__device__ __forceinline__ bool uws_wave_summary(const A& a, I lo, int cnt, int code, uint4* dual_out, PfxPair& P) {
+  const int lane = threadIdx.x & 63, t0 = lane * CHAIN_K;
+  PfxPair Q = {0u, 0u};
+  bool anybad = false;
+  const unsigned re = (unsigned)(code & 0xFF);
+  const bool dual = (code & UWS_DUAL_FLAG) != 0;
+  typename A::value_t x[CHAIN_K];
+  a.load_items(lo, cnt, t0, x);
+  bool anytie = false;
+  unsigned f; bool tie, bad;
+#pragma unroll
+  for (int k = 0; k < CHAIN_K; k++) {
+    A::classify(x[k], re, f, tie, bad);
+    anybad |= bad; anytie |= tie;
+    P.a0 += f;
+  }
+  if (dual) {
+#pragma unroll
+    for (int k = 0; k < CHAIN_K; k++) {
+      A::classify(x[k], re + 1u, f, tie, bad);
+      anybad |= bad; anytie |= tie;
+      Q.a0 += f;
+    }
+  }
+  if (__ballot(anytie) == 0ull) {
+    P.a0 = P.a1 = uws_wave_scan_u(P.a0);
+    if (dual) Q.a0 = Q.a1 = uws_wave_scan_u(Q.a0);
+  } else {
+    unsigned re_t = re;
+    asm volatile("" : "+s"(re_t));
+    P = PfxPair{0u, 0u}; Q = PfxPair{0u, 0u};
+#pragma unroll
+    for (int k = 0; k < CHAIN_K; k++) {
+      A::classify(x[k], re_t, f, tie, bad);
+      P = pfx_compose(P, pfx_element_pair(f, tie));
+    }
+    P = pfx_pair_wave_scan(P);
+    if (dual) {
+#pragma unroll
+      for (int k = 0; k < CHAIN_K; k++) {
+        A::classify(x[k], re_t + 1u, f, tie, bad);
+        Q = pfx_compose(Q, pfx_element_pair(f, tie));
+      }
+      Q = pfx_pair_wave_scan(Q);
+    }
+  }
+  if (dual) dual_out[lane] = make_uint4(P.a0, P.a1, Q.a0, Q.a1);
+  return __ballot(anybad) == 0ull;
+}
+__device__ __forceinline__ int uws_summary_code(int code, bool ok, const PfxPair& P) {
+  return (ok && ((code & UWS_DUAL_FLAG) || (P.a0 < (1u << 24) && P.a1 < (1u << 24)))) ? code : -1;
+}
+template <class A, class I, class DUAL>
+__device__ __forceinline__ float uws_walk_summaries(const A& a, I n, int base, int nl, int v_code, unsigned v_d0,
+                                                    unsigned v_d1, DUAL dual_of, float r, float& v_rin) {
+  const int kind = a.kind;
+  const int lane = threadIdx.x & 63;
+  int c = base == 0 ? 1 : 0;
+  while (c < nl) {
+    const unsigned rb = __float_as_uint(r);
+    const int re = (int)(rb >> 23);
+    const unsigned R = (rb & 0x7FFFFFu) | 0x800000u;
+    bool overflow = false;
+    const unsigned long long other = ~__ballot(lane < nl && v_code == re) & (~0ull << c);
+    const int cend = other ? __ffsll((long long)other) - 1 : 64;
+    if (cend > c) {
+      const bool in_run = lane >= c && lane < cend;
+      unsigned after;
+      if (__ballot(in_run && v_d0 != v_d1) == 0ull) {
+        after = R + uws_wave_scan_u(in_run ? v_d0 : 0u);
+      } else {
+        const PfxPair in = pfx_pair_wave_scan(in_run ? PfxPair{v_d0, v_d1} : PfxPair{0u, 0u});
+        after = R + ((R & 1u) ? in.a1 : in.a0);
+      }
+      const unsigned long long cross = __ballot(in_run && after >= (1u << 24));
+      const int c1 = cross ? __ffsll((long long)cross) - 1 : cend;
+      if (kind == CHAIN_RUNSUM) {
+        const unsigned prev = (unsigned)__builtin_amdgcn_update_dpp(0, (int)after, 0x138, 0xF, 0xF, false);
+        if (lane >= c && lane < c1) v_rin = lane == c ? r : chain_mant((unsigned)re, prev);
+      }
+      if (c1 > c) r = chain_mant((unsigned)re, (unsigned)__builtin_amdgcn_readlane((int)after, c1 - 1));
+#ifdef TDR_UW_TIMELINE
+      if (threadIdx.x == 0) g_uw_tl[12] += c1 - c;
+#endif
+      c = c1;
+      if (c1 == cend) continue;
+      overflow = true;
+    }
+    const I lo = (I)(base + c) * UWS_WC;
+    const int cnt = (int)min((I)UWS_WC, n - lo);
+    const int code = __builtin_amdgcn_readlane(v_code, c);
+    if (kind == CHAIN_RUNSUM) v_rin = (lane == c) ? r : v_rin;
+    int pos = 0;
+    const int re_now = (int)(__float_as_uint(r) >> 23);
+    if (!overflow && code >= 0 && re_now <= PFXM_RE_MAX && (code & 0x1FF) == (re_now | UWS_DUAL_FLAG)) {
+      r = uws_wave_dual(a, lo, cnt, r, dual_of(code), pos);
+      UW_COUNT(13);
+    }
+    if (pos < cnt) {
+      UW_COUNT(14);
+      r = uws_wave_walk(a, lo, cnt, r, pos);
+    }
+    c++;
+  }
+  return r;
+}
 template <class A>
 __device__ __forceinline__ float uws_chain_total_waves(const A& a, int n, UwsShared& sh, float* rin = nullptr) {
   const int kind = a.kind;
   constexpr int NW = UWS_THREADS / 64;
-  const int lane = threadIdx.x & 63, wave = __builtin_amdgcn_readfirstlane(threadIdx.x >> 6), t0 = lane * CHAIN_K;
+  const int lane = threadIdx.x & 63, wave = __builtin_amdgcn_readfirstlane(threadIdx.x >> 6);
   const int nwc = (n + UWS_WC - 1) / UWS_WC;
   float r = 0.f;
   if (wave == 0) {
@@ -1257,66 +1432,20 @@
     {
       const double own = lane < nwc ? sh.csum[lane] : 0.0;
       const double after = uws_wave_scan_d(own), before = after - own;
-      const int re_b = (int)(__float_as_uint((float)before) >> 23), re_a = (int)(__float_as_uint((float)after) >> 23);
-      const bool inr = lane >= 1 && lane < nwc && re_b >= PFXM_RE_MIN && re_a <= PFXM_RE_MAX;
-      const bool dualc = inr && re_a == re_b + 1;
-      const unsigned long long dm = __ballot(dualc);
+      bool dualc;
+      const int pred = uws_predict(before, after, dualc);
+      const bool have = lane >= 1 && lane < nwc;
+      const unsigned long long dm = __ballot(have && dualc);
       const int slot = __popcll(dm & ((1ull << lane) - 1ull));
-      my_code = (inr && re_a == re_b) ? re_b : (dualc && slot < UWS_DUAL_SLOTS) ? (re_b | UWS_DUAL_FLAG | (slot << 16)) : -1;
+      my_code = !have ? -1 : !dualc ? pred : slot < UWS_DUAL_SLOTS ? (pred | (slot << 16)) : -1;
     }
     for (int c = wave; c < nwc; c += NW - 1) {
       const int code = __builtin_amdgcn_readlane(my_code, c);
       const int lo = c * UWS_WC, cnt = min(UWS_WC, n - lo);
-      PfxPair P = {0u, 0u}, Q = {0u, 0u};
-      bool anybad = false;
-      if (code >= 0) {
-        const unsigned re = (unsigned)(code & 0xFF);
-        const bool dual = (code & UWS_DUAL_FLAG) != 0;
-        typename A::value_t x[CHAIN_K];
-        a.load_items(lo, cnt, t0, x);
-        bool anytie = false;
-        unsigned f; bool tie, bad;
-#pragma unroll
-        for (int k = 0; k < CHAIN_K; k++) {
-          A::classify(x[k], re, f, tie, bad);
-          anybad |= bad; anytie |= tie;
-          P.a0 += f;
-        }
-        if (dual) {
-#pragma unroll
-          for (int k = 0; k < CHAIN_K; k++) {
-            A::classify(x[k], re + 1u, f, tie, bad);
-            anybad |= bad; anytie |= tie;
-            Q.a0 += f;
-          }
-        }
-        if (__ballot(anytie) == 0ull) {
-          P.a0 = P.a1 = uws_wave_scan_u(P.a0);
-          if (dual) Q.a0 = Q.a1 = uws_wave_scan_u(Q.a0);
-        } else {
-          unsigned re_t = re;
-          asm volatile("" : "+s"(re_t));
-          P = PfxPair{0u, 0u}; Q = PfxPair{0u, 0u};
-#pragma unroll
-          for (int k = 0; k < CHAIN_K; k++) {
-            A::classify(x[k], re_t, f, tie, bad);
-            P = pfx_compose(P, pfx_element_pair(f, tie));
-          }
-          P = pfx_pair_wave_scan(P);
-          if (dual) {
-#pragma unroll
-            for (int k = 0; k < CHAIN_K; k++) {
-              A::classify(x[k], re_t + 1u, f, tie, bad);
-              Q = pfx_compose(Q, pfx_element_pair(f, tie));
-            }
-            Q = pfx_pair_wave_scan(Q);
-          }
-        }
-        if (dual) sh.dual[code >> 16][lane] = make_uint4(P.a0, P.a1, Q.a0, Q.a1);
-      }
-      const bool ok = code >= 0 && __ballot(anybad) == 0ull;
+      PfxPair P = {0u, 0u};
+      const bool ok = code >= 0 && uws_wave_summary(a, lo, cnt, code, sh.dual[(code >> 16) & (UWS_DUAL_SLOTS - 1)], P);
       if (lane == 63) {
-        sh.code[c] = (ok && ((code & UWS_DUAL_FLAG) || (P.a0 < (1u << 24) && P.a1 < (1u << 24)))) ? code : -1;
+        sh.code[c] = uws_summary_code(code, ok, P);
         sh.d0[c] = P.a0; sh.d1[c] = P.a1;
       }
     }
@@ -1324,55 +1453,11 @@
   pfx_sync();
   UW_STAMP(kind ? 5 : 2);
   if (wave == 0) {
-    const int v_code = (lane >= 1 && lane < nwc) ? sh.code[lane] : -1;
-    const unsigned v_d0 = (lane >= 1 && lane < nwc) ? sh.d0[lane] : 0u, v_d1 = (lane >= 1 && lane < nwc) ? sh.d1[lane] : 0u;
+    const bool have = lane >= 1 && lane < nwc;
+    const int v_code = have ? sh.code[lane] : -1;
+    const unsigned v_d0 = have ? sh.d0[lane] : 0u, v_d1 = have ? sh.d1[lane] : 0u;
     float v_rin = 0.f;
-    int c = 1;
-    while (c < nwc) {
-      const unsigned rb = __float_as_uint(r);
-      const int re = (int)(rb >> 23);
-      const unsigned R = (rb & 0x7FFFFFu) | 0x800000u;
-      bool overflow = false;
-      const unsigned long long other = ~__ballot(lane < nwc && v_code == re) & (~0ull << c);
-      const int cend = other ? __ffsll((long long)other) - 1 : 64;
-      if (cend > c) {
-        const bool in_run = lane >= c && lane < cend;
-        unsigned after;
-        if (__ballot(in_run && v_d0 != v_d1) == 0ull) {
-          after = R + uws_wave_scan_u(in_run ? v_d0 : 0u);
-        } else {
-          const PfxPair in = pfx_pair_wave_scan(in_run ? PfxPair{v_d0, v_d1} : PfxPair{0u, 0u});
-          after = R + ((R & 1u) ? in.a1 : in.a0);
-        }
-        const unsigned long long cross = __ballot(in_run && after >= (1u << 24));
-        const int c1 = cross ? __ffsll((long long)cross) - 1 : cend;
-        if (kind == CHAIN_RUNSUM) {
-          const unsigned prev = (unsigned)__builtin_amdgcn_update_dpp(0, (int)after, 0x138, 0xF, 0xF, false);
-          if (lane >= c && lane < c1) v_rin = lane == c ? r : chain_mant((unsigned)re, prev);
-        }
-        if (c1 > c) r = chain_mant((unsigned)re, (unsigned)__builtin_amdgcn_readlane((int)after, c1 - 1));
-#ifdef TDR_UW_TIMELINE
-        if (threadIdx.x == 0) g_uw_tl[12] += c1 - c;
-#endif
-        c = c1;
-        if (c1 == cend) continue;
-        overflow = true;
-      }
-      const int lo = c * UWS_WC, cnt = min(UWS_WC, n - lo);
-      const int code = __builtin_amdgcn_readlane(v_code, c);
-      if (kind == CHAIN_RUNSUM) v_rin = (lane == c) ? r : v_rin;
-      int pos = 0;
-      const int re_now = (int)(__float_as_uint(r) >> 23);
-      if (!overflow && code >= 0 && re_now <= PFXM_RE_MAX && (code & 0x1FF) == (re_now | UWS_DUAL_FLAG)) {
-        r = uws_wave_dual(a, lo, cnt, r, sh.dual[code >> 16], pos);
-        UW_COUNT(13);
-      }
-      if (pos < cnt) {
-        UW_COUNT(14);
-        r = uws_wave_walk(a, lo, cnt, r, pos);
-      }
-      c++;
-    }
+    r = uws_walk_summaries(a, n, 0, nwc, v_code, v_d0, v_d1, [&](int code) { return sh.dual[code >> 16]; }, r, v_rin);
     if (kind == CHAIN_RUNSUM) rin[lane] = v_rin;
     if (lane == 0) sh.total = r;
   }
@@ -1598,9 +1683,8 @@
   float cmax[64];
   int irregular;
 };
-__device__ __forceinline__ void pfs_wave_fill(int lo, int cnt, float r) {
-  extern __shared__ float uws_lraw[];
-  const UwsAddF a{{}, CHAIN_RUNSUM, 0.f};
+template <class A, class I>
+__device__ __forceinline__ void chain_wave_fill(const A& a, I lo, int cnt, float r, float (&pv)[CHAIN_K]) {
   const int t0 = (threadIdx.x & 63) * CHAIN_K;
   float x[CHAIN_K];
   a.load_items(lo, cnt, t0, x);
@@ -1609,12 +1693,19 @@
   for (int k = 0; k < CHAIN_K; k++) sink.pv[k] = 0.f;
   (void)chain_walk(a, x, t0, 0, cnt, r, ChainWave<true>{}, sink);
 #pragma unroll
+  for (int k = 0; k < CHAIN_K; k++) pv[k] = sink.pv[k];
+}
+__device__ __forceinline__ void pfs_wave_fill(int lo, int cnt, float r) {
+  extern __shared__ float uws_lraw[];
+  const int t0 = (threadIdx.x & 63) * CHAIN_K;
+  float pv[CHAIN_K];
+  chain_wave_fill(UwsAddF{{}, CHAIN_RUNSUM, 0.f}, lo, cnt, r, pv);
+#pragma unroll
   for (int k = 0; k < CHAIN_K; k++)
-    if (t0 + k < cnt) uws_lraw[uws_idx(lo + t0 + k)] = sink.pv[k];
+    if (t0 + k < cnt) uws_lraw[uws_idx(lo + t0 + k)] = pv[k];
 }
 __device__ __forceinline__ void pfx_small_body(const float* __restrict__ w, int n, float* __restrict__ runmax,
-                                               float* __restrict__ prefix_opt,
-                                               float* __restrict__ tail) {
+                                               float* __restrict__ prefix_opt) {
   extern __shared__ float uws_lraw[];
   float* const lraw = uws_lraw;
   __shared__ PfsShared sh;
@@ -1641,11 +1732,10 @@
   }
   if (__ballot(irr) != 0ull && lane == 0) atomicOr(&sh.irregular, 1);
   pfx_sync();
-  const float total = uws_chain_total_waves(UwsAddF{{}, CHAIN_RUNSUM, 0.f}, n, sh.u, sh.rin);
+  (void)uws_chain_total_waves(UwsAddF{{}, CHAIN_RUNSUM, 0.f}, n, sh.u, sh.rin);
   for (int c = 1 + wave; c < nwc; c += NW) pfs_wave_fill(c * UWS_WC, min(UWS_WC, n - c * UWS_WC), sh.rin[c]);
   pfx_sync();
   if (sh.irregular == 0) {
-    if (tail && tid == 0) { tail[0] = total; tail[1] = total; }
     for (int i = tid; i < n; i += nt) {
       const float v = lraw[uws_idx(i)];
       runmax[i] = v;
@@ -1667,7 +1757,6 @@
   }
   pfx_sync();
   const float before = pfs_wave_scan_max(lane < nwc ? sh.cmax[lane] : -INFINITY);
-  if (tail && tid == 63) { tail[0] = total; tail[1] = before; }
   for (int c = wave; c < nwc; c += NW) {
     const int lo = c * UWS_WC, cnt = min(UWS_WC, n - lo);
     const float carry = c > 0 ? __uint_as_float((unsigned)__builtin_amdgcn_readlane((int)__float_as_uint(before), c - 1)) : -INFINITY;
@@ -1690,26 +1779,16 @@
       }
   }
 }
-static_assert(PFXM_THREADS % 64 == 0 && PFXW_THREADS % 64 == 0 && PFXM_THREADS <= UWS_THREADS && PFXW_THREADS <= UWS_THREADS,
-              "summary blocks: whole waves of the head's workgroup");
 __global__ __launch_bounds__(UWS_THREADS) void pfx_small_kernel(const float* __restrict__ w, int n,
-                                                                float* __restrict__ runmax, float* __restrict__ prefix_opt,
-                                                                float* __restrict__ tail, int64_t n_all,
-                                                                PfxChunk* __restrict__ ch, int c_first) {
-  if (blockIdx.x > 0) {
-    if (threadIdx.x < PFXM_THREADS)
-      chain_summary_body<PFXM_THREADS, PFXM_K>(PfxRunSum{{w}, CHAIN_RUNSUM, 0.f}, n_all, ch, c_first - 1);
-    return;
-  }
-  pfx_small_body(w, n, runmax, prefix_opt, tail);
+                                                                float* __restrict__ runmax, float* __restrict__ prefix_opt) {
+  pfx_small_body(w, n, runmax, prefix_opt);
 }
 __global__ __launch_bounds__(UWS_THREADS) void pfx_small_batch_kernel(const TdrBatchEntry* __restrict__ tab) {
   const TdrBatchEntry& e = tab[blockIdx.x];
-  pfx_small_body(e.w_out, (int)e.n, e.runmax_out, nullptr, nullptr);
+  pfx_small_body(e.w_out, (int)e.n, e.runmax_out, nullptr);
 }
 #define TDR_PFX_SMALL_MAX_N 32768
-static int pfx_small(const float* w, int64_t n, float* runmax, float* prefix_opt, hipStream_t st, float* tail = nullptr,
-                     int64_t n_all = 0, PfxChunk* ch = nullptr, int nch = 0) {
+static int pfx_small(const float* w, int64_t n, float* runmax, float* prefix_opt, hipStream_t st) {
   if (n < 1 || n > TDR_PFX_SMALL_MAX_N) return fail(TDR_ERR_ARG, "pfx_small: n out of range");
   const size_t lds = ((size_t)n + (size_t)(n >> 5) + 1 + UWS_PAD) * sizeof(float);
   static bool attr_set[64] = {false};
@@ -1721,97 +1800,174 @@
       return fail(TDR_ERR_HIP, "pfx_small: cannot raise the dynamic LDS limit");
     if (dev < 64) attr_set[dev] = true;
   }
-  const int c_first = ch ? (int)(n / PFXM_CHUNK) : 0;
-  hipLaunchKernelGGL(pfx_small_kernel, dim3(1 + (ch ? (unsigned)std::max(0, nch - c_first) : 0u)), dim3(UWS_THREADS), lds,
-                     st, w, (int)n, runmax, prefix_opt, tail, n_all, ch, c_first);
+  hipLaunchKernelGGL(pfx_small_kernel, dim3(1), dim3(UWS_THREADS), lds, st, w, (int)n, runmax, prefix_opt);
   return TDR_OK;
 }
 
+#define UWG_WAVES (PFXM_THREADS / 64)
+using GridAddF = ChainAddend<float, ChainGlobal, CHAIN_BOUND_22>;
+using GridAddD = ChainAddend<double, ChainGlobal, CHAIN_BOUND_22>;
+__device__ __forceinline__ bool pfx_grid_irregular(const int* __restrict__ irr, int nch) {
+  int f = 0;
+  for (int j = threadIdx.x & 63; j < nch; j += 64) f |= irr[j];
+  return __ballot(f != 0) != 0ull;
+}
+template <class A>
+__device__ __forceinline__ void chain_grid_summary(const A& a, int64_t n, const ChainGridWs& ws) {
+  const int lane = threadIdx.x & 63, wave = __builtin_amdgcn_readfirstlane(threadIdx.x >> 6);
+  const long long nwc = ((long long)n + UWS_WC - 1) / UWS_WC;
+  const long long c = 1 + (long long)blockIdx.x * UWG_WAVES + wave;
+  if (c >= nwc) return;
+  constexpr int PER = PFXM_CHUNK / UWS_WC;
+  const int cc = (int)(c / PER);
+  double acc = 0.0;
+  for (int j = lane; j < cc; j += 64) acc += ws.ch[j].sum;
+  if (lane < (int)(c - (long long)cc * PER)) acc += ws.wc[(long long)cc * PER + lane].sum;
+  const double before = uws_readlane_d(uws_wave_scan_d(acc), 63);
+  bool dualc;
+  int code = uws_predict(before, before + ws.wc[c].sum, dualc);
+  if (dualc) {
+    int slot = 0;
+    if (lane == 0) slot = atomicAdd(&ws.ctl->slots, 1);
+    slot = __builtin_amdgcn_readfirstlane(slot);
+    code = slot < UWG_DUAL_SLOTS ? (code | (slot << 16)) : -1;
+  }
+  const long long lo = c * UWS_WC;
+  const int cnt = (int)min((long long)UWS_WC, (long long)n - lo);
+  PfxPair P = {0u, 0u};
+  const bool ok = code >= 0 && uws_wave_summary(a, lo, cnt, code, ws.dual + (size_t)(code >> 16) * 64, P);
+  if (lane == 63) {
+    WcRec* o = ws.wc + c;
+    o->code = uws_summary_code(code, ok, P);
+    o->d0 = P.a0; o->d1 = P.a1;
+  }
+}
+template <class A, class PUT>
+__device__ __forceinline__ float chain_grid_walk(const A& a, int64_t n, const ChainGridWs& ws, PUT keep) {
+  const int lane = threadIdx.x & 63;
+  const long long nwc = ((long long)n + UWS_WC - 1) / UWS_WC;
+  const int hn = (int)min((long long)UWS_WC, (long long)n);
+  float r = a.kind == CHAIN_RUNSUM ? chain_head_lanes<true>(a, hn, keep) : chain_head_lanes<false>(a, hn, keep);
+  for (long long base = 0; base < nwc; base += 64) {
+    const int nl = (int)min(64ll, nwc - base);
+    const bool have = lane < nl && base + lane >= 1;
+    const WcRec* rec = ws.wc + base + lane;
+    const int v_code = have ? rec->code : -1;
+    const unsigned v_d0 = have ? rec->d0 : 0u, v_d1 = have ? rec->d1 : 0u;
+    float v_rin = 0.f;
+    r = uws_walk_summaries(a, (long long)n, (int)base, nl, v_code, v_d0, v_d1,
+                           [&](int code) { return ws.dual + (size_t)(code >> 16) * 64; }, r, v_rin);
+    if (a.kind == CHAIN_RUNSUM && have) ws.wc[base + lane].rin = v_rin;
+  }
+  return r;
+}
 template <int KIND>
-__global__ __launch_bounds__(UWS_THREADS) void chain_head_kernel(const float* __restrict__ raw, const float* __restrict__ mean_dev,
-                                                                 int n, float* __restrict__ r_out, int64_t n_all,
-                                                                 PfxChunk* __restrict__ ch, int c_first) {
-  const float mean = KIND ? *mean_dev : 0.f;
-  if (blockIdx.x > 0) {
-    if (threadIdx.x < PFXW_THREADS)
-      chain_summary_body<PFXW_THREADS, CHAIN_K>(ChainStat{{raw}, KIND, mean}, n_all, ch, c_first - 1);
+__global__ __launch_bounds__(PFXM_THREADS) void chain_grid_summary_kernel(const float* __restrict__ raw,
+                                                                          const float* __restrict__ mean_dev, int64_t n,
+                                                                          ChainGridWs ws) {
+  if constexpr (KIND == CHAIN_SUM) chain_grid_summary(GridAddF{{raw}, CHAIN_SUM, 0.f}, n, ws);
+  else chain_grid_summary(GridAddD{{raw}, CHAIN_BOTTOM, *mean_dev}, n, ws);
+}
+template <int KIND>
+__global__ __launch_bounds__(64) void chain_grid_walk_kernel(const float* __restrict__ raw, const float* __restrict__ mean_dev,
+                                                             int64_t n, ChainGridWs ws, float* __restrict__ total_out) {
+  float r;
+  if constexpr (KIND == CHAIN_SUM) r = chain_grid_walk(GridAddF{{raw}, CHAIN_SUM, 0.f}, n, ws, [](int, float) {});
+  else r = chain_grid_walk(GridAddD{{raw}, CHAIN_BOTTOM, *mean_dev}, n, ws, [](int, float) {});
+  if (threadIdx.x == 0) *total_out = r;
+}
+static unsigned chain_grid_blocks(int64_t n) { return (unsigned)cdiv(cdiv(n, (int64_t)UWS_WC), (int64_t)UWG_WAVES); }
+static void chain_grid_total(const ChainSrc& s, int64_t n, float* total_out, const ChainGridWs& ws, hipStream_t st) {
+  const dim3 grid(chain_grid_blocks(n));
+  if (s.kind == CHAIN_SUM) {
+    hipLaunchKernelGGL(chain_grid_summary_kernel<CHAIN_SUM>, grid, dim3(PFXM_THREADS), 0, st, s.raw, s.mean, n, ws);
+    hipLaunchKernelGGL(chain_grid_walk_kernel<CHAIN_SUM>, dim3(1), dim3(64), 0, st, s.raw, s.mean, n, ws, total_out);
+  } else {
+    hipLaunchKernelGGL(chain_grid_summary_kernel<CHAIN_BOTTOM>, grid, dim3(PFXM_THREADS), 0, st, s.raw, s.mean, n, ws);
+    hipLaunchKernelGGL(chain_grid_walk_kernel<CHAIN_BOTTOM>, dim3(1), dim3(64), 0, st, s.raw, s.mean, n, ws, total_out);
+  }
+}
+__global__ __launch_bounds__(PFXM_THREADS) void pfx_grid_summary_kernel(const float* __restrict__ w, int64_t n, ChainGridWs ws,
+                                                                        int nch) {
+  if (pfx_grid_irregular(ws.irr, nch)) {
+    if ((int)blockIdx.x < nch) chain_summary_body<PFXM_THREADS, PFXM_K>(PfxRunSum{{w}, CHAIN_RUNSUM, 0.f}, n, ws.ch);
     return;
   }
-  extern __shared__ float uws_lraw[];
-  __shared__ UwsShared ush;
-  const int tid = threadIdx.x, lane = tid & 63, nwc = (n + UWS_WC - 1) / UWS_WC;
-  for (int c = tid >> 6; c < nwc; c += UWS_THREADS / 64) {
-    const int base = c * UWS_WC + lane;
-    float v[CHAIN_K];
-#pragma unroll
-    for (int m = 0; m < CHAIN_K; m++) v[m] = base + 64 * m < n ? raw[base + 64 * m] : __uint_as_float(0x7FC00000u);
-    double acc = 0;
-#pragma unroll
-    for (int m = 0; m < CHAIN_K; m++) {
-      if (base + 64 * m < n) uws_lraw[uws_idx(base + 64 * m)] = v[m];
-      const bool take = KIND == 0 ? v[m] == v[m] : (v[m] == v[m] && v[m] < mean);
-      double x = (double)(KIND == 0 ? v[m] : v[m] - mean);
-      if (KIND) x = x * x;
-      acc += take ? x : 0.0;
-    }
-    acc = uws_wave_scan_d(acc);
-    if (lane == 63) ush.csum[c] = acc;
-  }
-  pfx_sync();
-  float r;
-  if constexpr (KIND == CHAIN_SUM) r = uws_chain_total_waves(UwsAddF{{}, CHAIN_SUM, 0.f}, n, ush);
-  else r = uws_chain_total_waves(UwsAddD{{}, CHAIN_BOTTOM, mean}, n, ush);
-  if (tid == 0) *r_out = r;
-}
-static int chain_head_launch(const float* raw, const float* mean_dev, int kind, int n_head, float* r_out, int64_t n,
-                             PfxChunk* ch, int nch, hipStream_t st) {
-  const size_t lds = ((size_t)n_head + (size_t)(n_head >> 5) + 1 + UWS_PAD) * sizeof(float);
-  static bool attr_set[64] = {false};
-  int dev = 0;
-  if (hipGetDevice(&dev) != hipSuccess || dev < 0) dev = 0;
-  if (dev >= 64 || !attr_set[dev]) {
-    if (hipFuncSetAttribute(reinterpret_cast<const void*>(chain_head_kernel<0>), hipFuncAttributeMaxDynamicSharedMemorySize,
-                            133 * 1024) != hipSuccess ||
-        hipFuncSetAttribute(reinterpret_cast<const void*>(chain_head_kernel<1>), hipFuncAttributeMaxDynamicSharedMemorySize,
-                            133 * 1024) != hipSuccess)
-      return fail(TDR_ERR_HIP, "chain_head: cannot raise the dynamic LDS limit");
-    if (dev < 64) attr_set[dev] = true;
-  }
-  const int c_first = n_head / PFXM_CHUNK;
-  const dim3 grid(1 + (unsigned)std::max(0, nch - c_first));
-  if (kind == 0)
-    hipLaunchKernelGGL(chain_head_kernel<0>, grid, dim3(UWS_THREADS), lds, st, raw, mean_dev, n_head, r_out, n, ch, c_first);
-  else
-    hipLaunchKernelGGL(chain_head_kernel<1>, grid, dim3(UWS_THREADS), lds, st, raw, mean_dev, n_head, r_out, n, ch, c_first);
-  return TDR_OK;
-}
+  chain_grid_summary(GridAddF{{w}, CHAIN_RUNSUM, 0.f}, n, ws);
+}
+__global__ __launch_bounds__(PFXW_THREADS) void pfx_grid_walk_kernel(const float* __restrict__ w, int64_t n, ChainGridWs ws,
+                                                                    int nch, float* __restrict__ runmax,
+                                                                    float* __restrict__ prefix_opt, int head_len) {
+  const bool irregular = pfx_grid_irregular(ws.irr, nch);
+  if (threadIdx.x == 0) ws.ctl->irregular = irregular ? 1 : 0;
+  if (irregular) {
+    pfx_walk_body(w, n, ws.ch, nch, runmax, prefix_opt, head_len);
+    return;
+  }
+  if (threadIdx.x >= 64) return;
+  (void)chain_grid_walk(GridAddF{{w}, CHAIN_RUNSUM, 0.f}, n, ws, [&](int i, float v) {
+    runmax[i] = v;
+    if (prefix_opt) prefix_opt[i] = v;
+  });
+}
+__global__ __launch_bounds__(PFXM_THREADS) void pfx_grid_fill_kernel(const float* __restrict__ w, int64_t n, ChainGridWs ws,
+                                                                    int nch, float* __restrict__ runmax,
+                                                                    float* __restrict__ prefix_opt) {
+  if (ws.ctl->irregular) {
+    if ((int)blockIdx.x < nch) pfx_chunk_fill_body(w, n, ws.ch, (int)blockIdx.x, runmax, prefix_opt);
+    return;
+  }
+  const int lane = threadIdx.x & 63, wave = __builtin_amdgcn_readfirstlane(threadIdx.x >> 6), t0 = lane * CHAIN_K;
+  const long long c = (long long)blockIdx.x * UWG_WAVES + wave;
+  const long long lo = c * UWS_WC;
+  if (c == 0 || lo >= (long long)n) return;
+  const int cnt = (int)min((long long)UWS_WC, (long long)n - lo);
+  float pv[CHAIN_K];
+  chain_wave_fill(GridAddF{{w}, CHAIN_RUNSUM, 0.f}, lo, cnt, ws.wc[c].rin, pv);
+  if (t0 + CHAIN_K <= cnt) {
+    float4* o = reinterpret_cast<float4*>(runmax + lo + t0);
+    o[0] = make_float4(pv[0], pv[1], pv[2], pv[3]);
+    o[1] = make_float4(pv[4], pv[5], pv[6], pv[7]);
+    if (prefix_opt) {
+      float4* q = reinterpret_cast<float4*>(prefix_opt + lo + t0);
+      q[0] = make_float4(pv[0], pv[1], pv[2], pv[3]);
+      q[1] = make_float4(pv[4], pv[5], pv[6], pv[7]);
+    }
+  } else {
+#pragma unroll
+    for (int k = 0; k < CHAIN_K; k++)
+      if (t0 + k < cnt) {
+        runmax[lo + t0 + k] = pv[k];
+        if (prefix_opt) prefix_opt[lo + t0 + k] = pv[k];
+      }
+  }
+}
+static_assert(CHAIN_K == 8, "pfx_grid_fill_kernel: two float4 per lane");
 
 #define TDR_PFX_MULTI_MIN_N 6144
 #define TDR_PFX_EXACT_MIN_N 24576
 #define TDR_PFX_SMALL_MIN_N 256
-extern "C" int64_t tdr_prefix_workspace_bytes(int64_t n) {
-  return n < 1 ? 0 : (int64_t)sizeof(PfxChunk) * cdiv(n, (int64_t)PFXM_CHUNK);
-}
+extern "C" int64_t tdr_prefix_workspace_bytes(int64_t n) { return tdr_chain_workspace_bytes(n, n >= CHAIN_GRID_MIN_N); }
 static int prefix_multi(const float* w, int64_t n, float* runmax_out, float* prefix_out, void* workspace,
                         hipStream_t st) {
   const int64_t nch64 = cdiv(n, (int64_t)PFXM_CHUNK);
   if (nch64 > (1 << 24)) return fail(TDR_ERR_ARG, "prefix: n too large");
   const int nch = (int)nch64;
-  PfxChunk* ch = reinterpret_cast<PfxChunk*>(workspace);
-  const int c_first = chain_head_chunks(n);
-  float* tail = reinterpret_cast<float*>(&ch[0].r0);
-  static_assert(offsetof(PfxChunk, carry0) == offsetof(PfxChunk, r0) + sizeof(float), "tail: sum, maximum");
-  hipLaunchKernelGGL(pfx_chunk_sum_kernel, dim3(nch), dim3(PFXM_THREADS), 0, st, w, n, ch);
-  if (c_first > 0) {
-    const int rc = pfx_small(w, (int64_t)c_first * PFXM_CHUNK, runmax_out, prefix_out, st, tail, n, ch, nch);
-    if (rc) return rc;
-  } else if (nch > c_first) {
-    hipLaunchKernelGGL(pfx_chunk_summary_kernel, dim3(nch - c_first), dim3(PFXM_THREADS), 0, st, w, n, ch, c_first);
-  }
   const int head_len = tdr_cfg().pfx_head;
-  hipLaunchKernelGGL(pfx_walk_kernel, dim3(1), dim3(PFXW_THREADS), 0, st, w, n, ch, nch, runmax_out, prefix_out,
-                     head_len, c_first, (const float*)tail);
-  hipLaunchKernelGGL(pfx_chunk_fill_kernel, dim3(nch), dim3(PFXM_THREADS), 0, st, w, n, (const PfxChunk*)ch,
+  const bool grid = tdr_chain_grid(n);
+  const ChainGridWs ws = chain_grid_ws(workspace, n, grid);
+  hipLaunchKernelGGL(pfx_chunk_sum_kernel, dim3(nch), dim3(PFXW_THREADS), 0, st, w, n, ws);
+  if (grid) {
+    const dim3 blocks(std::max(chain_grid_blocks(n), (unsigned)nch));
+    hipLaunchKernelGGL(pfx_grid_summary_kernel, blocks, dim3(PFXM_THREADS), 0, st, w, n, ws, nch);
+    hipLaunchKernelGGL(pfx_grid_walk_kernel, dim3(1), dim3(PFXW_THREADS), 0, st, w, n, ws, nch, runmax_out, prefix_out,
+                       head_len);
+    hipLaunchKernelGGL(pfx_grid_fill_kernel, blocks, dim3(PFXM_THREADS), 0, st, w, n, ws, nch, runmax_out, prefix_out);
+    return TDR_OK;
+  }
+  hipLaunchKernelGGL(pfx_chunk_summary_kernel, dim3(nch), dim3(PFXM_THREADS), 0, st, w, n, ws.ch);
+  hipLaunchKernelGGL(pfx_walk_kernel, dim3(1), dim3(PFXW_THREADS), 0, st, w, n, ws.ch, nch, runmax_out, prefix_out, head_len);
+  hipLaunchKernelGGL(pfx_chunk_fill_kernel, dim3(nch), dim3(PFXM_THREADS), 0, st, w, n, (const PfxChunk*)ws.ch,
                      runmax_out, prefix_out);
   return TDR_OK;
 }
```

Result: faster. 25.42 million, median of 6 (+1.3%).
